# Audio-WestlakeU/FullSubNet

Hardware: NVIDIA H100
Metric: frames_per_sec (higher is better)
Workload: dtype f16x3(hi+lo split, fp32-class)xf32acc

## Files before the change

### fullsubnet_b200/_lib.py

```python
from __future__ import annotations

import ctypes as C
import os
from typing import Optional

import numpy as np
import torch

_HERE = os.path.dirname(os.path.abspath(__file__))
LIB_PATH = os.path.join(_HERE, "csrc", "libfsn_b200.so")

FSN_OK, FSN_ERR_SHAPE, FSN_ERR_UNSUPPORTED, FSN_ERR_CUDA, FSN_ERR_WORKSPACE = 0, 1, 2, 3, 4
ACT = {None: 0, False: 0, "": 0, "ReLU": 1, "Tanh": 2, "ReLU6": 3}
CELL = {"LSTM": 0, "GRU": 1}
PREC = {"fp32": 0, "f16_tc": 1, "tf32_tc": 2, "f16x3_tc": 3}


class ModelDesc(C.Structure):
    _fields_ = [(n, C.c_int32) for n in (
        "num_freqs", "look_ahead", "fb_num_neighbors", "sb_num_neighbors", "fb_hidden", "sb_hidden",
        "fb_activation", "sb_activation", "norm_type", "num_groups_in_drop_band", "precision", "cell_type")]


class SeqWeights(C.Structure):
# ... 29 lines not shown

class FastGrads(C.Structure):
    _fields_ = [("enc1", LstmGrads), ("enc2", LstmGrads), ("enc_fc_w", C.c_void_p), ("enc_fc_b", C.c_void_p),
                ("bn", LstmGrads * 2), ("bn_fc_w", C.c_void_p), ("bn_fc_b", C.c_void_p),
                ("dec1", LstmGrads), ("dec2", LstmGrads), ("dec_fc_w", C.c_void_p), ("dec_fc_b", C.c_void_p)]


MAX_PARAM_TENSORS = 64
SB_PROBE_FIELDS, SB_PROBE_SLOTS = 16, 4


class ParamList(C.Structure):
    _fields_ = [("n", C.c_int), ("param", C.c_void_p * MAX_PARAM_TENSORS), ("grad", C.c_void_p * MAX_PARAM_TENSORS),
                ("exp_avg", C.c_void_p * MAX_PARAM_TENSORS), ("exp_avg_sq", C.c_void_p * MAX_PARAM_TENSORS),
                ("numel", C.c_int64 * MAX_PARAM_TENSORS)]


class FullbandDesc(C.Structure):
    _fields_ = [("num_freqs", C.c_int32), ("hidden", C.c_int32), ("num_layers", C.c_int32), ("look_ahead", C.c_int32),
                ("activation", C.c_int32), ("norm_type", C.c_int32), ("precision", C.c_int32), ("cell_type", C.c_int32)]


class FullbandGrads(C.Structure):
    _fields_ = [("layer", LstmGrads * 8), ("fc_w", C.c_void_p), ("fc_b", C.c_void_p)]


IMP_MAX_SECTIONS = 8


class ImprovedDesc(C.Structure):
    _fields_ = [("n_fft", C.c_int32), ("hop_length", C.c_int32), ("win_length", C.c_int32), ("num_freqs", C.c_int32),
                ("fdrc", C.c_float), ("num_sections", C.c_int32), ("freq_cutoffs", C.c_int32 * IMP_MAX_SECTIONS),
                ("sb_num_center", C.c_int32 * IMP_MAX_SECTIONS), ("sb_num_neighbor", C.c_int32 * IMP_MAX_SECTIONS),
                ("fb_num_center", C.c_int32 * IMP_MAX_SECTIONS), ("fb_num_neighbor", C.c_int32 * IMP_MAX_SECTIONS),
                ("fb_hidden", C.c_int32), ("sb_hidden", C.c_int32), ("fb_activation", C.c_int32),
                ("sb_activation", C.c_int32), ("precision", C.c_int32), ("cell_type", C.c_int32)]


class ImprovedWeights(C.Structure):
    _fields_ = [("fb", SeqWeights), ("sb", SeqWeights * IMP_MAX_SECTIONS), ("sb_packed", C.c_void_p * IMP_MAX_SECTIONS)]


class ImprovedGrads(C.Structure):
    _fields_ = [("fb", SeqGrads), ("sb", SeqGrads * IMP_MAX_SECTIONS)]


_P, _I, _L, _F, _S = C.c_void_p, C.c_int, C.c_int64, C.c_float, C.c_size_t
_SIGNATURES = {
    "fsn_version": (C.c_int, []),
    "fsn_last_error": (C.c_char_p, []),
    "fsn_built_arch": (C.c_int, []),
    "fsn_stft": (C.c_int, [_P, _I, _I, _I, _I, _I, _P, _P, _P, _P, _P, _I, _P]),
    "fsn_istft": (C.c_int, [_P, _P, _I, _P, _I, _I, _I, _I, _I, _I, _P, _P]),
    "fsn_decompress_cirm": (C.c_int, [_P, _P, _L, _F, _F, _P]),
    "fsn_compress_cirm": (C.c_int, [_P, _P, _L, _F, _F, _P]),
    "fsn_build_cirm": (C.c_int, [_P, _P, _P, _P, _P, _L, _P]),
    "fsn_drop_band": (C.c_int, [_P, _P, _I, _I, _I, _I, _I, _P]),
    "fsn_model_workspace_bytes": (_S, [C.POINTER(ModelDesc), _I, _I]),
    "fsn_sb_packed_bytes": (_S, [C.POINTER(ModelDesc)]),
    "fsn_pack_sb_weights": (C.c_int, [C.POINTER(ModelDesc), C.POINTER(SeqWeights), _P, _P]),
    "fsn_model_forward": (C.c_int, [C.POINTER(ModelDesc), C.POINTER(SeqWeights), C.POINTER(SeqWeights), _P, _P,
                                    _I, _I, _P, _P, _S, _P]),
    "fsn_enhance_workspace_bytes": (_S, [C.POINTER(ModelDesc), _I, _I, _I, _I]),
    "fsn_enhance": (C.c_int, [C.POINTER(ModelDesc), C.POINTER(SeqWeights), C.POINTER(SeqWeights), _P, _P, _P, _I, _I,
                              _I, _I, _I, _P, _P, _P, _F, _P, _S, _P]),
    "fsn_fast_workspace_bytes": (_S, [C.POINTER(FastDesc), _I, _I]),
    "fsn_fast_packed_bytes": (_S, [C.POINTER(FastDesc)]),
    "fsn_fast_pack_bn_weights": (C.c_int, [C.POINTER(FastDesc), C.POINTER(FastWeights), _P, _P]),
    "fsn_fast_model_forward": (C.c_int, [C.POINTER(FastDesc), C.POINTER(FastWeights), _P, _I, _I, _P, _P, _S, _P]),
    "fsn_improved_workspace_bytes": (_S, [C.POINTER(ImprovedDesc), _I, _I]),
    "fsn_improved_forward": (C.c_int, [C.POINTER(ImprovedDesc), C.POINTER(ImprovedWeights), _P, _I, _I, _P, _P, _P, _S,
                                       _P]),
    "fsn_improved_enhance_workspace_bytes": (_S, [C.POINTER(ImprovedDesc), _I, _I]),
    "fsn_improved_enhance": (C.c_int, [C.POINTER(ImprovedDesc), C.POINTER(ImprovedWeights), _P, _P, _I, _I, _P, _P, _P, _F,
                                       _P, _S, _P]),
    "fsn_improved_packed_bytes": (_S, [C.POINTER(ImprovedDesc), _I]),
    "fsn_improved_pack_sb_weights": (C.c_int, [C.POINTER(ImprovedDesc), C.POINTER(ImprovedWeights), _I, _P, _P]),
    "fsn_improved_train_workspace_bytes": (_S, [C.POINTER(ImprovedDesc), _I, _I]),
    "fsn_improved_train_forward": (C.c_int, [C.POINTER(ImprovedDesc), C.POINTER(ImprovedWeights), _P, _I, _I, _P, _P, _S,
                                             _P]),
    "fsn_improved_train_backward": (C.c_int, [C.POINTER(ImprovedDesc), C.POINTER(ImprovedWeights), _P, _I, _I,
                                              C.POINTER(ImprovedGrads), _P, _S, _P]),
    "fsn_train_workspace_bytes": (_S, [C.POINTER(ModelDesc), _I, _I]),
    "fsn_train_forward": (C.c_int, [C.POINTER(ModelDesc), C.POINTER(SeqWeights), C.POINTER(SeqWeights), _P, _I, _I, _P,
                                    _P, _S, _P]),
    "fsn_train_backward": (C.c_int, [C.POINTER(ModelDesc), C.POINTER(SeqWeights), C.POINTER(SeqWeights), _P, _I, _I,
                                     C.POINTER(SeqGrads), C.POINTER(SeqGrads), _P, _S, _P]),
    "fsn_fast_train_workspace_bytes": (_S, [C.POINTER(FastDesc), _I, _I]),
    "fsn_fast_train_forward": (C.c_int, [C.POINTER(FastDesc), C.POINTER(FastWeights), _P, _I, _I, _P, _P, _S, _P]),
    "fsn_fast_train_backward": (C.c_int, [C.POINTER(FastDesc), C.POINTER(FastWeights), _P, _I, _I, C.POINTER(FastGrads), _P,
                                          _S, _P]),
    "fsn_mse_loss_scratch_bytes": (_S, []),
    "fsn_mse_loss": (C.c_int, [_P, _P, _I, _I, _I, _P, _P, _P, _S, _P]),
    "fsn_cirm_mse_per_clip_workspace_bytes": (_S, [_I, _I, _I, _I]),
    "fsn_cirm_mse_per_clip": (C.c_int, [_P, _P, _P, _I, _I, _I, _I, _I, _P, _P, _P, _S, _P]),
    "fsn_clip_adam_scratch_bytes": (_S, []),
    "fsn_clip_adam": (C.c_int, [C.POINTER(ParamList), _F, _F, _F, _F, _F, _F, _I, _P, _P, _S, _P]),
    "fsn_clip_adam_steps": (C.c_int, [C.POINTER(ParamList), _F, _F, _F, _F, _F, _F, _P, _P, _P, _S, _P]),
    "fsn_fullband_workspace_bytes": (_S, [C.POINTER(FullbandDesc), _I, _I]),
    "fsn_fullband_forward": (C.c_int, [C.POINTER(FullbandDesc), _P, _P, _P, _P, _I, _I, _P, _P, _S, _P]),
    "fsn_fullband_enhance_workspace_bytes": (_S, [C.POINTER(FullbandDesc), _I, _I, _I, _I]),
    "fsn_fullband_enhance": (C.c_int, [C.POINTER(FullbandDesc), _P, _P, _P, _P, _P, _I, _I, _I, _I, _I, _P, _P, _P, _F, _P,
                                       _S, _P]),
    "fsn_fullband_stream_state_bytes": (_S, [C.POINTER(FullbandDesc), _I, _I, _I]),
    "fsn_fullband_stream_workspace_bytes": (_S, [C.POINTER(FullbandDesc), _I, _I, _I, _I]),
    "fsn_fullband_stream_delay": (C.c_int, [C.POINTER(FullbandDesc), _I, _I]),
    "fsn_fullband_stream_step": (C.c_int, [C.POINTER(FullbandDesc), _P, _P, _P, _P, _P, _P, _I, _I, _I, _I, _I, _P, _P, _S,
                                           _P, _S, _P]),
    "fsn_fast_stream_state_bytes": (_S, [C.POINTER(FastDesc), _I, _I, _I]),
    "fsn_fast_stream_workspace_bytes": (_S, [C.POINTER(FastDesc), _I, _I, _I, _I]),
    "fsn_fast_stream_delay": (C.c_int, [C.POINTER(FastDesc), _I, _I]),
    "fsn_fast_stream_step": (C.c_int, [C.POINTER(FastDesc), C.POINTER(FastWeights), _P, _P, _P, _I, _I, _I, _I, _I, _P, _P,
                                       _S, _P, _S, _P]),
    "fsn_fast_stream_tc_state_bytes": (_S, [C.POINTER(FastDesc), _I, _I, _I]),
    "fsn_fast_stream_tc_workspace_bytes": (_S, [C.POINTER(FastDesc), _I, _I, _I, _I]),
    "fsn_fast_stream_tc_delay": (C.c_int, [C.POINTER(FastDesc), _I, _I]),
    "fsn_fast_stream_tc_step": (C.c_int, [C.POINTER(FastDesc), C.POINTER(FastWeights), _P, _P, _P, _I, _I, _I, _I, _I, _P,
                                          _P, _S, _P, _S, _P]),
    "fsn_stream_state_bytes": (_S, [C.POINTER(ModelDesc), _I, _I, _I]),
    "fsn_stream_workspace_bytes": (_S, [C.POINTER(ModelDesc), _I, _I, _I, _I]),
    "fsn_stream_delay": (C.c_int, [C.POINTER(ModelDesc), _I, _I]),
    "fsn_stream_step": (C.c_int, [C.POINTER(ModelDesc), C.POINTER(SeqWeights), C.POINTER(SeqWeights), _P, _P, _P, _I, _I,
                                  _I, _I, _I, _P, _P, _S, _P, _S, _P]),
    "fsn_stream_tc_state_bytes": (_S, [C.POINTER(ModelDesc), _I, _I, _I]),
    "fsn_stream_tc_workspace_bytes": (_S, [C.POINTER(ModelDesc), _I, _I, _I, _I]),
    "fsn_stream_tc_delay": (C.c_int, [C.POINTER(ModelDesc), _I, _I]),
    "fsn_stream_tc_step": (C.c_int, [C.POINTER(ModelDesc), C.POINTER(SeqWeights), C.POINTER(SeqWeights), _P, _P, _P, _P,
                                     _I, _I, _I, _I, _I, _P, _P, _S, _P, _S, _P]),
    "fsn_fullband_train_workspace_bytes": (_S, [C.POINTER(FullbandDesc), _I, _I]),
    "fsn_fullband_train_forward": (C.c_int, [C.POINTER(FullbandDesc), _P, _P, _P, _P, _I, _I, _P, _P, _S, _P]),
    "fsn_fullband_train_backward": (C.c_int, [C.POINTER(FullbandDesc), _P, _P, _P, _P, _I, _I, C.POINTER(FullbandGrads), _P,
                                              _S, _P]),
    "fsn_peak_normalize_int16": (C.c_int, [_P, _I, _I, _F, _P, _P]),
    "fsn_si_sdr": (C.c_int, [_P, _P, _I, _I, _P, _P]),
    "fsn_si_sdr_lengths": (C.c_int, [_P, _P, _P, _I, _I, _P, _P]),
    "fsn_stoi_workspace_bytes": (_S, [_I, _I, _I]),
    "fsn_stoi": (C.c_int, [_P, _P, _P, _I, _I, _I, _P, _P, _S, _P]),
    "fsn_rir_convolve": (C.c_int, [_P, _P, _P, _I, _I, _I, _P, _P]),
    "fsn_snr_mix": (C.c_int, [_P, _P, _P, _P, _F, _F, _I, _I, _P, _P, _P]),
    "fsn_debug_row_to_unit": (C.c_int, [_I, _I, _I, _I, C.POINTER(C.c_int), C.POINTER(C.c_int)]),
    "fsn_debug_unit_to_row": (C.c_int, [_I, _I, _I, _I, _I]),
    "fsn_debug_reflect_count": (C.c_int, [_I, _I, _I]),
    "fsn_debug_lstm_tc_workspace_bytes": (_S, [_I, _I, _I, _I, _I]),
    "fsn_debug_lstm_layer_tc": (C.c_int, [_P, _P, _P, _P, _P, _I, _I, _I, _I, _I, _P, _P, _S, _P]),
    "fsn_debug_lstm_tc_carry": (C.c_int, [_P, _P, _P, _P, _P, _I, _I, _I, _I, _I, _P, _P, _P, _I, _P, _P, _S, _P]),
    "fsn_debug_linear_tc": (C.c_int, [_P, _I, _I, _P, _P, _I, _I, _I, _P, _P, _S, _P]),
    "fsn_debug_lstm_rec_tc_scratch_bytes": (_S, [_I, _I]),
    "fsn_debug_lstm_rec_tc": (C.c_int, [_P, _P, _P, _P, _L, _L, _P, _L, _L, _I, _I, _I, _I, _P, _P, _P, _L, _P, _I, _P, _P,
                                        _S, _P]),
    "fsn_debug_sb_lstm_tc_packed_bytes": (_S, [_I, _I]),
    "fsn_debug_sb_lstm_tc_max_clusters": (C.c_int, [_I, _I, _I, _I, C.POINTER(C.c_int)]),
    "fsn_debug_sb_lstm_tc": (C.c_int, [C.POINTER(SeqWeights), _I, _I, _I, _I, _I, _I, _P, _P, _I, _I, _I, _I, _P, _P, _I,
                                       _I, _I, _I, _I, _P, _P, _P]),
    "fsn_debug_sb_lstm_tc_carry": (C.c_int, [C.POINTER(SeqWeights), _I, _I, _I, _I, _I, _P, _P, _I, _I, _I, _P, _I, _P,
                                             _I, _P, _P, _P, _P, _P]),
    "fsn_debug_sb_lstm_tc_phased": (C.c_int, [C.POINTER(SeqWeights), _I, _I, _I, _I, _P, _P, _I, _I, _I, _I, _P, _P, _P,
                                              _P, _P, _P, _P, _P, _P, _P]),
    "fsn_debug_sb_lstm_tc_probe": (C.c_int, [C.POINTER(SeqWeights), _I, _I, _I, _I, _I, _I, _P, _P, _I, _I, _I, _I, _P, _P,
                                             _I, _I, _I, _I, _I, _P, _P, _P, _I, _I, _P]),
    "fsn_debug_tgemm": (C.c_int, [_P, _L, _P, _L, _P, _L, _I, _I, _I, _I, _P, _L, _P]),
    "fsn_debug_tgemm_blocked": (C.c_int, [_P, _P, _P, _I, _I, _I, _I, _I, _P, _L, _P]),
    "fsn_debug_lstm_fwd_step": (C.c_int, [_P, _P, _P, _P, _I, _P, _P, _P, _P, _P, _P, _I, _I, _I, _P, _L, _P]),
    "fsn_debug_fc_gemm": (C.c_int, [_P, _P, _P, _P, _I, _I, _I, _I, _I, _P]),
    "fsn_debug_sgemm": (C.c_int, [_I, _P, _L, _P, _L, _P, _L, _I, _I, _I, _I, _P, _L, _P]),
    "fsn_debug_colsum": (C.c_int, [_P, _L, _I, _L, _P, _P, _P, _L, _P]),
    "fsn_debug_small_out_wgrad": (C.c_int, [_P, _P, _L, _I, _P, _P, _L, _P]),
    "fsn_debug_transpose": (C.c_int, [_P, _L, _I, _P, _P]),
    "fsn_debug_transpose_blocked": (C.c_int, [_P, _L, _I, _L, _P, _P, _I, C.POINTER(C.c_int), _P, _P]),
    "fsn_debug_gemm_tc": (C.c_int, [_P, _L, _I, _P, _I, _I, _P, _I, _P, _I, _I, _P, _L, _L, _P, _S, _P]),
    "fsn_debug_lstm_train_workspace_bytes": (_S, [_I, _I, _I, _I, _I, _I]),
    "fsn_debug_lstm_train": (C.c_int, [C.POINTER(LstmLayer), _I, _I, _I, _I, _I, _I, _P, _P, _P, _P, _I, _P, _P,
                                       C.POINTER(LstmGrads), _P, _P, _S, _P]),
    "fsn_debug_seq_stack_workspace_bytes": (_S, [_I, C.POINTER(C.c_int), _I, _I, _I, _I, _I, _I, _I, _I]),
    "fsn_debug_seq_stack": (C.c_int, [C.POINTER(LstmLayer), _I, C.POINTER(C.c_int), _I, _I, _I, _I, _I, _I, _I, _I, _P, _P,
                                      _P, _P, _I, _I, _P, _P, _S, C.POINTER(C.c_int), _P]),
    "fsn_debug_stft": (C.c_int, [_P, _I, _I, _I, _I, _I, _P, _P, _P, _P, _P, _P, _P, _I, _P]),
    "fsn_debug_istft": (C.c_int, [_P, _P, _I, _P, _I, _I, _I, _I, _I, _I, _I, _P, _P, _P, _P, _P, _F, _P, _P]),
    "fsn_debug_istft_mask_adjoint": (C.c_int, [_P, _P, _P, _I, _I, _I, _I, _I, _I, _P, _P]),
    "fsn_debug_wav_epilogue": (C.c_int, [_P, _P, _I, _I, _P, _P, _F, _P, _P, _I, _I, _I, _P]),
    "fsn_debug_norm_unfold_bwd": (C.c_int, [_P, _P, _P, _P, _I, _I, _I, _I, _I, _I, _F, _I, _P, _P, _P]),
    "fsn_debug_fast_norm_unfold_bwd": (C.c_int, [_P, _P, _P, _P, _P, _P, _I, _I, _I, _I, _I, _I, _I, _F, _P, _P, _P, _P]),
    "fsn_debug_imp_unfold_bwd": (C.c_int, [_P, _P, _P, _P, _I, _I, _I, _I, _I, _I, _I, _I, _I, _I, _I, _P, _P, _P]),
    "fsn_debug_imp_section_input": (C.c_int, [_P, _P, _I, _I, _I, _I, _I, _I, _I, _I, _I, _I, _P, _P, _P]),
    "fsn_debug_imp_section_lstm_tc_workspace_bytes": (_S, [_I, _I, _I, _I, _I]),
    "fsn_debug_imp_section_lstm_tc": (C.c_int, [C.POINTER(SeqWeights), _I, _I, _I, _P, _I, _I, _I, _I, _P, _P, _P, _S, _P]),
    "fsn_debug_norm_stats": (C.c_int, [_P, _I, _I, _I, _I, _L, _L, _P, _P, _I, _I, _P, _F, _F, _F, _P, _P, _P, _P, _P]),
    "fsn_debug_train_stats": (C.c_int, [_P, _I, _I, _I, _I, _I, _P, _P]),
    "fsn_debug_forgetting_scale": (C.c_int, [_P, _I, _P, _I, _I, _I, _I, _L, _L, _F, _P, _P, _I, _I, _P, _P, _P, _P, _P]),
    "fsn_debug_forgetting_bwd": (C.c_int, [_P, _P, _P, _P, _I, _I, _I, _I, _I, _I, _P, _P, _P]),
    "fsn_debug_stoi_stages": (C.c_int, [_P, _P, _P, _I, _I, _I, _P, _P, _P, _P, _P, _P, _P, _S, _P]),
    "fsn_debug_cum_clip_scale": (C.c_int, [_P, _I, _I, _I, _L, _L, _F, _P, _P, _P]),
    "fsn_debug_cum_unit_scale": (C.c_int, [_P, _P, _I, _I, _I, _I, _I, _I, _F, _I, _P, _P]),
    "fsn_debug_forget_unit_broadcast": (C.c_int, [_P, _I, _I, _I, _I, _P, _P]),
    "fsn_debug_fast_bn": (C.c_int, [_P, _P, _L, _L, _I, _I, _I, _I, _I, _I, _I, _F, _P, _P, _P, _P, _P]),
    "fsn_debug_fast_dec_input": (C.c_int, [_P, _P, _L, _L, _L, _I, _I, _I, _I, _I, _L, _L, _P, _P]),
    "fsn_debug_transpose_mag": (C.c_int, [_P, _I, _I, _I, _I, _L, _L, _P, _P, _P, _P]),
    "fsn_debug_crm_output": (C.c_int, [_P, _L, _L, _I, _I, _I, _I, _P, _P]),
    "fsn_debug_scale_rows": (C.c_int, [_P, _P, _L, _I, _I, _I, _P, _P]),
    "fsn_debug_imp_compress": (C.c_int, [_P, _I, _I, _I, _F, _I, _P, _P]),
    "fsn_debug_train_gather": (C.c_int, [_P, _P, _P, _P, _I, _I, _I, _I, _I, _I, _P, _P]),
    "fsn_debug_sb_head": (C.c_int, [_P, _I, _I, _I, _P, _P, _I, _I, _I, _I, _I, _I, _L, _L, _I, _P, _P]),
    "fsn_debug_sb_head_bwd": (C.c_int, [_P, _P, _I, _I, _I, _I, _I, _I, _I, _I, _I, _L, _L, _P, _P]),
    "fsn_debug_train_dy": (C.c_int, [_P, _P, _I, _I, _I, _I, _I, _I, _P, _P]),
    "fsn_last_error_code": (C.c_int, []),
    "fsn_last_launch_count": (C.c_int64, []),
    "fsn_total_launch_count": (C.c_int64, []),
    "fsn_set_profiling": (C.c_int, [_I]),
    "fsn_last_stage_ms": (C.c_float, [_I]),
}
EXPORTED_SYMBOLS = tuple(_SIGNATURES)

_lib: Optional[C.CDLL] = None


def load() -> C.CDLL:
    global _lib
    if _lib is None:
        if not os.path.exists(LIB_PATH):
            raise RuntimeError(
                f"fullsubnet_b200: {LIB_PATH} is missing. Build it with `python -c 'import __graft_entry__ as g; "
                "g.build()'` (nvcc, sm_90a). There is no CPU/PyTorch fallback for this path.")
        lib = C.CDLL(LIB_PATH)
        for name, (res, args) in _SIGNATURES.items():
            fn = getattr(lib, name)
            fn.restype, fn.argtypes = res, args
        _lib = lib
    return _lib


def check(rc: int) -> None:
    if rc == FSN_OK:
        return
    msg = load().fsn_last_error().decode()
    if rc == FSN_ERR_SHAPE:
        raise AssertionError(msg)
    if rc == FSN_ERR_UNSUPPORTED:
        raise NotImplementedError(msg)
    raise RuntimeError(f"libfsn_b200 error {rc}: {msg}")


def check_workspace(nbytes: int) -> int:
    if nbytes == 0:
        check(load().fsn_last_error_code() or FSN_ERR_SHAPE)
    return nbytes


def require_cuda(t: torch.Tensor, what: str) -> torch.Tensor:
    if not t.is_cuda:
        raise RuntimeError(
            f"fullsubnet_b200: {what} must be a CUDA tensor (got {t.device}); this package has no CPU path.")
    if t.dtype != torch.float32:
        t = t.float()
    return t.contiguous()


def lengths_table(lengths, B: int, L: int) -> np.ndarray:
    if isinstance(lengths, torch.Tensor):
        if lengths.is_cuda or lengths.is_floating_point() or lengths.is_complex() or lengths.dim() != 1:
            raise ValueError("lengths must be a 1-D CPU integer tensor or a sequence of ints")
        lengths = lengths.tolist()
    lens = np.ascontiguousarray([int(v) for v in lengths], dtype=np.int32)
    if lens.shape != (B,):
        raise ValueError(f"lengths has {lens.size} entries for a batch of {B} clips")
    if lens.size and int(lens.max()) > L:
        b = int(lens.argmax())
        raise ValueError(f"lengths[{b}] = {int(lens[b])} exceeds the {L} samples of a row")
    return lens


def stream_ptr(device) -> int:
    return torch.cuda.current_stream(device).cuda_stream


def ptr(t: Optional[torch.Tensor]) -> Optional[int]:
    return None if t is None else t.data_ptr()
```

### fullsubnet_b200/csrc/fsn_internal.cuh

```cuda
#pragma once
#include <cudaTypedefs.h>
#include <cuda_fp16.h>

#include "fsn_common.cuh"

namespace fsn {

struct Carver {
  char* base; size_t off;
  explicit Carver(void* p) : base((char*)p), off(0) {}
  template <class T> T* take(size_t n) {
    T* r = base ? (T*)(base + off) : nullptr;
    off = align_up(off + n * sizeof(T), 256);
    return r;
  }
};

inline fsn_lstm_layer seq_layer(const fsn_seq_weights& w, int l) { return {w.w_ih[l], w.w_hh[l], w.b_ih[l], w.b_hh[l]}; }

inline unsigned ew_grid(size_t n) {
  const size_t g = (n + 255) / 256;
  return (unsigned)(g < 1 ? 1 : (g > 132 * 16 ? 132 * 16 : g));
}

// ... 226 lines not shown
                 unsigned int* peak_bits = nullptr, const int* lens = nullptr);

struct WavWs {
  float *real, *imag, *crm;
  unsigned int* peak;
  int* lens;
};
void wav_carve(Carver& c, int B, int F, int T, WavWs& w);
int wav_check(const int32_t* lengths, int B, int L_max, int n_fft, bool pow2_lengths, const float* enhanced,
              const char* who);
int wav_prologue(const int32_t* lengths, int B, WavWs& w, cudaStream_t st);
int wav_epilogue(const WavWs& w, const float* enhanced, int B, int L, int16_t* pcm, float gain, float* crm_out, int F, int T,
                 int hop, cudaStream_t st);

int istft_mask_adjoint_launch(const float* dwav, const float* real, const float* imag, int B, int L, int T, int n_fft,
                              int hop, int win_length, float* dcrm, cudaStream_t st);

struct SecGeom { int lo, N, cs, ns, cf, nf, W; };
struct ImpDims { int B, L, T, F, Fu, S; SecGeom sec[FSN_IMP_MAX_SECTIONS]; int maxRW, maxR; };
int imp_dims(const fsn_improved_desc* d, int B, int L, ImpDims& m);
int imp_compress_launch(const float* mag, int B, int F, int T, float fdrc, bool tm, float* out, cudaStream_t st);
int imp_section_input_launch(const float* magc, const float* fbT, int B, int T, int Fu, const SecGeom& g, float* X, float2* fs,
                             bool tm, cudaStream_t st);
int sec_geom(int lo, int hi, int cs, int ns, int cf, int nf, int Fu, SecGeom& g);
int imp_unfold_bwd_launch(const float* dX, const float* invs, const float* dot, float cnt, const SecGeom& g, int B, int T,
                          int Fu, bool first, int act, const float* y, float* dfb, cudaStream_t st);
inline HeadGeom imp_head_geom(const SecGeom& g, int F, int T) { return HeadGeom{g.N, g.cs, g.lo, F, (size_t)T}; }

struct FbState {
  const float* h_init[2]; const float* c_init[2];
  float* h_fin[2]; float* c_fin[2];
  const int* restart;
  int fin_step;
};
bool fb_persistent_supported(int F, int H0, int H1);
int fb_persistent_launch(const fsn_lstm_layer* L, const float* x, const float* inv1, float* h0buf, float* h1all,
                         unsigned int* barrier, int R, int F, int H0, int H1, int Tp, cudaStream_t st,
                         const FbState* io = nullptr);

bool lstm_rec_tc_supported(int H, bool x3);
int lstm_rec_tc_rows_per_launch(int H);
size_t lstm_rec_tc_scratch_bytes(int H, bool x3);
struct RecCarry {
  const float *h_init, *c_init;
  float* c_fin;
  size_t row;
  const int* restart;
  int fin_step;
};
struct RecTcInfo {
  int rows_per_launch, stages, launches, smem_bytes;
};
int lstm_rec_tc_launch(const float* w_hh, const float* b_ih, const float* b_hh, const float* P, size_t p_row, size_t p_t,
                       float* hall, size_t h_row, size_t h_t, int R, int T, int H, bool x3, void* scratch,
                       cudaStream_t st, const RecCarry* io = nullptr, RecTcInfo* info = nullptr);
int split_tf32_launch(const float* in, size_t rows, int K, size_t ldi, const float* row_scale, int rows_per_scale,
                      float* out, int Kp, int cat, cudaStream_t st, int scale_B = 0);
int bias_act_launch(float* x, size_t rows, int N, size_t ld, const float* bias, int act, cudaStream_t st);
struct LstmTcWs { float *a, *w, *P; void* rec; };
void lstm_tc_carve(Carver& c, size_t rows_T, int Kmax, int Hmax, bool x3, LstmTcWs& ws);
int lstm_layer_tc(const fsn_lstm_layer& L, const float* x, size_t ldx, int K, const float* row_scale, int rows_per_scale,
                  int scale_B, int R, int T, int H, bool x3, const LstmTcWs& ws, float* hall, cudaStream_t st,
                  const RecCarry* io = nullptr);
int linear_tc(const float* x, size_t ldx, int K, const float* W, const float* bias, int N, int act, float* out, size_t ldo,
              size_t rows, bool x3, const LstmTcWs& ws, cudaStream_t st);
int gemm_tc_split_launch(const float* a, size_t lda, const float* W, int N, int K, float* w, float* C, size_t ldc, size_t M,
                         bool x3, cudaStream_t st);

static const int SEQ_MAX_LAYERS = 8;
struct SeqStack {
  int R, Tp, K0, n, O, act;
  int H[SEQ_MAX_LAYERS];
  fsn_lstm_layer L[SEQ_MAX_LAYERS];
  bool gru, step_scale, tc, x3;
  bool force_stepwise;
  const float *x, *scale, *fc_w, *fc_b;
  float* out;
};
enum SeqPath {
  SEQ_PATH_TC = FSN_SEQ_PATH_TC,
  SEQ_PATH_PERSISTENT = FSN_SEQ_PATH_PERSISTENT,
  SEQ_PATH_STEP2 = FSN_SEQ_PATH_STEP2,
  SEQ_PATH_ONE_LAYER = FSN_SEQ_PATH_ONE_LAYER
};
SeqPath seq_stack_path(const SeqStack& s);
struct SeqStackWs {
  float *hall[2], *h0[2], *c0, *c1, *pp;
  unsigned int* barrier;
  LstmTcWs tc;
};
void seq_stack_carve(Carver& c, const SeqStack& s, SeqStackWs& w);
int seq_stack_forward(const SeqStack& s, const SeqStackWs& w, cudaStream_t st);

struct StreamGeom { int n, hop, la, c, D, Hs, Rc, Q, E; };
int stream_geom(int n_fft, int hop, int win_length, int la, StreamGeom& g);
struct StreamMeta { int pos, active; float acc; int pad; };
int stream_prologue(const int32_t* start, const int32_t* tail, int B, char* state, size_t slot_bytes, int* pos0, int* act0,
                    int* tail_dev, cudaStream_t st);
int stream_norm_launch(const float2* fs, int B, int S, int K, int F, const StreamGeom& g, int norm_type, const int* pos0,
                       const int* act0, const int* tail, char* state, size_t slot_bytes, float* scaleT, cudaStream_t st,
                       const float2* fs2 = nullptr, size_t acc_off = 0);
int stream_cum_unit_launch(const float* magT, const float* fbT, int B, int S, int K, int F, int Ns, int Nf,
                           const StreamGeom& g, const int* pos0, const int* act0, char* state, size_t slot_bytes,
                           size_t run_off, float* scaleT, cudaStream_t st);
int stream_reset_launch(const int* pos0, int B, const StreamGeom& g, int j, int H, float* h, size_t h_row, float* c,
                        cudaStream_t st);
int stream_restart_launch(const int* pos0, int B, const StreamGeom& g, int* restart, cudaStream_t st);
int stream_dsp_check(int n_fft, int hop, int win_length);
int stft_stream_launch(const float* win, int Wn, int Hs, const int* pos0, const int* tail, int B, int n_fft, int hop,
                       int win_length, int c, int S, int Q, float* magT, float* spec, cudaStream_t st);
int istft_stream_launch(const float* spec, const float* crm, const int* pos0, const int* act0, const int* tail, int B,
                        int K, int D, int n_fft, int hop, int win_length, int c, int la, int Rc, int Q, int S, float* wav,
                        cudaStream_t st);
struct StackCarry { char* state; size_t slot, h, c; const int* pos0; StreamGeom g; const int* restart; int K; };
struct StreamStackWs { SeqStackWs seq; float* h; float *h_fin[2], *c_fin[2]; };
void stream_stack_carve(Carver& c, const SeqStack& s, StreamStackWs& w);
int stream_seq_stack(const SeqStack& s, const StreamStackWs& w, const StackCarry& io, cudaStream_t st);
int copy_rows(void* dst, size_t dp, const void* src, size_t sp, size_t width, int B, cudaStream_t st);

struct StreamSlot {
  size_t hist, spec, crm, end;
  StreamSlot(const StreamGeom& g, int F);
  size_t sec(size_t floats) { const size_t at = end; end = align_up(end + floats * 4, 16); return at; }
  size_t slot() const { return align_up(end, 256); }
};
struct StreamWs {
  int *pos0, *act0, *tail;
  float *wav, *magT, *spec, *crm;
};
void stream_carve(Carver& c, const StreamGeom& g, int B, int K, int F, StreamWs& w);
int stream_query_check(int rc, const char* who, int B, int K_max);
inline int stream_delay(int rc, const StreamGeom& g) { return rc ? -rc : g.D; }
int stream_check(const char* who, const StreamGeom& g, int B, int K, const int32_t* tail, const float* wav,
                 const float* enhanced, int& St);
int stream_check_sizes(const void* state, size_t state_bytes, size_t slot, int B, const void* workspace,
                       size_t workspace_bytes, size_t ws_need);
int stream_open(const StreamGeom& g, const StreamSlot& sl, const StreamWs& w, int F, int B, int K, int St, int win_length,
                const int32_t* start, const int32_t* tail, const float* wav, char* state, int* restart, cudaStream_t st);
int stream_close(const StreamGeom& g, const StreamSlot& sl, const StreamWs& w, int F, int B, int K, int St, int win_length,
                 const float* y, float* enhanced, char* state, cudaStream_t st);

struct SbTcArgs {
  const void* packed;
  const float* magT; const float* fbT; const float* inv2;
  const float* unit_scale;
  float* crm;
  int B, F, Tp, la, Ns, Nf, H, act;
  int steps, shrink;
  bool x3;
  RowMap map;
  int stages, cluster;
  long long* stamps;
  int stamp_ctas, stamp_its;
};
size_t sb_tc_packed_bytes(const fsn_model_desc* d);
size_t sb_tc_packed_bytes_raw(int H, bool x3, bool proj = false);
int sb_tc_pack(const fsn_model_desc* d, const fsn_seq_weights* sb, void* packed, cudaStream_t st);
int sb_tc_pack_raw(const fsn_seq_weights* sb, int H, int Ksb, int fc_out, void* packed, cudaStream_t st, bool x3,
                   bool proj = false);
int sb_tc_forward(const SbTcArgs& a, cudaStream_t st);
struct SbCarry {
  float *h, *c;
  size_t slot, layer;
  int rps;
  const int* restart;
  int store_step;
  size_t crm_bs;
  int crm_t0;
  const float* x;
  const int* store_at;
};
int sb_tc_carry_forward(const SbTcArgs& a, const SbCarry& io, cudaStream_t st);
bool sb_tc_supported(const fsn_model_desc* d);
void sb_tc_ring_defaults(int& stages, int& cluster);
struct SbProjArgs {
  const void* packed;
  const float* P;
  float* h1;
  int R, T, H;
  bool x3;
  int stages, cluster;
};
int sb_proj_forward(const SbProjArgs& a, cudaStream_t st);
struct ImpSecTcWs { LstmTcWs gemm; float *P, *h1; };
void imp_section_tc_carve(Carver& c, size_t rows_T, int Wmax, int H, bool x3, ImpSecTcWs& w);
int imp_section_lstm_tc(const fsn_seq_weights& sw, const void* packed, const float* X, int R, int T, int W, int H, bool x3,
                        const ImpSecTcWs& w, cudaStream_t st, int stages = 0, int cluster = 0);

}
```

### fullsubnet_b200/csrc/fsn_model.cu

```cuda
#include <string.h>

#include "fsn_internal.cuh"

namespace fsn {

static thread_local char g_err[512] = "";
static thread_local int64_t g_launches = 0;

void set_error(const char* fmt, ...) {
  va_list ap;
  va_start(ap, fmt);
  vsnprintf(g_err, sizeof(g_err), fmt, ap);
  va_end(ap);
}
static thread_local int g_err_code = 0;
int& last_error_code() { return g_err_code; }
int64_t& launch_counter() { return g_launches; }
static int64_t g_total_launches = 0;
int64_t& total_launch_counter() { return g_total_launches; }

static thread_local bool g_prof = false;
static thread_local cudaEvent_t g_ev[5] = {nullptr, nullptr, nullptr, nullptr, nullptr};
static thread_local bool g_ev_valid[5] = {false, false, false, false, false};
static void prof_mark(int i, cudaStream_t st) {
  if (!g_prof) return;
  if (!g_ev[i] && cudaEventCreate(&g_ev[i]) != cudaSuccess) return;
  g_ev_valid[i] = (cudaEventRecord(g_ev[i], st) == cudaSuccess);
}
static void prof_reset() { for (int i = 0; i < 5; ++i) g_ev_valid[i] = false; }

struct ModelWs {
  float *magT, *fbT, *inv1, *inv2;
  float2 *fs, *sums_mag, *sums_fb;
  float *cum1, *cum2;
  float2* fs2;
  SeqStackWs fb;
  float *sb_h0[2], *sb_h1[2], *sb_c0, *sb_c1;
  size_t bytes;
};

static SeqStack fb_stack(const fsn_model_desc* d, int B, int Tp) {
  SeqStack s;
  memset(&s, 0, sizeof(s));
  const int F = d->num_freqs;
  s.R = B; s.Tp = Tp; s.K0 = F; s.n = 2; s.H[0] = s.H[1] = d->fb_hidden; s.O = F; s.act = d->fb_activation;
  s.gru = d->cell_type == FSN_CELL_GRU;
  s.step_scale = norm_per_step(d->norm_type);
  s.x3 = d->precision == FSN_PREC_F16X3_TC;
  s.tc = (s.x3 || d->precision == FSN_PREC_F16_TC) && !s.gru && lstm_rec_tc_supported(d->fb_hidden, s.x3);
  return s;
}

int make_dims(const fsn_model_desc* d, int B, int T, Dims& m) {
  FSN_REQUIRE(d && d->num_freqs > 1 && d->fb_hidden > 0 && d->sb_hidden > 0 && d->look_ahead >= 0, FSN_ERR_SHAPE,
              "model: bad descriptor");
  FSN_REQUIRE(B > 0 && T > 0, FSN_ERR_SHAPE, "model: empty input (B=%d, T=%d)", B, T);
  FSN_REQUIRE(d->norm_type == FSN_NORM_OFFLINE_LAPLACE || d->norm_type == FSN_NORM_CUMULATIVE_LAPLACE ||
                  d->norm_type == FSN_NORM_FORGETTING,
              FSN_ERR_UNSUPPORTED,
              "You must set up a type of Norm. (offline_laplace_norm / cumulative_laplace_norm / forgetting_norm are built)");
  FSN_REQUIRE(d->cell_type == FSN_CELL_LSTM || (d->cell_type == FSN_CELL_GRU && d->precision == FSN_PREC_FP32),
              FSN_ERR_UNSUPPORTED, "model: sequence_model must be LSTM, or GRU on the fp32 kernels (precision fp32)");
  FSN_REQUIRE(d->sb_num_neighbors >= 0 && d->fb_num_neighbors >= 0 && d->sb_num_neighbors < d->num_freqs &&
                  d->fb_num_neighbors < d->num_freqs,
              FSN_ERR_SHAPE, "model: reflect padding needs num_neighbors < num_freqs");
  m.B = B; m.T = T; m.Tp = T + d->look_ahead; m.F = d->num_freqs;
  m.G = (B > 1 && d->num_groups_in_drop_band > 1) ? d->num_groups_in_drop_band : 1;
  if (B > 1)
    FSN_REQUIRE(B > d->num_groups_in_drop_band, FSN_ERR_SHAPE,
                "Batch size = %d, num_groups = %d. The batch size should larger than the num_groups.", B,
                d->num_groups_in_drop_band);
  m.Fsub = (m.G > 1) ? m.F / m.G : m.F;
  FSN_REQUIRE(m.Fsub > 0, FSN_ERR_SHAPE, "model: num_freqs < num_groups");
  m.R = B * m.Fsub;
  m.Ksb = (2 * d->sb_num_neighbors + 1) + (2 * d->fb_num_neighbors + 1);
  return FSN_OK;
}

static void carve_model(const fsn_model_desc* d, const Dims& m, void* base, ModelWs& w) {
  Carver c(base);
  const size_t BTF = (size_t)m.B * m.Tp * m.F;
  w.magT = c.take<float>(BTF);
  w.fbT = c.take<float>(BTF);
  w.fs = c.take<float2>((size_t)m.B * m.Tp);
  w.sums_mag = c.take<float2>(m.B);
  w.sums_fb = c.take<float2>(m.B);
  w.inv1 = c.take<float>(m.B);
  w.inv2 = c.take<float>(m.B);
  seq_stack_carve(c, fb_stack(d, m.B, m.Tp), w.fb);
  if (d->precision == FSN_PREC_FP32) {
    const size_t RH = (size_t)m.R * d->sb_hidden;
    for (int i = 0; i < 2; ++i) { w.sb_h0[i] = c.take<float>(RH); w.sb_h1[i] = c.take<float>(RH); }
    w.sb_c0 = c.take<float>(RH);
    w.sb_c1 = c.take<float>(RH);
  }
  w.cum1 = w.cum2 = nullptr;
  w.fs2 = nullptr;
  if (norm_per_step(d->norm_type)) {
    w.cum1 = c.take<float>((size_t)m.Tp * m.B);
    w.cum2 = c.take<float>((size_t)m.Tp * m.R);
  }
  if (d->norm_type == FSN_NORM_FORGETTING) w.fs2 = c.take<float2>((size_t)m.B * m.Tp);
  w.bytes = c.off;
}

static int model_core(const fsn_model_desc* d, const fsn_seq_weights* fb, const fsn_seq_weights* sb,
                      const void* sb_packed, const Dims& m, const ModelWs& w, float* crm, cudaStream_t st,
                      const int* lens = nullptr, int hop = 0) {
  int rc;
  const int F = m.F, Tp = m.Tp, B = m.B, Hs = d->sb_hidden, la = d->look_ahead;
  const int tp_cnt = lens ? 1 : Tp;
  if ((rc = clip_stats_launch(w.magT, B, Tp, F, d->sb_num_neighbors, w.fs, w.sums_mag, st, lens, hop, la))) return rc;
  if ((rc = norm_scales_launch(w.sums_mag, w.sums_mag, B, (float)F * tp_cnt, 1.f, w.inv1, nullptr, st, 1e-5f, lens, hop,
                               la)))
    return rc;
  const bool cum = d->norm_type == FSN_NORM_CUMULATIVE_LAPLACE, fgt = d->norm_type == FSN_NORM_FORGETTING;
  const float cum_eps = 1.1920928955078125e-07f;
  if (cum && (rc = cum_clip_scale_launch(w.fs, B, Tp, F, cum_eps, w.cum1, st))) return rc;
  if (fgt && (rc = forget_scale_launch(w.fs, nullptr, B, Tp, (float)F, w.cum1, nullptr, st))) return rc;

  SeqStack s = fb_stack(d, B, Tp);
  s.L[0] = seq_layer(*fb, 0); s.L[1] = seq_layer(*fb, 1);
  s.x = w.magT; s.scale = (cum || fgt) ? w.cum1 : w.inv1; s.fc_w = fb->fc_w; s.fc_b = fb->fc_b; s.out = w.fbT;
  if ((rc = seq_stack_forward(s, w.fb, st))) return rc;

  if ((rc = clip_stats_launch(w.fbT, B, Tp, F, d->fb_num_neighbors, fgt ? w.fs2 : w.fs, w.sums_fb, st, lens, hop, la)))
    return rc;
  if ((rc = norm_scales_launch(w.sums_mag, w.sums_fb, B, 1.f, (float)F * m.Ksb * tp_cnt, nullptr, w.inv2, st, 1e-5f, lens,
                               hop, la)))
    return rc;

  prof_mark(2, st);
  RowMap map{B, F, m.Fsub, m.G};
  if (cum && (rc = cum_unit_scale_launch(w.magT, w.fbT, map, m.R, Tp, d->sb_num_neighbors, d->fb_num_neighbors, cum_eps,
                                         w.cum2, st)))
    return rc;
  if (fgt) {
    if ((rc = forget_scale_launch(w.fs, w.fs2, B, Tp, (float)F * m.Ksb, w.cum1, nullptr, st))) return rc;
    if ((rc = forget_unit_broadcast_launch(w.cum1, map, m.R, Tp, w.cum2, st))) return rc;
  }
  if (d->precision == FSN_PREC_F16_TC || d->precision == FSN_PREC_F16X3_TC) {
    FSN_REQUIRE(sb_packed, FSN_ERR_SHAPE, "model: the tensor-core precisions need packed sub-band weights");
    SbTcArgs a;
    memset(&a, 0, sizeof(a));
    a.packed = sb_packed; a.magT = w.magT; a.fbT = w.fbT; a.inv2 = w.inv2; a.crm = crm;
    a.B = B; a.F = F; a.Tp = Tp; a.la = d->look_ahead; a.Ns = d->sb_num_neighbors; a.Nf = d->fb_num_neighbors;
    a.H = Hs; a.act = d->sb_activation; a.map = map; a.x3 = d->precision == FSN_PREC_F16X3_TC;
    a.unit_scale = (cum || fgt) ? w.cum2 : nullptr;
    rc = sb_tc_forward(a, st);
    prof_mark(3, st);
    return rc;
  }

  const Step2State s2{{w.sb_h0[0], w.sb_h0[1]}, w.sb_c0, {w.sb_h1[0], w.sb_h1[1]}, w.sb_c1, Hs, 0};
  for (int t = 0; t < Tp; ++t) {
    StepParams p;
    memset(&p, 0, sizeof(p));
    p.R = m.R; p.H = Hs; p.gru = d->cell_type == FSN_CELL_GRU;
    p.K0 = m.Ksb;
    p.w_ih = sb->w_ih[0]; p.w_hh = sb->w_hh[0]; p.b_ih = sb->b_ih[0]; p.b_hh = sb->b_hh[0];
    p.magT = w.magT; p.fbT = w.fbT; p.inv2 = w.inv2;
    p.unit_scale = (cum || fgt) ? w.cum2 + (size_t)t * m.R : nullptr;
    p.F = F; p.Tp = Tp; p.t = t; p.Ns = d->sb_num_neighbors; p.Nf = d->fb_num_neighbors; p.map = map;
    if ((rc = lstm_step2_launch(p, SEG0_GATHER, t, seq_layer(*sb, 1), s2, st))) return rc;
    if (t >= d->look_ahead)
      if ((rc = sb_head_launch(s2.h1_at(t), m.R, Hs, 1, sb->fc_w, sb->fc_b, 2, d->sb_activation, crm,
                               fsn_head_geom(m.Fsub, m.T), t - d->look_ahead, st)))
        return rc;
  }
  prof_mark(3, st);
  return FSN_OK;
}

}

using namespace fsn;

extern "C" int fsn_version(void) { return 102; }
extern "C" const char* fsn_last_error(void) { return g_err; }
extern "C" int fsn_last_error_code(void) { return g_err_code; }
extern "C" int64_t fsn_last_launch_count(void) { return g_launches; }
extern "C" int64_t fsn_total_launch_count(void) { return g_total_launches; }
extern "C" int fsn_set_profiling(int enable) { g_prof = enable != 0; return FSN_OK; }
extern "C" float fsn_last_stage_ms(int stage) {
  if (stage < 0 || stage > 3 || !g_ev_valid[stage] || !g_ev_valid[stage + 1]) return -1.0f;
  float ms = -1.0f;
  if (cudaEventElapsedTime(&ms, g_ev[stage], g_ev[stage + 1]) != cudaSuccess) return -1.0f;
  return ms;
}
extern "C" int fsn_debug_row_to_unit(int B, int F, int G, int r, int* b, int* f) {
  const int g = (B > 1 && G > 1) ? G : 1;
  RowMap m{B, F, g > 1 ? F / g : F, g};
  if (r < 0 || r >= B * m.Fsub) return FSN_ERR_SHAPE;
  row_to_unit(m, r, *b, *f);
  return FSN_OK;
}
extern "C" int fsn_debug_unit_to_row(int B, int F, int G, int b, int f) {
  const int g = (B > 1 && G > 1) ? G : 1;
  RowMap m{B, F, g > 1 ? F / g : F, g};
  return unit_to_row(m, b, f);
}
extern "C" int fsn_debug_reflect_count(int r, int F, int N) { return reflect_count(r, F, N); }

extern "C" int fsn_built_arch(void) {
#ifdef FSN_BUILT_ARCH
  return FSN_BUILT_ARCH;
#else
  return 0;
#endif
}

extern "C" size_t fsn_model_workspace_bytes(const fsn_model_desc* d, int B, int T) {
  Dims m;
  if (make_dims(d, B, T, m)) return 0;
  ModelWs w;
  carve_model(d, m, nullptr, w);
  return w.bytes;
}

extern "C" size_t fsn_sb_packed_bytes(const fsn_model_desc* d) { return sb_tc_packed_bytes(d); }

extern "C" int fsn_pack_sb_weights(const fsn_model_desc* d, const fsn_seq_weights* sb, void* packed,
                                   fsn_stream_t stream) {
  return sb_tc_pack(d, sb, packed, (cudaStream_t)stream);
}

extern "C" int fsn_model_forward(const fsn_model_desc* d, const fsn_seq_weights* fb, const fsn_seq_weights* sb,
                                 const void* sb_packed, const float* noisy_mag, int B, int T, float* crm,
                                 void* workspace, size_t workspace_bytes, fsn_stream_t stream) {
  g_launches = 0;
  Dims m;
  int rc = make_dims(d, B, T, m);
  if (rc) return rc;
  if ((rc = layout_clips_check(B, false, "model"))) return rc;
  FSN_REQUIRE(d->precision == FSN_PREC_FP32 || sb_tc_supported(d), FSN_ERR_UNSUPPORTED,
              "FSN_PREC_F16_TC / FSN_PREC_F16X3_TC need sb_hidden in {128,256,384} and sub-band input width <= 32");
  ModelWs w;
  carve_model(d, m, workspace, w);
  FSN_REQUIRE(workspace && workspace_bytes >= w.bytes, FSN_ERR_WORKSPACE, "workspace too small: %zu < %zu",
              workspace_bytes, w.bytes);
  cudaStream_t st = (cudaStream_t)stream;
  prof_reset();
  prof_mark(0, st);
  if ((rc = transpose_mag_launch(noisy_mag, B, m.F, T, m.Tp, (size_t)m.Tp * m.F, m.F, w.magT, nullptr, nullptr, st))) return rc;
  prof_mark(1, st);
  return model_core(d, fb, sb, sb_packed, m, w, crm, st);
}

static int enhance_dims(const fsn_model_desc* d, int B, int L, int n_fft, int hop, fsn_model_desc& dd, Dims& m) {
  FSN_REQUIRE(hop > 0 && n_fft > 0, FSN_ERR_SHAPE, "enhance: bad n_fft/hop");
  dd = *d;
  dd.num_groups_in_drop_band = 1;
  int rc = make_dims(&dd, B, 1 + L / hop, m);
  if (rc) return rc;
  FSN_REQUIRE(n_fft / 2 + 1 == d->num_freqs, FSN_ERR_SHAPE, "enhance: n_fft/2+1 = %d != num_freqs = %d",
              n_fft / 2 + 1, d->num_freqs);
  return FSN_OK;
}

static size_t carve_enhance(const fsn_model_desc* d, const Dims& m, void* base, WavWs& e, ModelWs& w) {
  Carver c(base);
  wav_carve(c, m.B, m.F, m.T, e);
  carve_model(d, m, base ? (char*)base + c.off : nullptr, w);
  return c.off + w.bytes;
}

extern "C" size_t fsn_enhance_workspace_bytes(const fsn_model_desc* d, int B, int L_max, int n_fft, int hop) {
  fsn_model_desc dd;
  Dims m;
  if (enhance_dims(d, B, L_max, n_fft, hop, dd, m)) return 0;
  WavWs e;
  ModelWs w;
  return carve_enhance(&dd, m, nullptr, e, w);
}

extern "C" int fsn_enhance(const fsn_model_desc* d, const fsn_seq_weights* fb, const fsn_seq_weights* sb,
                           const void* sb_packed, const float* wav, const int32_t* lengths, int B, int L_max, int n_fft,
                           int hop, int win_length, float* enhanced, float* crm_out, int16_t* pcm, float gain,
                           void* workspace, size_t workspace_bytes, fsn_stream_t stream) {
  g_launches = 0;
  fsn_model_desc dd;
  Dims m;
  int rc = enhance_dims(d, B, L_max, n_fft, hop, dd, m);
  if (rc) return rc;
  FSN_REQUIRE(dd.precision == FSN_PREC_FP32 || sb_tc_supported(&dd), FSN_ERR_UNSUPPORTED,
              "FSN_PREC_F16_TC / FSN_PREC_F16X3_TC need sb_hidden in {128,256,384} and sub-band input width <= 32");
  if ((rc = wav_check(lengths, B, L_max, n_fft, true, enhanced, "enhance"))) return rc;
  WavWs e;
  ModelWs w;
  const size_t bytes = carve_enhance(&dd, m, workspace, e, w);
  FSN_REQUIRE(workspace && workspace_bytes >= bytes, FSN_ERR_WORKSPACE, "workspace too small: %zu < %zu",
              workspace_bytes, bytes);
  cudaStream_t st = (cudaStream_t)stream;
  float* crm = crm_out ? crm_out : e.crm;
  prof_reset();
  prof_mark(0, st);
  if ((rc = wav_prologue(lengths, B, e, st))) return rc;
  if ((rc = stft_launch(wav, B, L_max, n_fft, hop, win_length, nullptr, nullptr, e.real, e.imag, w.magT, m.Tp, st,
                        e.lens)))
    return rc;
  prof_mark(1, st);
// ... 222 lines not shown
```

### fullsubnet_b200/csrc/fsn_subband_tc.cu

```cuda
#include <cuda_fp16.h>
#include <stdlib.h>
#include <string.h>

#include "fsn_internal.cuh"
#include "fsn_tc_ptx.cuh"
#include "fsn_wgmma.cuh"

namespace fsn {
namespace tc {

using namespace ptx;

constexpr int NB = 32;
constexpr int KB = 64;
constexpr int KS = 32;
constexpr int US = 64;
constexpr int W_SUB = US * KS * 2;
constexpr int W_TILE = 4 * W_SUB;
constexpr int S_KBLK = NB * KB * 2;
constexpr int X_BLK = NB * KS * 2;
constexpr int MAX_STAGES = 4;
constexpr int MAX_MT = 3;
constexpr int OUT_T = 8;
constexpr int NTHREADS = 128 + 128 * MAX_MT;

struct PackedLayout {
  int H, MT, nkb0, nkb1, parts;
  size_t tiles0, tiles1;
  size_t off_bias, off_fcw, off_fcb, bytes;
};

__host__ __device__ inline PackedLayout packed_layout(int H, bool x3, bool proj = false) {
  PackedLayout L;
  L.H = H; L.MT = H / 128;
  L.nkb0 = (proj ? 0 : 1) + H / KS; L.nkb1 = 2 * H / KS;
  L.parts = x3 ? 2 : 1;
  L.tiles0 = (size_t)L.MT * L.nkb0 * L.parts;
  L.tiles1 = (size_t)L.MT * L.nkb1 * L.parts;
  L.off_bias = 2 * (L.tiles0 + L.tiles1) * W_TILE;
  L.off_fcw = L.off_bias + (size_t)2 * 4 * H * sizeof(float);
  L.off_fcb = L.off_fcw + (size_t)2 * H * sizeof(float);
  L.bytes = L.off_fcb + 256;
  return L;
}

__global__ void pack_kernel(const float* __restrict__ wih0, const float* __restrict__ whh0,
                            const float* __restrict__ wih1, const float* __restrict__ whh1,
                            const float* __restrict__ bih0, const float* __restrict__ bhh0,
                            const float* __restrict__ bih1, const float* __restrict__ bhh1,
                            const float* __restrict__ fcw, const float* __restrict__ fcb, int H, int Ksb, int x3,
                            int fc_out, int proj, uint8_t* __restrict__ out) {
  const PackedLayout L = packed_layout(H, x3 != 0, proj != 0);
  const size_t per_half = L.tiles0 + L.tiles1;
  const size_t total = 2 * per_half * 4 * US * 4;
  for (size_t i = blockIdx.x * (size_t)blockDim.x + threadIdx.x; i < total; i += (size_t)gridDim.x * blockDim.x) {
    const int c = (int)(i & 3);
    const int r = (int)((i >> 2) & (US - 1));
    const int g = (int)((i >> 8) & 3);
    const size_t st_abs = i >> 10;
    const int half = (int)(st_abs / per_half);
    size_t st = st_abs - half * per_half;
    const int layer = st >= L.tiles0;
    if (layer) st -= L.tiles0;
    const int part = (int)(st % L.parts);
    st /= L.parts;
    const int nkb = layer ? L.nkb1 : L.nkb0;
    const int kb = (int)(st % nkb);
    const int m = (int)(st / nkb);
    const int wrow = g * H + (half * L.MT + m) * US + r;
    __half v[8];
#pragma unroll
    for (int e = 0; e < 8; ++e) {
      const int kk = c * 8 + e;
      float w = 0.f;
      if (layer == 0 && proj) {
        w = whh0[(size_t)wrow * H + kb * KS + kk];
      } else if (layer == 0) {
        if (kb == 0) { if (kk < Ksb) w = wih0[(size_t)wrow * Ksb + kk]; }
        else w = whh0[(size_t)wrow * H + (kb - 1) * KS + kk];
      } else {
        const int k = kb * KS + kk;
        w = (k < H) ? wih1[(size_t)wrow * H + k] : whh1[(size_t)wrow * H + (k - H)];
      }
      const __half hi = __float2half_rn(w);
      v[e] = part ? __float2half_rn(w - __half2float(hi)) : hi;
    }
    uint8_t* dst = out + st_abs * W_TILE + g * W_SUB + swz64_off(r, c * 8);
    *reinterpret_cast<uint4*>(dst) = *reinterpret_cast<const uint4*>(v);
  }
  float* bias = reinterpret_cast<float*>(out + L.off_bias);
  float* pfcw = reinterpret_cast<float*>(out + L.off_fcw);
  float* pfcb = reinterpret_cast<float*>(out + L.off_fcb);
  for (int i = blockIdx.x * blockDim.x + threadIdx.x; i < 4 * H; i += gridDim.x * blockDim.x) {
    bias[i] = proj ? 0.f : bih0[i] + bhh0[i];
    bias[4 * H + i] = bih1[i] + bhh1[i];
  }
  for (int i = blockIdx.x * blockDim.x + threadIdx.x; i < 2 * H; i += gridDim.x * blockDim.x)
    pfcw[i] = (!proj && i < fc_out * H) ? fcw[i] : 0.f;
  if (blockIdx.x == 0 && threadIdx.x < 2)
    pfcb[threadIdx.x] = (!proj && (int)threadIdx.x < fc_out) ? fcb[threadIdx.x] : 0.f;
}

struct Smem {
  uint32_t w, x, h0, h1, lo, fcw, fcp, outst, rows, bars, total;
};
__host__ __device__ inline Smem smem_plan(int H, int stages, bool x3) {
  Smem s;
  const int nkh = H / KB;
  uint32_t o = 0;
  s.w = o; o += stages * W_TILE;
  s.x = o; o += 2 * X_BLK;
  s.h0 = o; o += 2 * nkh * S_KBLK;
  s.h1 = o; o += nkh * S_KBLK;
  s.lo = o; o += x3 ? (o - s.x) : 0;
  s.fcw = o; o += 4 * MAX_MT * 2 * NB * 4;
  s.fcp = o; o += 2 * 2 * NB * 4;
  s.outst = o; o += NB * 2 * OUT_T * 4;
  s.rows = o; o += NB * 16;
  s.bars = o; o += 256;
  s.total = o;
  return s;
}

struct Bars {
  uint64_t w_full[MAX_STAGES], w_empty[MAX_STAGES];
  uint64_t x_full[2], x_empty[2];
  uint64_t h0_ready[2], h0_empty[2];
  uint64_t h1_ready, h1_empty, fc_done;
  uint64_t l1_done;
  uint64_t fcp_full[2], fcp_empty[2];
  uint64_t turn[MAX_MT];
};
static_assert(sizeof(Bars) <= 256, "barrier block too large");

struct RowInfo {
  int src_b, src_f;
  float scale;
  union {
    int out_idx;
    int restart;
  };
};

struct KArgs {
  const uint8_t* packed;
  const float* magT; const float* fbT; const float* inv2;
  const float* unit_scale;
  float* crm;
  int R, F, Tp, la, T, Ns, Nf, H, Ksb, act, Fsub, stages, cluster;
  int src_T, shrink;
  RowMap map;
  long long* stamps;
  int stamp_ctas, stamp_its;
  const float* proj; float* h1;
  float* io_h; float* io_c;
  size_t io_slot, io_layer, crm_bs;
  const int* restart;
  int io_rps, store_step, crm_t0;
  const float* xin;
  const int* store_at;
};

enum ProbeField {
  PF_T_BEGIN = 0,
  PF_T_MMA0 = 1,
  PF_T_MMA1 = 2,
  PF_T_END = 3,
  PF_OPERAND = 4,
  PF_TURN = 5,
  PF_W_FULL = 6,
  PF_WAIT_GROUP = 7,
  PF_GROUP_LAT = 8,
  PF_STAGES = 9,
  PF_CELL = 10,
  PF_L1_DONE = 11,
  PF_H1_EMPTY = 12,
  PF_H0_EMPTY = 13,
  PF_FC_DONE = 14,
  PF_GT_BEGIN = 15,
  PROBE_FIELDS = 16
};
constexpr int PROBE_SLOTS = MAX_MT + 1;
static_assert(PROBE_FIELDS == FSN_SB_PROBE_FIELDS && PROBE_SLOTS == FSN_SB_PROBE_SLOTS,
              "probe record layout differs from fsn_b200.h (and fullsubnet_b200/_lib.py)");

__device__ __forceinline__ long long globaltimer() {
  uint64_t t;
  asm volatile("mov.u64 %0, %%globaltimer;" : "=l"(t));
  return (long long)t;
}

__device__ __forceinline__ float act_apply(float v, int act) {
  switch (act) {
    case FSN_ACT_RELU: return fmaxf(v, 0.f);
    case FSN_ACT_TANH: return tanhf(v);
    case FSN_ACT_RELU6: return fminf(fmaxf(v, 0.f), 6.f);
    default: return v;
  }
}
template <bool X3> __device__ __forceinline__ float sg(float x) { return X3 ? 1.0f / (1.0f + expf(-x)) : fast_sigmoid(x); }
template <bool X3> __device__ __forceinline__ float th(float x) { return X3 ? 1.0f - 2.0f / (1.0f + expf(2.0f * x)) : fast_tanh(x); }

__device__ __forceinline__ void release_stage(uint32_t bar, uint32_t pred, uint32_t local, uint32_t remote,
                                              uint32_t rank) {
  mbar_arrive_elect_if(bar, pred & local);
  mbar_arrive_remote_elect_if(bar, rank, pred & remote);
}

__device__ __forceinline__ float proj_at(const KArgs& a, int t, int row0, int s, int q, int lane, int g, int i) {
  const int j = i >> 2, hh = (i >> 1) & 1, e = i & 1;
  const int u = s * US + 16 * q + (lane >> 2) + 8 * hh;
  const int r = min(row0 + 8 * j + 2 * (lane & 3) + e, a.R - 1);
  return __ldg(a.proj + ((size_t)t * a.R + r) * 4 * a.H + g * a.H + u);
}

__device__ __forceinline__ size_t carry_idx(const KArgs& a, int r, int u) {
  const int sl = r / a.io_rps;
  return (size_t)sl * a.io_slot + (size_t)(r - sl * a.io_rps) * a.H + u;
}

template <bool X3, bool PROBE, bool PROJ, bool CARRY, bool PHASED = false>
__device__ __forceinline__ void sb_lstm_tc_body(const KArgs& a) {
  static_assert(!PHASED || CARRY, "the block-phased policy is a carry policy");
  constexpr int PARTS = X3 ? 2 : 1;
  long long pt = 0;
  auto mark = [&]() -> uint32_t {
    if constexpr (PROBE) {
      const long long n = clock64();
      const uint32_t d = (uint32_t)(n - pt);
      pt = n;
      return d;
    } else {
      return 0u;
    }
  };
  auto record = [&](int it, int layer, int slot) -> long long* {
    return a.stamps + ((((size_t)blockIdx.x * a.stamp_its + it) * 2 + layer) * PROBE_SLOTS + slot) * PROBE_FIELDS;
  };
  const bool probe_cta = PROBE && (int)blockIdx.x < a.stamp_ctas;
  extern __shared__ uint8_t smem_raw[];
  uint8_t* smem = smem_raw + ((1024u - (smem_u32(smem_raw) & 1023u)) & 1023u);
  const int H = a.H;
  const int MT = H / 128;
  const int nkh = H / KB;
  const int STAGES = a.stages;
  const int CL = a.cluster;
  const uint32_t cl_rank = cluster_ctarank();
  const int half = (int)(cl_rank & 1u);
  const uint32_t peer = cl_rank ^ 1u;
  const uint16_t cl_mask = (uint16_t)((0x55u & ((1u << (2 * CL)) - 1u)) << half);
  const Smem sp = smem_plan(H, STAGES, X3);
  const uint32_t LO = sp.lo - sp.x;
  const PackedLayout PL = packed_layout(H, X3, PROJ);
  Bars& bars = *reinterpret_cast<Bars*>(smem + sp.bars);
  RowInfo* rows = reinterpret_cast<RowInfo*>(smem + sp.rows);
  float* fc_part = reinterpret_cast<float*>(smem + sp.fcw);
  float* fcp = reinterpret_cast<float*>(smem + sp.fcp);
  float* outst = reinterpret_cast<float*>(smem + sp.outst);
  const int warp = threadIdx.x >> 5, lane = threadIdx.x & 31;
  const int row0 = (blockIdx.x >> 1) * NB;
  const int Tp = a.Tp;

  if (threadIdx.x == 0) {
    for (int s = 0; s < STAGES; ++s) { mbar_init(&bars.w_full[s], 1); mbar_init(&bars.w_empty[s], CL); }
    for (int i = 0; i < 2; ++i) {
      mbar_init(&bars.x_full[i], 1); mbar_init(&bars.x_empty[i], 4 * MT);
      mbar_init(&bars.h0_ready[i], 5 * MT);
      mbar_init(&bars.h0_empty[i], MT);
      mbar_init(&bars.fcp_full[i], 1); mbar_init(&bars.fcp_empty[i], 1);
    }
    mbar_init(&bars.h1_ready, 5 * MT);
    mbar_init(&bars.h1_empty, MT);
    mbar_init(&bars.fc_done, 1);
    mbar_init(&bars.l1_done, 4 * MT);
    for (int m = 0; m < MAX_MT; ++m) mbar_init(&bars.turn[m], 4);
    asm volatile("fence.mbarrier_init.release.cluster;" ::: "memory");
  }
  if (!PROJ && threadIdx.x < NB) {
    RowInfo ri;
    const int r = row0 + threadIdx.x;
    ri.src_b = -1; ri.src_f = 0; ri.scale = 0.f; ri.out_idx = 0;
    if (r < a.R) {
      row_to_unit(a.map, r, ri.src_b, ri.src_f);
      if constexpr (CARRY) {
        ri.restart = a.restart[r / a.io_rps];
        if constexpr (PHASED) ri.scale = __int_as_float(a.store_at[r / a.io_rps]);
      } else {
        ri.scale = a.inv2[ri.src_b];
        const int bq = r / a.Fsub, fq = r - bq * a.Fsub;
        ri.out_idx = bq * 2 * a.Fsub + fq;
      }
    }
    rows[threadIdx.x] = ri;
  }
  {
    uint4* z = reinterpret_cast<uint4*>(smem + sp.x);
    const int n16 = (sp.fcw - sp.x) / 16;
    for (int i = threadIdx.x; i < n16; i += blockDim.x) z[i] = make_uint4(0, 0, 0, 0);
  }
  if constexpr (CARRY) {
    __syncthreads();
    const int nkh0 = H / KB;
    for (int i = threadIdx.x; i < 2 * NB * H; i += blockDim.x) {
      const int l = i / (NB * H), n = (i / H) % NB, U = i % H;
      const int r = row0 + n;
      if (r >= a.R || a.restart[r / a.io_rps] == 0) continue;
      const float v = a.io_h[carry_idx(a, r, U) + l * a.io_layer];
      uint8_t* p = smem + (l ? sp.h1 : sp.h0 + nkh0 * S_KBLK) + (U >> 6) * S_KBLK + (n >> 3) * 1024 + (n & 7) * 128 +
                   ((((U & 63) >> 3) ^ (n & 7)) << 4) + (U & 7) * 2;
      const __half hi = __float2half_rn(v);
      *reinterpret_cast<__half*>(p) = hi;
      if (X3) *reinterpret_cast<__half*>(p + (sp.lo - sp.x)) = __float2half_rn(v - __half2float(hi));
    }
  }
  fence_proxy_async_smem();
  __syncthreads();
  cluster_sync_all();

  if (warp < 4) {
    asm volatile("setmaxnreg.dec.sync.aligned.u32 56;");
  if (warp == 0) {
    const uint8_t* stream = a.packed + (size_t)half * (PL.tiles0 + PL.tiles1) * W_TILE;
    uint32_t stage = 0, phase = 0;
    for (int it = 0; it <= Tp; ++it) {
      const size_t t_begin = (it < Tp) ? 0 : PL.tiles0;
      const size_t t_end = (it >= 1) ? PL.tiles0 + PL.tiles1 : PL.tiles0;
      const uint8_t* src = stream + t_begin * W_TILE;
      long long p_t0 = 0, p_g0 = 0;
      uint32_t p_empty = 0;
      if constexpr (PROBE) { p_g0 = globaltimer(); p_t0 = clock64(); pt = p_t0; }
      for (size_t tile = t_begin; tile < t_end; ++tile, src += W_TILE) {
        mark();
        mbar_wait_cta<false>(&bars.w_empty[stage], phase ^ 1);
        p_empty += mark();
        if (elect_one()) {
          mbar_expect_tx(&bars.w_full[stage], W_TILE);
          if (CL == 1) {
            bulk_g2s(smem + sp.w + stage * W_TILE, src, W_TILE, &bars.w_full[stage]);
          } else {
            const uint32_t slice = W_TILE / CL, off = (cl_rank >> 1) * slice;
            bulk_g2s_mc(smem + sp.w + stage * W_TILE + off, src + off, slice, &bars.w_full[stage], cl_mask);
          }
        }
        __syncwarp();
        if (++stage == (uint32_t)STAGES) { stage = 0; phase ^= 1; }
      }
      if (probe_cta && it < a.stamp_its && lane == 0) {
        long long* r = record(it, 0, MAX_MT);
        r[PF_T_BEGIN] = p_t0; r[PF_T_END] = clock64(); r[PF_OPERAND] = p_empty;
        r[PF_STAGES] = (long long)(t_end - t_begin); r[PF_GT_BEGIN] = p_g0;
      }
    }
  } else if (!PROJ && warp == 2) {
    const int nmag = 2 * a.Ns + 1;
// ... 98 lines not shown
      if constexpr (CARRY) {
#pragma unroll
        for (int i = 0; i < 16; ++i) {
          const int hh = i >> 3, j = (i >> 1) & 3, e = i & 1;
          const int r = row0 + 8 * j + 2 * (lane & 3) + e;
          if (r < a.R) {
            const float* p = a.io_c + carry_idx(a, r, s * US + 16 * q + (lane >> 2) + 8 * hh);
            c0[i] = p[0];
            c1[i] = p[a.io_layer];
          }
        }
      }
      const uint32_t a_lo0 = wg::desc_lo(smem_u32(smem + sp.w));
      const uint32_t w_full0 = smem_u32(&bars.w_full[0]), w_empty0 = smem_u32(&bars.w_empty[0]);
      const uint32_t turn_next = smem_u32(&bars.turn[m + 1 < MT ? m + 1 : 0]);
      const uint32_t rel_local = CL == 1 && q == 0, rel_remote = CL > 1 && q < CL;
      const uint32_t rel_rank = 2 * q + half;
      int h0_seen = 0, h1_seen = 0, turns = 0;
      bool first_block = true;
      size_t tile_base = 0;
      for (int it = 0; it <= Tp; ++it) {
        for (int layer = 0; layer < 2; ++layer) {
          const int t = it - layer;
          if (t < 0 || t >= Tp) continue;
          long long p_t0 = 0, p_g0 = 0, p_mma0 = 0, p_mma1 = 0, p_commit = 0, p_commit_prev = 0;
          uint32_t p_opnd = 0, p_turn = 0, p_wfull = 0, p_wgw = 0, p_lat = 0, p_cell = 0, p_l1 = 0, p_h1e = 0, p_h0e = 0,
                   p_fc = 0;
          if constexpr (PROBE) { p_g0 = globaltimer(); p_t0 = clock64(); pt = p_t0; }
          if (layer == 0) {
            if constexpr (!PROJ) mbar_wait_cta<false>(&bars.x_full[t & 1], (t >> 1) & 1);
            for (; h0_seen < t; ++h0_seen) mbar_wait_cta<false>(&bars.h0_ready[h0_seen & 1], (h0_seen >> 1) & 1);
          } else {
            for (; h0_seen < t + 1; ++h0_seen) mbar_wait_cta<false>(&bars.h0_ready[h0_seen & 1], (h0_seen >> 1) & 1);
            for (; h1_seen < t; ++h1_seen) mbar_wait_cta<false>(&bars.h1_ready, h1_seen & 1);
          }
          p_opnd += mark();
          const uint32_t x_addr = smem_u32(smem + sp.x + (t & 1) * X_BLK);
          const uint32_t h0_cur = smem_u32(smem + sp.h0 + (t & 1) * nkh * S_KBLK);
          const uint32_t h0_prev = smem_u32(smem + sp.h0 + ((t + 1) & 1) * nkh * S_KBLK);
          const uint32_t h1_prev = smem_u32(smem + sp.h1);
          const int nkb = layer ? PL.nkb1 : PL.nkb0;
          const size_t first = tile_base + (layer ? ((it < Tp) ? PL.tiles0 : 0) : 0) + (size_t)m * nkb * PARTS;
          float acc[4][16];
#pragma unroll
          for (int g = 0; g < 4; ++g) {
#pragma unroll
            for (int i = 0; i < 16; ++i) acc[g][i] = 0.f;
            if constexpr (PROJ && X3) {
              if (layer == 0) {
#pragma unroll
                for (int i = 0; i < 16; ++i) acc[g][i] = proj_at(a, t, row0, s, q, lane, g, i);
              }
            }
            wg::fence_operand(acc[g]);
          }
          if constexpr (PROJ && !X3) {
            if (layer == 0) {
#pragma unroll
              for (int i = 0; i < 4; ++i) {
                const int idx = lane + 32 * i;
                const int r = min(row0 + (idx & 31), a.R - 1);
                const float* p = a.proj + ((size_t)t * a.R + r) * 4 * H + (idx >> 5) * H + s * US + 16 * q;
                asm volatile("prefetch.global.L2 [%0];" ::"l"(p));
              }
            }
          }
          int prev_stage = -1;
          if (m > 0 || !first_block) { mbar_wait_cta<false>(&bars.turn[m], turns & 1); ++turns; }
          first_block = false;
          p_turn += mark();
          p_mma0 = pt;
          int stage = __shfl_sync(0xffffffffu, (int)(first % (size_t)STAGES), 0);
          uint32_t wphase = __shfl_sync(0xffffffffu, (uint32_t)((first / (size_t)STAGES) & 1), 0);
          auto issue_stage = [&](int part, uint32_t bd, uint32_t b_hi, uint32_t ends_block) {
            mark();
            mbar_wait_cta_warp(w_full0 + 8 * stage, wphase);
            p_wfull += mark();
            mbar_arrive_elect_if(turn_next, ends_block);
            wg::fence();
            const uint32_t ad = a_lo0 + stage * (W_TILE >> 4);
#pragma unroll
            for (int kk = 0; kk < 2; ++kk)
#pragma unroll
              for (int g = 0; g < 4; ++g) {
                const uint32_t a_off = g * (W_SUB >> 4) + kk * 2;
                wg::mma_f16_n32_w(acc[g], ad, a_off, wg::DESC_SW64_HI, bd, kk * 2, b_hi);
                if (X3 && part == 0) wg::mma_f16_n32_w(acc[g], ad, a_off, wg::DESC_SW64_HI, bd, (LO >> 4) + kk * 2, b_hi);
              }
            wg::commit();
            if constexpr (PROBE) p_commit = clock64();
            mark();
            wg::wait<1>();
            p_wgw += mark();
            if constexpr (PROBE) {
              if (prev_stage >= 0) p_lat += (uint32_t)(pt - p_commit_prev);
              p_commit_prev = p_commit;
            }
            release_stage(w_empty0 + 8 * prev_stage, prev_stage >= 0, rel_local, rel_remote, rel_rank);
            prev_stage = stage;
            if (++stage == STAGES) { stage = 0; wphase ^= 1; }
          };
          if (!PROJ && layer == 0) {
#pragma unroll
            for (int part = 0; part < PARTS; ++part) issue_stage(part, wg::desc_lo(x_addr), wg::DESC_SW64_HI, 0u);
          }
          const int nseg = layer ? 2 : 1;
          int seg = 0;
          do {
            uint32_t bd = wg::desc_lo(layer == 0 ? h0_prev : seg == 0 ? h0_cur : h1_prev);
            int kb = 0;
            do {
              const uint32_t ends_block = seg == nseg - 1 && kb == nkh - 1;
#pragma unroll
              for (int part = 0; part < PARTS; ++part) issue_stage(part, bd, wg::DESC_SW128_HI, 0u);
#pragma unroll
              for (int part = 0; part < PARTS; ++part)
                issue_stage(part, bd + (64 >> 4), wg::DESC_SW128_HI, part == PARTS - 1 ? ends_block : 0u);
              bd += S_KBLK >> 4;
            } while (++kb < nkh);
          } while (++seg < nseg);
          mark();
          wg::wait<0>();
#pragma unroll
          for (int g = 0; g < 4; ++g) wg::fence_operand(acc[g]);
          if constexpr (PROJ && !X3) {
            if (layer == 0) {
#pragma unroll
              for (int g = 0; g < 4; ++g)
#pragma unroll
                for (int i = 0; i < 16; ++i) acc[g][i] += proj_at(a, t, row0, s, q, lane, g, i);
            }
          }
          p_wgw += mark();
          if constexpr (PROBE) { p_lat += (uint32_t)(pt - p_commit_prev); p_mma1 = pt; }
          release_stage(w_empty0 + 8 * prev_stage, 1u, rel_local, rel_remote, rel_rank);
          if (lane == 0 && (!PROJ || layer)) mbar_arrive(layer ? &bars.l1_done : &bars.x_empty[t & 1]);
          if (layer == 1 && lane == 0) {
            if (q == 2) mbar_arrive_remote(&bars.h0_empty[t & 1], peer);
            if (q == 3) mbar_arrive_remote(&bars.h1_empty, peer);
          }
          p_cell += mark();
          if (!PROJ && layer == 1 && t >= 1) mbar_wait_cta<false>(&bars.fc_done, (t - 1) & 1);
          p_fc += mark();
          float fsum[2][8];
#pragma unroll
          for (int i = 0; i < 16; ++i) fsum[i >> 3][i & 7] = 0.f;
          __half hv[2][8];
          __half lv[2][8];
          uint8_t* hb = smem + (layer ? sp.h1 : sp.h0 + (t & 1) * nkh * S_KBLK) + s * S_KBLK;
#pragma unroll
          for (int hh = 0; hh < 2; ++hh) {
            const int u = s * US + 16 * q + (lane >> 2) + 8 * hh;
            const float* bl = bias_g + (layer ? 4 * H : 0);
            const float bi = bl[u], bff = bl[H + u], bg = bl[2 * H + u], bo = bl[3 * H + u];
            const float w0 = fcw[u], w1 = fcw[H + u];
#pragma unroll
            for (int j = 0; j < 4; ++j)
#pragma unroll
              for (int e = 0; e < 2; ++e) {
                const int ri = 4 * j + 2 * hh + e;
                const int ci = hh * 8 + j * 2 + e;
                float cp = layer ? c1[ci] : c0[ci];
                if constexpr (CARRY) {
                  if (rows[8 * j + 2 * (lane & 3) + e].restart == t) cp = 0.f;
                }
                const float cn = sg<X3>(acc[1][ri] + bff) * cp + sg<X3>(acc[0][ri] + bi) * th<X3>(acc[2][ri] + bg);
                if (layer) c1[ci] = cn; else c0[ci] = cn;
                const float h = sg<X3>(acc[3][ri] + bo) * th<X3>(cn);
                __half hi = __float2half_rn(h);
                __half lo = __float2half_rn(h - __half2float(hi));
                if constexpr (CARRY) {
                  const int n = 8 * j + 2 * (lane & 3) + e, r = row0 + n;
                  int store_t;
                  if constexpr (PHASED) store_t = __float_as_int(rows[n].scale); else store_t = a.store_step;
                  if (t == store_t && r < a.R) {
                    const size_t o = carry_idx(a, r, u) + layer * a.io_layer;
                    a.io_h[o] = h;
                    a.io_c[o] = cn;
                  }
                  if (rows[n].restart == t + 1) hi = lo = __float2half_rn(0.f);
                }
                hv[hh][j * 2 + e] = hi;
                lv[hh][j * 2 + e] = lo;
                if (!PROJ && layer) { fsum[0][j * 2 + e] += h * w0; fsum[1][j * 2 + e] += h * w1; }
                if constexpr (PROJ) {
                  const int r = row0 + 8 * j + 2 * (lane & 3) + e;
                  if (layer && r < a.R) a.h1[((size_t)t * a.R + r) * H + u] = h;
                }
              }
          }
          if (layer == 1) {
            if constexpr (!PROJ) {
#pragma unroll
              for (int o = 0; o < 2; ++o)
#pragma unroll
                for (int r = 0; r < 8; ++r) {
                  float v = fsum[o][r];
                  v += __shfl_xor_sync(0xffffffffu, v, 4);
                  v += __shfl_xor_sync(0xffffffffu, v, 8);
                  v += __shfl_xor_sync(0xffffffffu, v, 16);
                  fsum[o][r] = v;
                }
              if (lane < 4) {
#pragma unroll
                for (int o = 0; o < 2; ++o)
#pragma unroll
                  for (int r = 0; r < 8; ++r) my_part[o * NB + 8 * (r >> 1) + 2 * lane + (r & 1)] = fsum[o][r];
              }
            }
            p_cell += mark();
            mbar_wait_cta<false>(&bars.l1_done, t & 1);
            p_l1 += mark();
            mbar_wait_cta<false>(&bars.h1_empty, t & 1);
            p_h1e += mark();
          } else if (t >= 2) {
            p_cell += mark();
            mbar_wait_cta<false>(&bars.h0_empty[t & 1], ((t - 2) >> 1) & 1);
            p_h0e += mark();
          }
#pragma unroll
          for (int hh = 0; hh < 2; ++hh) {
            const int u = 16 * q + (lane >> 2) + 8 * hh;
            uint8_t* ub = hb + (u & 7) * 2;
            const int chunk = u >> 3;
#pragma unroll
            for (int j = 0; j < 4; ++j)
#pragma unroll
              for (int e = 0; e < 2; ++e) {
                const int n = 8 * j + 2 * (lane & 3) + e;
                uint8_t* p = ub + (n >> 3) * 1024 + (n & 7) * 128 + ((chunk ^ (n & 7)) << 4);
                *reinterpret_cast<__half*>(p) = hv[hh][j * 2 + e];
                if (X3) *reinterpret_cast<__half*>(p + LO) = lv[hh][j * 2 + e];
              }
          }
          fence_proxy_async_smem();
          __syncwarp();
          uint64_t* ready = layer ? &bars.h1_ready : &bars.h0_ready[t & 1];
          if (lane == 0) mbar_arrive(ready);
          named_sync(1 + m, 128);
          if (q == 0 && lane == 0) {
            mbar_arrive_expect_tx_remote(ready, peer, PARTS * S_KBLK);
            bulk_s2s_remote(hb, S_KBLK, ready, peer);
            if (X3) bulk_s2s_remote(hb + LO, S_KBLK, ready, peer);
          }
          if constexpr (PROBE) {
            p_cell += mark();
            if (probe_cta && it < a.stamp_its && q == 0 && lane == 0) {
              long long* r = record(it, layer, m);
              r[PF_T_BEGIN] = p_t0; r[PF_T_MMA0] = p_mma0; r[PF_T_MMA1] = p_mma1; r[PF_T_END] = pt;
              r[PF_OPERAND] = p_opnd; r[PF_TURN] = p_turn; r[PF_W_FULL] = p_wfull; r[PF_WAIT_GROUP] = p_wgw;
              r[PF_GROUP_LAT] = p_lat; r[PF_STAGES] = nkb * PARTS; r[PF_CELL] = p_cell; r[PF_L1_DONE] = p_l1;
              r[PF_H1_EMPTY] = p_h1e; r[PF_H0_EMPTY] = p_h0e; r[PF_FC_DONE] = p_fc; r[PF_GT_BEGIN] = p_g0;
            }
          }
        }
        tile_base += ((it < Tp) ? PL.tiles0 : 0) + ((it >= 1) ? PL.tiles1 : 0);
      }
    }
  }

  __syncthreads();
  cluster_sync_all();
}

template <bool X3, bool PROBE>
__global__ void __launch_bounds__(NTHREADS, 1) sb_lstm_tc_kernel(const __grid_constant__ KArgs a) {
  sb_lstm_tc_body<X3, PROBE, false, false>(a);
}

template <bool X3>
__global__ void __launch_bounds__(NTHREADS, 1) sb_proj_lstm_tc_kernel(const __grid_constant__ KArgs a) {
  sb_lstm_tc_body<X3, false, true, false>(a);
}

template <bool X3>
__global__ void __launch_bounds__(NTHREADS, 1) sb_carry_lstm_tc_kernel(const __grid_constant__ KArgs a) {
  sb_lstm_tc_body<X3, false, false, true>(a);
}

template <bool X3>
__global__ void __launch_bounds__(NTHREADS, 1) sb_phased_lstm_tc_kernel(const __grid_constant__ KArgs a) {
  sb_lstm_tc_body<X3, false, false, true, true>(a);
}

}

static int sb_ksb(const fsn_model_desc* d) { return (2 * d->sb_num_neighbors + 1) + (2 * d->fb_num_neighbors + 1); }

static bool sb_tc_shape_ok(int H, int Ksb) { return H % 128 == 0 && H / 128 <= tc::MAX_MT && H >= 128 && Ksb <= tc::KS; }

bool sb_tc_supported(const fsn_model_desc* d) {
  if (d->cell_type != FSN_CELL_LSTM) return false;
  return sb_tc_shape_ok(d->sb_hidden, sb_ksb(d));
}

size_t sb_tc_packed_bytes_raw(int H, bool x3, bool proj) { return tc::packed_layout(H, x3, proj).bytes; }

size_t sb_tc_packed_bytes(const fsn_model_desc* d) {
  if (!sb_tc_supported(d)) return 0;
  return sb_tc_packed_bytes_raw(d->sb_hidden, d->precision == FSN_PREC_F16X3_TC);
}

int sb_tc_pack_raw(const fsn_seq_weights* sb, int H, int Ksb, int fc_out, void* packed, cudaStream_t st, bool x3,
                   bool proj) {
  FSN_REQUIRE(sb_tc_shape_ok(H, proj ? 0 : Ksb), FSN_ERR_UNSUPPORTED,
              "the fp16 tensor-core LSTM stack needs a hidden size in {128,256,384} and an input width <= 32");
  int dev = 0, sms = 132;
  cudaGetDevice(&dev);
  cudaDeviceGetAttribute(&sms, cudaDevAttrMultiProcessorCount, dev);
  tc::pack_kernel<<<sms * 4, 256, 0, st>>>(sb->w_ih[0], sb->w_hh[0], sb->w_ih[1], sb->w_hh[1], sb->b_ih[0], sb->b_hh[0],
                                           sb->b_ih[1], sb->b_hh[1], sb->fc_w, sb->fc_b, H, Ksb, x3 ? 1 : 0, fc_out,
                                           proj ? 1 : 0, (uint8_t*)packed);
  FSN_CHECK_LAUNCH("sb pack_kernel");
  return FSN_OK;
}

int sb_tc_pack(const fsn_model_desc* d, const fsn_seq_weights* sb, void* packed, cudaStream_t st) {
  FSN_REQUIRE(sb_tc_supported(d), FSN_ERR_UNSUPPORTED,
              "FSN_PREC_F16_TC / FSN_PREC_F16X3_TC need sb_hidden in {128,256,384} and sub-band input width <= 32");
  return sb_tc_pack_raw(sb, d->sb_hidden, sb_ksb(d), 2, packed, st, d->precision == FSN_PREC_F16X3_TC);
}

template <bool X3, bool PROBE = false>
static int sb_tc_config(int H, int stages, int cluster, int pairs, cudaStream_t st, cudaLaunchConfig_t& cfg,
                        cudaLaunchAttribute* attr, const void* kern = (const void*)tc::sb_lstm_tc_kernel<X3, PROBE>) {
  const tc::Smem sp = tc::smem_plan(H, stages, X3);
  const size_t smem = sp.total + 1024;
  int rc = check_cuda(cudaFuncSetAttribute(kern, cudaFuncAttributeMaxDynamicSharedMemorySize, (int)smem),
                      "sb_lstm_tc smem attr");
  if (rc) return rc;
  memset(&cfg, 0, sizeof(cfg));
  cfg.gridDim = dim3(2 * pairs);
  cfg.blockDim = dim3(128 + 128 * (H / 128));
  cfg.dynamicSmemBytes = smem;
  cfg.stream = st;
  attr[0].id = cudaLaunchAttributeClusterDimension;
  attr[0].val.clusterDim.x = 2 * cluster;
  attr[0].val.clusterDim.y = 1;
  attr[0].val.clusterDim.z = 1;
  cfg.attrs = attr;
  cfg.numAttrs = 1;
  return FSN_OK;
}

template <bool X3, bool PROBE>
static int sb_tc_launch(const tc::KArgs& a, int H, cudaStream_t st) {
  const int pairs = cdiv(cdiv(a.R, tc::NB), a.cluster) * a.cluster;
  cudaLaunchConfig_t cfg;
  cudaLaunchAttribute attr[1];
  int rc = sb_tc_config<X3, PROBE>(H, a.stages, a.cluster, pairs, st, cfg, attr);
  if (rc) return rc;
  rc = check_cuda(cudaLaunchKernelEx(&cfg, tc::sb_lstm_tc_kernel<X3, PROBE>, a), "sb_lstm_tc_kernel launch");
  if (rc) return rc;
  FSN_CHECK_LAUNCH("sb_lstm_tc_kernel");
  return FSN_OK;
}

static int sb_tc_kargs(const SbTcArgs& s, tc::KArgs& a) {
  memset(&a, 0, sizeof(a));
  a.packed = (const uint8_t*)s.packed;
  a.magT = s.magT; a.fbT = s.fbT; a.inv2 = s.inv2; a.unit_scale = s.unit_scale; a.crm = s.crm;
  a.R = s.map.B * s.map.Fsub; a.F = s.F; a.Tp = s.steps > 0 ? s.steps : s.Tp; a.la = s.la; a.T = a.Tp - s.la;
  a.src_T = s.Tp; a.shrink = s.shrink > 1 ? s.shrink : 1;
  a.Ns = s.Ns; a.Nf = s.Nf; a.H = s.H; a.Ksb = (2 * s.Ns + 1) + (2 * s.Nf + 1); a.act = s.act;
  a.Fsub = s.map.Fsub; a.map = s.map;
  a.stamps = s.stamps; a.stamp_ctas = s.stamp_ctas; a.stamp_its = s.stamp_its;
  FSN_REQUIRE(sb_tc_shape_ok(a.H, a.Ksb), FSN_ERR_UNSUPPORTED, "sb_lstm_tc: unsupported hidden size %d / input width %d",
              a.H, a.Ksb);
  a.proj = nullptr; a.h1 = nullptr;
  int stages = 0, cluster = 0;
  sb_tc_ring_defaults(stages, cluster);
  a.stages = s.stages ? s.stages : stages;
  a.cluster = s.cluster ? s.cluster : cluster;
  return FSN_OK;
}

int sb_tc_forward(const SbTcArgs& s, cudaStream_t st) {
  tc::KArgs a;
  int rc = sb_tc_kargs(s, a);
  if (rc) return rc;
  if (s.stamps) return s.x3 ? sb_tc_launch<true, true>(a, s.H, st) : sb_tc_launch<false, true>(a, s.H, st);
  return s.x3 ? sb_tc_launch<true, false>(a, s.H, st) : sb_tc_launch<false, false>(a, s.H, st);
}

int sb_tc_carry_forward(const SbTcArgs& s, const SbCarry& io, cudaStream_t st) {
  const bool phased = io.store_at != nullptr;
  FSN_REQUIRE((phased ? io.x != nullptr : s.unit_scale != nullptr) && io.h && io.c && io.restart && io.rps > 0 && s.la == 0 &&
                  s.shrink <= 1 && s.map.G <= 1,
              FSN_ERR_SHAPE,
              "sb_carry_lstm_tc: per-row scales (block-phased: the input), state, restart steps, la = 0 and no drop_band / "
              "shrink");
  tc::KArgs a;
  int rc = sb_tc_kargs(s, a);
  if (rc) return rc;
  a.io_h = io.h; a.io_c = io.c; a.io_slot = io.slot; a.io_layer = io.layer; a.io_rps = io.rps;
  a.restart = io.restart; a.store_step = io.store_step; a.crm_bs = io.crm_bs; a.crm_t0 = io.crm_t0;
  a.xin = io.x; a.store_at = io.store_at;
  const int pairs = cdiv(cdiv(a.R, tc::NB), a.cluster) * a.cluster;
  cudaLaunchConfig_t cfg;
  cudaLaunchAttribute attr[1];
  void (*kern)(tc::KArgs);
  if (phased) kern = s.x3 ? tc::sb_phased_lstm_tc_kernel<true> : tc::sb_phased_lstm_tc_kernel<false>;
  else        kern = s.x3 ? tc::sb_carry_lstm_tc_kernel<true> : tc::sb_carry_lstm_tc_kernel<false>;
  rc = s.x3 ? sb_tc_config<true>(s.H, a.stages, a.cluster, pairs, st, cfg, attr, (const void*)kern)
            : sb_tc_config<false>(s.H, a.stages, a.cluster, pairs, st, cfg, attr, (const void*)kern);
  if (rc) return rc;
  const char* name = phased ? "sb_phased_lstm_tc_kernel" : "sb_carry_lstm_tc_kernel";
  if ((rc = check_cuda(cudaLaunchKernelEx(&cfg, kern, a), name))) return rc;
  FSN_CHECK_LAUNCH(name);
  return FSN_OK;
}

int sb_proj_forward(const SbProjArgs& s, cudaStream_t st) {
  FSN_REQUIRE(s.R > 0 && s.T > 0 && sb_tc_shape_ok(s.H, 0), FSN_ERR_UNSUPPORTED,
              "sb_proj_lstm_tc: unsupported hidden size %d (R=%d, T=%d)", s.H, s.R, s.T);
  FSN_REQUIRE(s.packed && s.P && s.h1, FSN_ERR_SHAPE, "sb_proj_lstm_tc: missing buffer");
  tc::KArgs a;
  memset(&a, 0, sizeof(a));
  a.packed = (const uint8_t*)s.packed; a.proj = s.P; a.h1 = s.h1;
  a.R = s.R; a.Tp = s.T; a.T = s.T; a.H = s.H;
  int stages = 0, cluster = 0;
  sb_tc_ring_defaults(stages, cluster);
  a.stages = s.stages ? s.stages : stages;
  a.cluster = s.cluster ? s.cluster : cluster;
  const int pairs = cdiv(cdiv(a.R, tc::NB), a.cluster) * a.cluster;
  cudaLaunchConfig_t cfg;
  cudaLaunchAttribute attr[1];
  const void* kern = s.x3 ? (const void*)tc::sb_proj_lstm_tc_kernel<true> : (const void*)tc::sb_proj_lstm_tc_kernel<false>;
  int rc = s.x3 ? sb_tc_config<true>(s.H, a.stages, a.cluster, pairs, st, cfg, attr, kern)
                : sb_tc_config<false>(s.H, a.stages, a.cluster, pairs, st, cfg, attr, kern);
  if (rc) return rc;
  rc = s.x3 ? check_cuda(cudaLaunchKernelEx(&cfg, tc::sb_proj_lstm_tc_kernel<true>, a), "sb_proj_lstm_tc_kernel launch")
            : check_cuda(cudaLaunchKernelEx(&cfg, tc::sb_proj_lstm_tc_kernel<false>, a), "sb_proj_lstm_tc_kernel launch");
  if (rc) return rc;
  FSN_CHECK_LAUNCH("sb_proj_lstm_tc_kernel");
  return FSN_OK;
}

void sb_tc_ring_defaults(int& stages, int& cluster) {
  static int stages_env = -1;
  if (stages_env < 0) {
    const char* e = getenv("FSN_TC_STAGES");
    stages_env = e ? atoi(e) : 4;
    if (stages_env < 2) stages_env = 2;
    if (stages_env > tc::MAX_STAGES) stages_env = tc::MAX_STAGES;
  }
  static int cluster_env = -1;
  if (cluster_env < 0) {
    const char* e = getenv("FSN_TC_CLUSTER");
    cluster_env = e ? atoi(e) : 1;
    if (cluster_env != 1 && cluster_env != 2 && cluster_env != 4) cluster_env = 1;
  }
  stages = stages_env;
  cluster = cluster_env;
}

}

extern "C" size_t fsn_debug_sb_lstm_tc_packed_bytes(int H, int x3) {
  return fsn::sb_tc_shape_ok(H, 0) ? fsn::sb_tc_packed_bytes_raw(H, x3 != 0) : 0;
}

extern "C" int fsn_debug_sb_lstm_tc_max_clusters(int H, int x3, int stages, int cluster, int* clusters) {
  using namespace fsn;
  FSN_REQUIRE(cluster == 1 || cluster == 2 || cluster == 4, FSN_ERR_UNSUPPORTED,
              "sb_lstm_tc: cluster size %d (1, 2 or 4)", cluster);
  FSN_REQUIRE(stages >= 2 && stages <= tc::MAX_STAGES, FSN_ERR_UNSUPPORTED, "sb_lstm_tc: ring depth %d (2, 3 or 4)",
              stages);
  FSN_REQUIRE(sb_tc_shape_ok(H, 0), FSN_ERR_UNSUPPORTED, "sb_lstm_tc: unsupported hidden size %d", H);
  FSN_REQUIRE(clusters, FSN_ERR_SHAPE, "sb_lstm_tc: missing output");
  cudaLaunchConfig_t cfg;
  cudaLaunchAttribute attr[1];
  int rc = x3 ? sb_tc_config<true>(H, stages, cluster, cluster, nullptr, cfg, attr)
              : sb_tc_config<false>(H, stages, cluster, cluster, nullptr, cfg, attr);
  if (rc) return rc;
  return x3 ? check_cuda(cudaOccupancyMaxActiveClusters(clusters, tc::sb_lstm_tc_kernel<true, false>, &cfg), "sb_lstm_tc occupancy")
            : check_cuda(cudaOccupancyMaxActiveClusters(clusters, tc::sb_lstm_tc_kernel<false, false>, &cfg), "sb_lstm_tc occupancy");
}

static int sb_lstm_tc_hook(const fsn_seq_weights* sb, int H, int Ns, int Nf, int fc_out, int act, int x3,
                           const float* magT, const float* fbT, int B, int F, int src_T, int G, const float* inv2,
                           const float* unit_scale, int la, int steps, int shrink, int stages, int cluster, void* packed,
                           float* crm, long long* stamps, int stamp_ctas, int stamp_steps, fsn_stream_t stream) {
  using namespace fsn;
  FSN_REQUIRE(cluster == 0 || cluster == 1 || cluster == 2 || cluster == 4, FSN_ERR_UNSUPPORTED,
              "sb_lstm_tc: cluster size %d (0, 1, 2 or 4)", cluster);
  FSN_REQUIRE(stages == 0 || (stages >= 2 && stages <= tc::MAX_STAGES), FSN_ERR_UNSUPPORTED,
              "sb_lstm_tc: ring depth %d (0, 2, 3 or 4)", stages);
  FSN_REQUIRE(sb && magT && fbT && inv2 && packed && crm, FSN_ERR_SHAPE, "sb_lstm_tc: missing buffer");
  FSN_REQUIRE(B > 0 && F > 1 && src_T > 0 && Ns >= 0 && Nf >= 0 && Ns < F && Nf < F, FSN_ERR_SHAPE,
              "sb_lstm_tc: bad shape B=%d F=%d src_T=%d Ns=%d Nf=%d", B, F, src_T, Ns, Nf);
  FSN_REQUIRE(fc_out == 1 || fc_out == 2, FSN_ERR_SHAPE, "sb_lstm_tc: fc_out %d (1 or 2)", fc_out);
  FSN_REQUIRE(act >= FSN_ACT_NONE && act <= FSN_ACT_RELU6, FSN_ERR_SHAPE, "sb_lstm_tc: activation %d", act);
  FSN_REQUIRE(shrink >= 1 && G >= 1, FSN_ERR_SHAPE, "sb_lstm_tc: shrink %d / groups %d", shrink, G);
  const int g = (B > 1 && G > 1) ? G : 1;
  FSN_REQUIRE(B == 1 || B > G, FSN_ERR_SHAPE, "sb_lstm_tc: batch size %d <= num_groups %d", B, G);
  const int Fsub = g > 1 ? F / g : F;
  FSN_REQUIRE(Fsub > 0, FSN_ERR_SHAPE, "sb_lstm_tc: num_freqs < num_groups");
  const int max_steps = shrink > 1 ? 1 + cdiv(src_T - 1, shrink) : src_T;
  FSN_REQUIRE(steps > 0 && steps <= max_steps && la >= 0 && la < steps, FSN_ERR_SHAPE,
              "sb_lstm_tc: steps %d / look-ahead %d for %d source frames (shrink %d)", steps, la, src_T, shrink);
  FSN_REQUIRE(!(unit_scale && shrink > 1), FSN_ERR_UNSUPPORTED, "sb_lstm_tc: per-step scales with time down-sampling");
  FSN_REQUIRE(sb_tc_shape_ok(H, (2 * Ns + 1) + (2 * Nf + 1)), FSN_ERR_UNSUPPORTED,
              "sb_lstm_tc: unsupported hidden size %d / input width %d", H, (2 * Ns + 1) + (2 * Nf + 1));
  if (stamps) {
    const int ctas = 2 * cdiv(B * Fsub, tc::NB);
    FSN_REQUIRE(stamp_ctas >= 1 && stamp_ctas <= ctas, FSN_ERR_SHAPE, "sb_lstm_tc probe: %d sampled CTAs (1 .. %d)",
                stamp_ctas, ctas);
    FSN_REQUIRE(stamp_steps >= 1 && stamp_steps <= steps + 1, FSN_ERR_SHAPE,
                "sb_lstm_tc probe: %d sampled iterations (1 .. steps + 1 = %d)", stamp_steps, steps + 1);
  }
  cudaStream_t st = (cudaStream_t)stream;
  int rc = sb_tc_pack_raw(sb, H, (2 * Ns + 1) + (2 * Nf + 1), fc_out, packed, st, x3 != 0);
  if (rc) return rc;
  SbTcArgs a;
  memset(&a, 0, sizeof(a));
  a.packed = packed; a.magT = magT; a.fbT = fbT; a.inv2 = inv2; a.unit_scale = unit_scale; a.crm = crm;
  a.B = B; a.F = F; a.Tp = src_T; a.la = la; a.Ns = Ns; a.Nf = Nf; a.H = H; a.act = act;
  a.steps = steps; a.shrink = shrink; a.x3 = x3 != 0;
  a.map = RowMap{B, F, Fsub, g};
  a.stages = stages; a.cluster = cluster;
  a.stamps = stamps; a.stamp_ctas = stamp_ctas; a.stamp_its = stamp_steps;
  return sb_tc_forward(a, st);
}

extern "C" int fsn_debug_sb_lstm_tc(const fsn_seq_weights* sb, int H, int Ns, int Nf, int fc_out, int act, int x3,
                                    const float* magT, const float* fbT, int B, int F, int src_T, int G,
                                    const float* inv2, const float* unit_scale, int la, int steps, int shrink, int stages,
                                    int cluster, void* packed, float* crm, fsn_stream_t stream) {
  return sb_lstm_tc_hook(sb, H, Ns, Nf, fc_out, act, x3, magT, fbT, B, F, src_T, G, inv2, unit_scale, la, steps, shrink,
                         stages, cluster, packed, crm, nullptr, 0, 0, stream);
}

extern "C" int fsn_debug_sb_lstm_tc_probe(const fsn_seq_weights* sb, int H, int Ns, int Nf, int fc_out, int act, int x3,
                                          const float* magT, const float* fbT, int B, int F, int src_T, int G,
                                          const float* inv2, const float* unit_scale, int la, int steps, int shrink,
                                          int stages, int cluster, void* packed, float* crm, long long* stamps,
                                          int stamp_ctas, int stamp_steps, fsn_stream_t stream) {
  using namespace fsn;
  FSN_REQUIRE(stamps, FSN_ERR_SHAPE, "sb_lstm_tc probe: missing stamp buffer");
  return sb_lstm_tc_hook(sb, H, Ns, Nf, fc_out, act, x3, magT, fbT, B, F, src_T, G, inv2, unit_scale, la, steps, shrink,
                         stages, cluster, packed, crm, stamps, stamp_ctas, stamp_steps, stream);
}

extern "C" int fsn_debug_sb_lstm_tc_carry(const fsn_seq_weights* sb, int H, int Ns, int Nf, int act, int x3,
                                          const float* magT, const float* fbT, int B, int F, int src_T,
                                          const float* unit_scale, int steps, const int32_t* restart, int store_step,
                                          float* h, float* c, void* packed, float* crm, fsn_stream_t stream) {
  using namespace fsn;
  FSN_REQUIRE(sb && magT && fbT && unit_scale && restart && h && c && packed && crm, FSN_ERR_SHAPE,
              "sb_carry_lstm_tc: missing buffer");
  FSN_REQUIRE(B > 0 && F > 1 && src_T > 0 && Ns >= 0 && Nf >= 0 && Ns < F && Nf < F && steps > 0 && steps <= src_T &&
                  store_step >= -1 && store_step < steps,
              FSN_ERR_SHAPE, "sb_carry_lstm_tc: bad shape B=%d F=%d src_T=%d steps=%d store_step=%d", B, F, src_T, steps,
              store_step);
  FSN_REQUIRE(act >= FSN_ACT_NONE && act <= FSN_ACT_RELU6, FSN_ERR_SHAPE, "sb_carry_lstm_tc: activation %d", act);
  FSN_REQUIRE(sb_tc_shape_ok(H, (2 * Ns + 1) + (2 * Nf + 1)), FSN_ERR_UNSUPPORTED,
              "sb_carry_lstm_tc: unsupported hidden size %d / input width %d", H, (2 * Ns + 1) + (2 * Nf + 1));
  cudaStream_t st = (cudaStream_t)stream;
  int rc = sb_tc_pack_raw(sb, H, (2 * Ns + 1) + (2 * Nf + 1), 2, packed, st, x3 != 0);
  if (rc) return rc;
  SbTcArgs a;
  memset(&a, 0, sizeof(a));
  a.packed = packed; a.magT = magT; a.fbT = fbT; a.unit_scale = unit_scale; a.crm = crm;
  a.B = B; a.F = F; a.Tp = src_T; a.Ns = Ns; a.Nf = Nf; a.H = H; a.act = act; a.steps = steps; a.x3 = x3 != 0;
  a.map = RowMap{B, F, F, 1};
  const size_t R = (size_t)B * F;
  const SbCarry io{h, c, (size_t)H, R * H, 1, restart, store_step, (size_t)steps * 2 * F, 0};
  return sb_tc_carry_forward(a, io, st);
}
```

### fullsubnet_b200/csrc/fsn_tc_ptx.cuh

```cuda
#pragma once
#include <cuda_fp16.h>
#include <stdint.h>
#include <stdio.h>

namespace fsn {
namespace ptx {

__device__ __forceinline__ uint32_t smem_u32(const void* p) { return (uint32_t)__cvta_generic_to_shared(p); }

__device__ __forceinline__ uint32_t cluster_ctarank() {
  uint32_t r;
  asm volatile("mov.u32 %0, %%cluster_ctarank;" : "=r"(r));
  return r;
}
__device__ __forceinline__ uint32_t mapa(uint32_t addr, uint32_t rank) {
  uint32_t r;
  asm volatile("mapa.shared::cluster.u32 %0, %1, %2;" : "=r"(r) : "r"(addr), "r"(rank));
  return r;
}
__device__ __forceinline__ void cluster_sync_all() {
  asm volatile("barrier.cluster.arrive.release.aligned;\n\tbarrier.cluster.wait.acquire.aligned;" ::: "memory");
}
__device__ __forceinline__ bool elect_one() {
  uint32_t pred;
// ... 4 lines not shown
      : "=r"(pred));
  return pred != 0;
}

__device__ __forceinline__ void mbar_init(uint64_t* bar, uint32_t count) {
  asm volatile("mbarrier.init.shared::cta.b64 [%0], %1;" ::"r"(smem_u32(bar)), "r"(count));
}
__device__ __forceinline__ void mbar_expect_tx(uint64_t* bar, uint32_t bytes) {
  asm volatile("mbarrier.arrive.expect_tx.shared::cta.b64 _, [%0], %1;" ::"r"(smem_u32(bar)), "r"(bytes) : "memory");
}
__device__ __forceinline__ void mbar_arrive_cluster(uint64_t* bar, uint32_t rank) {
  asm volatile("mbarrier.arrive.release.cluster.shared::cluster.b64 _, [%0];" ::"r"(mapa(smem_u32(bar), rank))
               : "memory");
}
__device__ __forceinline__ void mbar_arrive_cluster_relaxed(uint64_t* bar, uint32_t rank) {
  asm volatile("mbarrier.arrive.relaxed.cluster.shared::cluster.b64 _, [%0];" ::"r"(mapa(smem_u32(bar), rank))
               : "memory");
}
__device__ __forceinline__ void fence_release_cluster() { asm volatile("fence.acq_rel.cluster;" ::: "memory"); }
__device__ __forceinline__ bool mbar_try_wait(uint64_t* bar, uint32_t parity) {
  uint32_t ok;
  asm volatile(
      "{\n\t.reg .pred p;\n\t"
      "mbarrier.try_wait.parity.acquire.cluster.shared::cta.b64 p, [%1], %2;\n\t"
      "selp.b32 %0, 1, 0, p;\n\t}"
      : "=r"(ok)
      : "r"(smem_u32(bar)), "r"(parity)
      : "memory");
  return ok != 0;
}
__device__ __forceinline__ bool mbar_test_wait(uint64_t* bar, uint32_t parity) {
  uint32_t ok;
  asm volatile(
      "{\n\t.reg .pred p;\n\t"
      "mbarrier.test_wait.parity.acquire.cluster.shared::cta.b64 p, [%1], %2;\n\t"
      "selp.b32 %0, 1, 0, p;\n\t}"
      : "=r"(ok)
      : "r"(smem_u32(bar)), "r"(parity)
      : "memory");
  return ok != 0;
}
template <bool RELAXED>
__device__ __forceinline__ void mbar_wait(uint64_t* bar, uint32_t parity) {
  uint32_t spins = 0;
  while (!mbar_try_wait(bar, parity)) {
    if (RELAXED) __nanosleep(64);
    if (++spins > (RELAXED ? (1u << 24) : (1u << 27))) asm volatile("trap;");
  }
}

__device__ __forceinline__ void mbar_wait_mma(uint64_t* bar, uint32_t parity) {
  uint32_t spins = 0;
  while (!mbar_try_wait(bar, parity))
    if (++spins > (1u << 27)) asm volatile("trap;");
}

__device__ __forceinline__ bool mbar_try_wait_cta(uint64_t* bar, uint32_t parity) {
  uint32_t ok;
  asm volatile(
      "{\n\t.reg .pred p;\n\t"
      "mbarrier.try_wait.parity.acquire.cta.shared::cta.b64 p, [%1], %2;\n\t"
      "selp.b32 %0, 1, 0, p;\n\t}"
      : "=r"(ok)
      : "r"(smem_u32(bar)), "r"(parity)
      : "memory");
  return ok != 0;
}
template <bool SLEEP>
__device__ __forceinline__ void mbar_wait_cta(uint64_t* bar, uint32_t parity) {
  uint32_t spins = 0;
  while (!mbar_try_wait_cta(bar, parity)) {
    if (SLEEP) __nanosleep(64);
    if (++spins > (SLEEP ? (1u << 24) : (1u << 27))) asm volatile("trap;");
  }
}
__device__ __forceinline__ void mbar_wait_cta_warp(uint32_t bar, uint32_t parity) {
  asm volatile(
      "{\n\t.reg .pred p;\n\t.reg .b32 n;\n\t"
      "mov.b32 n, 0;\n"
      "WAIT:\n\t"
      "mbarrier.try_wait.parity.acquire.cta.shared::cta.b64 p, [%0], %1;\n\t"
      "vote.sync.all.pred p, p, 0xffffffff;\n\t"
      "@p bra.uni DONE;\n\t"
      "add.u32 n, n, 1;\n\t"
      "setp.gt.u32 p, n, 134217728;\n\t"
      "@p trap;\n\t"
      "bra.uni WAIT;\n"
      "DONE:\n\t}"
      ::"r"(bar), "r"(parity)
      : "memory");
}
__device__ __forceinline__ void mbar_arrive_elect_if(uint32_t bar, uint32_t pred) {
  asm volatile(
      "{\n\t.reg .pred e, p;\n\t"
      "elect.sync _|e, 0xffffffff;\n\t"
      "setp.ne.and.b32 p, %1, 0, e;\n\t"
      "@p mbarrier.arrive.shared::cta.b64 _, [%0];\n\t}"
      ::"r"(bar), "r"(pred)
      : "memory");
}
__device__ __forceinline__ void mbar_arrive_remote_elect_if(uint32_t bar, uint32_t rank, uint32_t pred) {
  asm volatile(
      "{\n\t.reg .pred e, p;\n\t.reg .b32 r;\n\t"
      "elect.sync _|e, 0xffffffff;\n\t"
      "setp.ne.and.b32 p, %2, 0, e;\n\t"
      "@p mapa.shared::cluster.u32 r, %0, %1;\n\t"
      "@p mbarrier.arrive.shared::cluster.b64 _, [r];\n\t}"
      ::"r"(bar), "r"(rank), "r"(pred)
      : "memory");
}
__device__ __forceinline__ void fence_proxy_async_smem() { asm volatile("fence.proxy.async.shared::cta;" ::: "memory"); }
__device__ __forceinline__ void mbar_arrive_remote(uint64_t* bar, uint32_t rank) {
  asm volatile("mbarrier.arrive.shared::cluster.b64 _, [%0];" ::"r"(mapa(smem_u32(bar), rank)) : "memory");
}
__device__ __forceinline__ void mbar_arrive_expect_tx_remote(uint64_t* bar, uint32_t rank, uint32_t bytes) {
  asm volatile("mbarrier.arrive.expect_tx.shared::cluster.b64 _, [%0], %1;" ::"r"(mapa(smem_u32(bar), rank)), "r"(bytes)
               : "memory");
}
__device__ __forceinline__ void bulk_s2s_remote(const void* src, uint32_t bytes, uint64_t* bar, uint32_t rank) {
  const uint32_t s = smem_u32(src);
  asm volatile("cp.async.bulk.shared::cluster.shared::cta.mbarrier::complete_tx::bytes [%0], [%1], %2, [%3];" ::"r"(
                   mapa(s, rank)),
               "r"(s), "r"(bytes), "r"(mapa(smem_u32(bar), rank))
               : "memory");
}
__device__ __forceinline__ void st_remote_f32(float* p, uint32_t rank, float v) {
  asm volatile("st.shared::cluster.f32 [%0], %1;" ::"r"(mapa(smem_u32(p), rank)), "f"(v) : "memory");
}
__device__ __forceinline__ void named_sync(uint32_t id, uint32_t count) {
  asm volatile("bar.sync %0, %1;" ::"r"(id), "r"(count) : "memory");
}

__device__ __forceinline__ void bulk_g2s(void* dst, const void* src, uint32_t bytes, uint64_t* bar) {
  asm volatile("cp.async.bulk.shared::cluster.global.mbarrier::complete_tx::bytes [%0], [%1], %2, [%3];" ::"r"(
                   smem_u32(dst)),
               "l"(src), "r"(bytes), "r"(smem_u32(bar))
               : "memory");
}
__device__ __forceinline__ void bulk_g2s_mc(void* dst, const void* src, uint32_t bytes, uint64_t* bar, uint16_t mask) {
  asm volatile(
      "cp.async.bulk.shared::cluster.global.mbarrier::complete_tx::bytes.multicast::cluster [%0], [%1], %2, [%3], %4;" ::"r"(
          smem_u32(dst)),
      "l"(src), "r"(bytes), "r"(smem_u32(bar)), "h"(mask)
      : "memory");
}
__device__ __forceinline__ void tma_load_2d(void* dst, const void* tmap, int c0, int c1, uint64_t* bar) {
  asm volatile(
      "cp.async.bulk.tensor.2d.shared::cluster.global.mbarrier::complete_tx::bytes [%0], [%1, {%2, %3}], [%4];" ::"r"(
          smem_u32(dst)),
      "l"(tmap), "r"(c0), "r"(c1), "r"(smem_u32(bar))
      : "memory");
}
__device__ __forceinline__ void fence_proxy_async() { asm volatile("fence.proxy.async;" ::: "memory"); }

__device__ __forceinline__ void mbar_arrive(uint64_t* bar) {
  asm volatile("mbarrier.arrive.shared::cta.b64 _, [%0];" ::"r"(smem_u32(bar)) : "memory");
}
__host__ __device__ __forceinline__ int swz128_off(int row, int k) {
  return (row >> 3) * 1024 + (row & 7) * 128 + ((((k >> 3) ^ (row & 7)) & 7) << 4) + (k & 7) * 2;
}
__host__ __device__ __forceinline__ int swz64_off(int row, int k) {
  return (row >> 3) * 512 + (row & 7) * 64 + ((((k >> 3) ^ ((row >> 1) & 3)) & 3) << 4) + (k & 7) * 2;
}

__device__ __forceinline__ float fast_sigmoid(float x) { return __fdividef(1.0f, 1.0f + __expf(-x)); }
__device__ __forceinline__ float fast_tanh(float x) { return 1.0f - __fdividef(2.0f, 1.0f + __expf(2.0f * x)); }

}
}
```

### fullsubnet_b200/csrc/fsn_wgmma.cuh

```cuda
#pragma once
#include <stdint.h>

namespace fsn {
namespace wg {

__device__ __forceinline__ void fence() { asm volatile("wgmma.fence.sync.aligned;" ::: "memory"); }
__device__ __forceinline__ void commit() { asm volatile("wgmma.commit_group.sync.aligned;" ::: "memory"); }
template <int N>
__device__ __forceinline__ void wait() { asm volatile("wgmma.wait_group.sync.aligned %0;" ::"n"(N) : "memory"); }
template <int R>
__device__ __forceinline__ void fence_operand(float (&d)[R]) {
#pragma unroll
  for (int i = 0; i < R; ++i) asm volatile("" : "+f"(d[i])::"memory");
}

__device__ __forceinline__ uint64_t desc_sw128(uint32_t saddr) {
  return (uint64_t)((saddr >> 4) & 0x3FFF) | (1ull << 16) | (64ull << 32) | (1ull << 62);
}
__device__ __forceinline__ uint64_t desc_sw64(uint32_t saddr) {
  return (uint64_t)((saddr >> 4) & 0x3FFF) | (1ull << 16) | (32ull << 32) | (2ull << 62);
}

__device__ __forceinline__ void mma_f16_n16(float (&d)[8], uint64_t a, uint64_t b, uint32_t scale_d) {
  asm volatile(
      "{\n\t.reg .pred p;\n\tsetp.ne.b32 p, %10, 0;\n\t"
      "wgmma.mma_async.sync.aligned.m64n16k16.f32.f16.f16 {%0,%1,%2,%3,%4,%5,%6,%7}, %8, %9, p, 1, 1, 0, 0;\n\t}"
      : "+f"(d[0]), "+f"(d[1]), "+f"(d[2]), "+f"(d[3]), "+f"(d[4]), "+f"(d[5]), "+f"(d[6]), "+f"(d[7])
      : "l"(a), "l"(b), "r"(scale_d)
      : "memory");
}

__device__ __forceinline__ void mma_f16_n32(float (&d)[16], uint64_t a, uint64_t b, uint32_t scale_d) {
  asm volatile(
      "{\n\t.reg .pred p;\n\tsetp.ne.b32 p, %18, 0;\n\t"
      "wgmma.mma_async.sync.aligned.m64n32k16.f32.f16.f16 {%0,%1,%2,%3,%4,%5,%6,%7,%8,%9,%10,%11,%12,%13,%14,%15}, %16, %17, p, 1, 1, 0, 0;\n\t}"
      : "+f"(d[0]), "+f"(d[1]), "+f"(d[2]), "+f"(d[3]), "+f"(d[4]), "+f"(d[5]), "+f"(d[6]), "+f"(d[7]), "+f"(d[8]), "+f"(d[9]), "+f"(d[10]), "+f"(d[11]), "+f"(d[12]), "+f"(d[13]), "+f"(d[14]), "+f"(d[15])
      : "l"(a), "l"(b), "r"(scale_d)
      : "memory");
}

constexpr uint32_t DESC_SW128_HI = 64u | (1u << 30), DESC_SW64_HI = 32u | (2u << 30);
__device__ __forceinline__ uint32_t desc_lo(uint32_t saddr) { return ((saddr >> 4) & 0x3FFF) | (1u << 16); }

__device__ __forceinline__ void mma_f16_n32_w(float (&d)[16], uint32_t a_lo, uint32_t a_off, uint32_t a_hi,
                                              uint32_t b_lo, uint32_t b_off, uint32_t b_hi) {
  asm volatile(
      "{\n\t.reg .b32 al, bl;\n\t.reg .b64 a, b;\n\t"
      "add.u32 al, %16, %17;\n\tadd.u32 bl, %19, %20;\n\t"
      "mov.b64 a, {al, %18};\n\tmov.b64 b, {bl, %21};\n\t"
      "wgmma.mma_async.sync.aligned.m64n32k16.f32.f16.f16 {%0,%1,%2,%3,%4,%5,%6,%7,%8,%9,%10,%11,%12,%13,%14,%15}, a, b, 1, 1, 1, 0, 0;\n\t}"
      : "+f"(d[0]), "+f"(d[1]), "+f"(d[2]), "+f"(d[3]), "+f"(d[4]), "+f"(d[5]), "+f"(d[6]), "+f"(d[7]), "+f"(d[8]), "+f"(d[9]), "+f"(d[10]), "+f"(d[11]), "+f"(d[12]), "+f"(d[13]), "+f"(d[14]), "+f"(d[15])
      : "r"(a_lo), "r"(a_off), "r"(a_hi), "r"(b_lo), "r"(b_off), "r"(b_hi)
      : "memory");
}

__device__ __forceinline__ void mma_f16_n64(float (&d)[32], uint64_t a, uint64_t b, uint32_t scale_d) {
  asm volatile(
      "{\n\t.reg .pred p;\n\tsetp.ne.b32 p, %34, 0;\n\t"
      "wgmma.mma_async.sync.aligned.m64n64k16.f32.f16.f16 {%0,%1,%2,%3,%4,%5,%6,%7,%8,%9,%10,%11,%12,%13,%14,%15,%16,%17,%18,%19,%20,%21,%22,%23,%24,%25,%26,%27,%28,%29,%30,%31}, %32, %33, p, 1, 1, 0, 0;\n\t}"
      : "+f"(d[0]), "+f"(d[1]), "+f"(d[2]), "+f"(d[3]), "+f"(d[4]), "+f"(d[5]), "+f"(d[6]), "+f"(d[7]), "+f"(d[8]), "+f"(d[9]), "+f"(d[10]), "+f"(d[11]), "+f"(d[12]), "+f"(d[13]), "+f"(d[14]), "+f"(d[15]), "+f"(d[16]), "+f"(d[17]), "+f"(d[18]), "+f"(d[19]), "+f"(d[20]), "+f"(d[21]), "+f"(d[22]), "+f"(d[23]), "+f"(d[24]), "+f"(d[25]), "+f"(d[26]), "+f"(d[27]), "+f"(d[28]), "+f"(d[29]), "+f"(d[30]), "+f"(d[31])
      : "l"(a), "l"(b), "r"(scale_d)
      : "memory");
}

__device__ __forceinline__ void mma_f16_n128(float (&d)[64], uint64_t a, uint64_t b, uint32_t scale_d) {
  asm volatile(
      "{\n\t.reg .pred p;\n\tsetp.ne.b32 p, %66, 0;\n\t"
      "wgmma.mma_async.sync.aligned.m64n128k16.f32.f16.f16 {%0,%1,%2,%3,%4,%5,%6,%7,%8,%9,%10,%11,%12,%13,%14,%15,%16,%17,%18,%19,%20,%21,%22,%23,%24,%25,%26,%27,%28,%29,%30,%31,%32,%33,%34,%35,%36,%37,%38,%39,%40,%41,%42,%43,%44,%45,%46,%47,%48,%49,%50,%51,%52,%53,%54,%55,%56,%57,%58,%59,%60,%61,%62,%63}, %64, %65, p, 1, 1, 0, 0;\n\t}"
      : "+f"(d[0]), "+f"(d[1]), "+f"(d[2]), "+f"(d[3]), "+f"(d[4]), "+f"(d[5]), "+f"(d[6]), "+f"(d[7]), "+f"(d[8]), "+f"(d[9]), "+f"(d[10]), "+f"(d[11]), "+f"(d[12]), "+f"(d[13]), "+f"(d[14]), "+f"(d[15]), "+f"(d[16]), "+f"(d[17]), "+f"(d[18]), "+f"(d[19]), "+f"(d[20]), "+f"(d[21]), "+f"(d[22]), "+f"(d[23]), "+f"(d[24]), "+f"(d[25]), "+f"(d[26]), "+f"(d[27]), "+f"(d[28]), "+f"(d[29]), "+f"(d[30]), "+f"(d[31]), "+f"(d[32]), "+f"(d[33]), "+f"(d[34]), "+f"(d[35]), "+f"(d[36]), "+f"(d[37]), "+f"(d[38]), "+f"(d[39]), "+f"(d[40]), "+f"(d[41]), "+f"(d[42]), "+f"(d[43]), "+f"(d[44]), "+f"(d[45]), "+f"(d[46]), "+f"(d[47]), "+f"(d[48]), "+f"(d[49]), "+f"(d[50]), "+f"(d[51]), "+f"(d[52]), "+f"(d[53]), "+f"(d[54]), "+f"(d[55]), "+f"(d[56]), "+f"(d[57]), "+f"(d[58]), "+f"(d[59]), "+f"(d[60]), "+f"(d[61]), "+f"(d[62]), "+f"(d[63])
      : "l"(a), "l"(b), "r"(scale_d)
      : "memory");
}

__device__ __forceinline__ void mma_tf32_n128(float (&d)[64], uint64_t a, uint64_t b, uint32_t scale_d) {
  asm volatile(
      "{\n\t.reg .pred p;\n\tsetp.ne.b32 p, %66, 0;\n\t"
      "wgmma.mma_async.sync.aligned.m64n128k8.f32.tf32.tf32 {%0,%1,%2,%3,%4,%5,%6,%7,%8,%9,%10,%11,%12,%13,%14,%15,%16,%17,%18,%19,%20,%21,%22,%23,%24,%25,%26,%27,%28,%29,%30,%31,%32,%33,%34,%35,%36,%37,%38,%39,%40,%41,%42,%43,%44,%45,%46,%47,%48,%49,%50,%51,%52,%53,%54,%55,%56,%57,%58,%59,%60,%61,%62,%63}, %64, %65, p, 1, 1;\n\t}"
      : "+f"(d[0]), "+f"(d[1]), "+f"(d[2]), "+f"(d[3]), "+f"(d[4]), "+f"(d[5]), "+f"(d[6]), "+f"(d[7]), "+f"(d[8]), "+f"(d[9]), "+f"(d[10]), "+f"(d[11]), "+f"(d[12]), "+f"(d[13]), "+f"(d[14]), "+f"(d[15]), "+f"(d[16]), "+f"(d[17]), "+f"(d[18]), "+f"(d[19]), "+f"(d[20]), "+f"(d[21]), "+f"(d[22]), "+f"(d[23]), "+f"(d[24]), "+f"(d[25]), "+f"(d[26]), "+f"(d[27]), "+f"(d[28]), "+f"(d[29]), "+f"(d[30]), "+f"(d[31]), "+f"(d[32]), "+f"(d[33]), "+f"(d[34]), "+f"(d[35]), "+f"(d[36]), "+f"(d[37]), "+f"(d[38]), "+f"(d[39]), "+f"(d[40]), "+f"(d[41]), "+f"(d[42]), "+f"(d[43]), "+f"(d[44]), "+f"(d[45]), "+f"(d[46]), "+f"(d[47]), "+f"(d[48]), "+f"(d[49]), "+f"(d[50]), "+f"(d[51]), "+f"(d[52]), "+f"(d[53]), "+f"(d[54]), "+f"(d[55]), "+f"(d[56]), "+f"(d[57]), "+f"(d[58]), "+f"(d[59]), "+f"(d[60]), "+f"(d[61]), "+f"(d[62]), "+f"(d[63])
      : "l"(a), "l"(b), "r"(scale_d)
      : "memory");
}

__device__ __forceinline__ void mma_tf32_n256(float (&d)[128], uint64_t a, uint64_t b, uint32_t scale_d) {
  asm volatile(
      "{\n\t.reg .pred p;\n\tsetp.ne.b32 p, %130, 0;\n\t"
      "wgmma.mma_async.sync.aligned.m64n256k8.f32.tf32.tf32 {%0,%1,%2,%3,%4,%5,%6,%7,%8,%9,%10,%11,%12,%13,%14,%15,%16,%17,%18,%19,%20,%21,%22,%23,%24,%25,%26,%27,%28,%29,%30,%31,%32,%33,%34,%35,%36,%37,%38,%39,%40,%41,%42,%43,%44,%45,%46,%47,%48,%49,%50,%51,%52,%53,%54,%55,%56,%57,%58,%59,%60,%61,%62,%63,%64,%65,%66,%67,%68,%69,%70,%71,%72,%73,%74,%75,%76,%77,%78,%79,%80,%81,%82,%83,%84,%85,%86,%87,%88,%89,%90,%91,%92,%93,%94,%95,%96,%97,%98,%99,%100,%101,%102,%103,%104,%105,%106,%107,%108,%109,%110,%111,%112,%113,%114,%115,%116,%117,%118,%119,%120,%121,%122,%123,%124,%125,%126,%127}, %128, %129, p, 1, 1;\n\t}"
      : "+f"(d[0]), "+f"(d[1]), "+f"(d[2]), "+f"(d[3]), "+f"(d[4]), "+f"(d[5]), "+f"(d[6]), "+f"(d[7]), "+f"(d[8]), "+f"(d[9]), "+f"(d[10]), "+f"(d[11]), "+f"(d[12]), "+f"(d[13]), "+f"(d[14]), "+f"(d[15]), "+f"(d[16]), "+f"(d[17]), "+f"(d[18]), "+f"(d[19]), "+f"(d[20]), "+f"(d[21]), "+f"(d[22]), "+f"(d[23]), "+f"(d[24]), "+f"(d[25]), "+f"(d[26]), "+f"(d[27]), "+f"(d[28]), "+f"(d[29]), "+f"(d[30]), "+f"(d[31]), "+f"(d[32]), "+f"(d[33]), "+f"(d[34]), "+f"(d[35]), "+f"(d[36]), "+f"(d[37]), "+f"(d[38]), "+f"(d[39]), "+f"(d[40]), "+f"(d[41]), "+f"(d[42]), "+f"(d[43]), "+f"(d[44]), "+f"(d[45]), "+f"(d[46]), "+f"(d[47]), "+f"(d[48]), "+f"(d[49]), "+f"(d[50]), "+f"(d[51]), "+f"(d[52]), "+f"(d[53]), "+f"(d[54]), "+f"(d[55]), "+f"(d[56]), "+f"(d[57]), "+f"(d[58]), "+f"(d[59]), "+f"(d[60]), "+f"(d[61]), "+f"(d[62]), "+f"(d[63]), "+f"(d[64]), "+f"(d[65]), "+f"(d[66]), "+f"(d[67]), "+f"(d[68]), "+f"(d[69]), "+f"(d[70]), "+f"(d[71]), "+f"(d[72]), "+f"(d[73]), "+f"(d[74]), "+f"(d[75]), "+f"(d[76]), "+f"(d[77]), "+f"(d[78]), "+f"(d[79]), "+f"(d[80]), "+f"(d[81]), "+f"(d[82]), "+f"(d[83]), "+f"(d[84]), "+f"(d[85]), "+f"(d[86]), "+f"(d[87]), "+f"(d[88]), "+f"(d[89]), "+f"(d[90]), "+f"(d[91]), "+f"(d[92]), "+f"(d[93]), "+f"(d[94]), "+f"(d[95]), "+f"(d[96]), "+f"(d[97]), "+f"(d[98]), "+f"(d[99]), "+f"(d[100]), "+f"(d[101]), "+f"(d[102]), "+f"(d[103]), "+f"(d[104]), "+f"(d[105]), "+f"(d[106]), "+f"(d[107]), "+f"(d[108]), "+f"(d[109]), "+f"(d[110]), "+f"(d[111]), "+f"(d[112]), "+f"(d[113]), "+f"(d[114]), "+f"(d[115]), "+f"(d[116]), "+f"(d[117]), "+f"(d[118]), "+f"(d[119]), "+f"(d[120]), "+f"(d[121]), "+f"(d[122]), "+f"(d[123]), "+f"(d[124]), "+f"(d[125]), "+f"(d[126]), "+f"(d[127])
      : "l"(a), "l"(b), "r"(scale_d)
      : "memory");
}

}
}
```

### include/fsn_b200.h

```cpp
#ifndef FSN_B200_H
#define FSN_B200_H

#include <stddef.h>
#include <stdint.h>

#ifdef __cplusplus
extern "C" {
#endif

typedef void* fsn_stream_t;

enum {
  FSN_OK = 0,
  FSN_ERR_SHAPE = 1,
  FSN_ERR_UNSUPPORTED = 2,
  FSN_ERR_CUDA = 3,
  FSN_ERR_WORKSPACE = 4
};

enum { FSN_ACT_NONE = 0, FSN_ACT_RELU = 1, FSN_ACT_TANH = 2, FSN_ACT_RELU6 = 3 };
enum { FSN_NORM_OFFLINE_LAPLACE = 0, FSN_NORM_CUMULATIVE_LAPLACE = 1, FSN_NORM_FORGETTING = 4 };
enum { FSN_CELL_LSTM = 0, FSN_CELL_GRU = 1 };
enum { FSN_PREC_FP32 = 0, FSN_PREC_F16_TC = 1, FSN_PREC_TF32_TC = 2, FSN_PREC_F16X3_TC = 3 };

// ... 186 lines not shown
int fsn_clip_adam(const fsn_param_list* L, float max_norm, float grad_scale, float lr, float beta1, float beta2,
                  float eps, int step, float* norm_out, void* scratch, size_t scratch_bytes, fsn_stream_t stream);
int fsn_clip_adam_steps(const fsn_param_list* L, float max_norm, float grad_scale, float lr, float beta1, float beta2,
                        float eps, const int* steps, float* norm_out, void* scratch, size_t scratch_bytes,
                        fsn_stream_t stream);

typedef struct fsn_fullband_desc {
  int32_t num_freqs;
  int32_t hidden;
  int32_t num_layers;
  int32_t look_ahead;
  int32_t activation;
  int32_t norm_type;
  int32_t precision;
  int32_t cell_type;
} fsn_fullband_desc;

size_t fsn_fullband_workspace_bytes(const fsn_fullband_desc* d, int B, int T);
int fsn_fullband_forward(const fsn_fullband_desc* d, const fsn_lstm_layer* layers, const float* fc_w, const float* fc_b,
                         const float* noisy_mag, int B, int T, float* out, void* workspace, size_t workspace_bytes,
                         fsn_stream_t stream);
size_t fsn_fullband_enhance_workspace_bytes(const fsn_fullband_desc* d, int B, int L_max, int n_fft, int hop);
int fsn_fullband_enhance(const fsn_fullband_desc* d, const fsn_lstm_layer* layers, const float* fc_w, const float* fc_b,
                         const float* wav, const int32_t* lengths, int B, int L_max, int n_fft, int hop, int win_length,
                         float* enhanced, float* crm_out, int16_t* pcm, float gain, void* workspace,
                         size_t workspace_bytes, fsn_stream_t stream);

size_t fsn_fullband_stream_state_bytes(const fsn_fullband_desc* d, int B, int n_fft, int hop);
size_t fsn_fullband_stream_workspace_bytes(const fsn_fullband_desc* d, int B, int K_max, int n_fft, int hop);
int fsn_fullband_stream_delay(const fsn_fullband_desc* d, int n_fft, int hop);
int fsn_fullband_stream_step(const fsn_fullband_desc* d, const fsn_lstm_layer* layers, const float* fc_w,
                             const float* fc_b, const float* wav, const int32_t* start, const int32_t* tail, int B, int K,
                             int n_fft, int hop, int win_length, float* enhanced, void* state, size_t state_bytes,
                             void* workspace, size_t workspace_bytes, fsn_stream_t stream);

size_t fsn_fast_stream_state_bytes(const fsn_fast_desc* d, int B, int n_fft, int hop);
size_t fsn_fast_stream_workspace_bytes(const fsn_fast_desc* d, int B, int K_max, int n_fft, int hop);
int fsn_fast_stream_delay(const fsn_fast_desc* d, int n_fft, int hop);
int fsn_fast_stream_step(const fsn_fast_desc* d, const fsn_fast_weights* w, const float* wav, const int32_t* start,
                         const int32_t* tail, int B, int K, int n_fft, int hop, int win_length, float* enhanced,
                         void* state, size_t state_bytes, void* workspace, size_t workspace_bytes, fsn_stream_t stream);

size_t fsn_fast_stream_tc_state_bytes(const fsn_fast_desc* d, int B, int n_fft, int hop);
size_t fsn_fast_stream_tc_workspace_bytes(const fsn_fast_desc* d, int B, int K_max, int n_fft, int hop);
int fsn_fast_stream_tc_delay(const fsn_fast_desc* d, int n_fft, int hop);
int fsn_fast_stream_tc_step(const fsn_fast_desc* d, const fsn_fast_weights* w, const float* wav, const int32_t* start,
                            const int32_t* tail, int B, int K, int n_fft, int hop, int win_length, float* enhanced,
                            void* state, size_t state_bytes, void* workspace, size_t workspace_bytes, fsn_stream_t stream);

size_t fsn_stream_state_bytes(const fsn_model_desc* d, int B, int n_fft, int hop);
size_t fsn_stream_workspace_bytes(const fsn_model_desc* d, int B, int K_max, int n_fft, int hop);
int fsn_stream_delay(const fsn_model_desc* d, int n_fft, int hop);
int fsn_stream_step(const fsn_model_desc* d, const fsn_seq_weights* fb, const fsn_seq_weights* sb, const float* wav,
                    const int32_t* start, const int32_t* tail, int B, int K, int n_fft, int hop, int win_length,
                    float* enhanced, void* state, size_t state_bytes, void* workspace, size_t workspace_bytes,
                    fsn_stream_t stream);

size_t fsn_stream_tc_state_bytes(const fsn_model_desc* d, int B, int n_fft, int hop);
size_t fsn_stream_tc_workspace_bytes(const fsn_model_desc* d, int B, int K_max, int n_fft, int hop);
int fsn_stream_tc_delay(const fsn_model_desc* d, int n_fft, int hop);
int fsn_stream_tc_step(const fsn_model_desc* d, const fsn_seq_weights* fb, const fsn_seq_weights* sb,
                       const void* sb_packed, const float* wav, const int32_t* start, const int32_t* tail, int B, int K,
                       int n_fft, int hop, int win_length, float* enhanced, void* state, size_t state_bytes,
                       void* workspace, size_t workspace_bytes, fsn_stream_t stream);

typedef struct fsn_fullband_grads {
  fsn_lstm_grads layer[8];
  float *fc_w, *fc_b;
} fsn_fullband_grads;
size_t fsn_fullband_train_workspace_bytes(const fsn_fullband_desc* d, int B, int T);
int fsn_fullband_train_forward(const fsn_fullband_desc* d, const fsn_lstm_layer* layers, const float* fc_w,
                               const float* fc_b, const float* noisy_mag, int B, int T, float* out, void* workspace,
                               size_t workspace_bytes, fsn_stream_t stream);
int fsn_fullband_train_backward(const fsn_fullband_desc* d, const fsn_lstm_layer* layers, const float* fc_w,
                                const float* fc_b, const float* dout, int B, int T, const fsn_fullband_grads* g,
                                void* workspace, size_t workspace_bytes, fsn_stream_t stream);

typedef struct fsn_improved_grads {
  fsn_seq_grads fb;
  fsn_seq_grads sb[FSN_IMP_MAX_SECTIONS];
} fsn_improved_grads;
size_t fsn_improved_train_workspace_bytes(const fsn_improved_desc* d, int B, int L);
int fsn_improved_train_forward(const fsn_improved_desc* d, const fsn_improved_weights* w, const float* wav, int B, int L,
                               float* enhanced, void* workspace, size_t workspace_bytes, fsn_stream_t stream);
int fsn_improved_train_backward(const fsn_improved_desc* d, const fsn_improved_weights* w, const float* d_enhanced, int B,
                                int L, const fsn_improved_grads* g, void* workspace, size_t workspace_bytes,
                                fsn_stream_t stream);

int fsn_peak_normalize_int16(const float* wav, int B, int L, float gain, int16_t* out, fsn_stream_t stream);

int fsn_si_sdr(const float* reference, const float* estimation, int B, int L, float* out, fsn_stream_t stream);
int fsn_si_sdr_lengths(const float* reference, const float* estimation, const int32_t* lengths, int B, int L_max,
                       float* out, fsn_stream_t stream);

size_t fsn_stoi_workspace_bytes(int B, int L_max, int sr);
int fsn_stoi(const float* clean, const float* estimate, const int32_t* lengths, int B, int L_max, int sr, float* out,
             void* workspace, size_t workspace_bytes, fsn_stream_t stream);

int fsn_rir_convolve(const float* x, const float* rir, const int* rir_len, int B, int L, int Lr_max, float* out,
                     fsn_stream_t stream);
int fsn_snr_mix(const float* clean, const float* noise, const float* snr, const float* noisy_target_dB_FS,
                float target_dB_FS, float eps, int B, int L, float* noisy_out, float* clean_out, fsn_stream_t stream);

int fsn_debug_row_to_unit(int B, int F, int G, int r, int* b, int* f);
int fsn_debug_unit_to_row(int B, int F, int G, int b, int f);
int fsn_debug_reflect_count(int r, int F, int N);

int fsn_debug_tgemm(const float* A, int64_t lda, const float* B, int64_t ldb, float* C, int64_t ldc, int M, int N,
                    int K, int accumulate, float* scratch, int64_t scratch_floats, fsn_stream_t stream);

int fsn_debug_tgemm_blocked(const float* A, const float* B, float* C, int M, int N, int K, int a_k0, int b_k0,
                            float* scratch, int64_t scratch_floats, fsn_stream_t stream);

int fsn_debug_lstm_fwd_step(const float* h_prev, const float* w_hh, const float* x, const float* w_ih, int K0, float* G,
                            const float* b_ih, const float* b_hh, const float* c_prev, float* c_out, float* h_out, int R,
                            int H, int half, void* scratch, int64_t scratch_bytes, fsn_stream_t stream);

int fsn_debug_fc_gemm(const float* A, const float* W, const float* bias, float* out, int M, int K, int O, int act,
                      int w_kmajor, fsn_stream_t stream);
int fsn_debug_sgemm(int ta, const float* A, int64_t lda, const float* B, int64_t ldb, float* C, int64_t ldc, int M, int N,
                    int K, int accumulate, float* scratch, int64_t scratch_floats, fsn_stream_t stream);
int fsn_debug_colsum(const float* X, int64_t rows, int cols, int64_t ldx, float* out, float* out2, float* scratch,
                     int64_t scratch_floats, fsn_stream_t stream);
int fsn_debug_small_out_wgrad(const float* dout, const float* Hm, int64_t rows, int H, float* dW, float* scratch,
                              int64_t scratch_floats, fsn_stream_t stream);
int fsn_debug_transpose(const float* in, int64_t rows, int cols, float* out, fsn_stream_t stream);
int fsn_debug_transpose_blocked(const float* in, int64_t K, int M, int64_t ld, float* out, float* colsum_part,
                                int max_slabs, int* slabs, float* bias_out, fsn_stream_t stream);
int fsn_debug_gemm_tc(const float* x, int64_t ldx, int K, const float* row_scale, int rows_per_scale, int scale_B,
                      const float* W, int N, const float* bias, int act, int x3, float* out, int64_t ldo, int64_t rows,
                      void* workspace, size_t workspace_bytes, fsn_stream_t stream);

size_t fsn_debug_lstm_tc_workspace_bytes(int R, int T, int K, int H, int x3);
int fsn_debug_lstm_layer_tc(const float* w_ih, const float* w_hh, const float* b_ih, const float* b_hh, const float* x,
                            int R, int T, int K, int H, int x3, float* hall, void* workspace, size_t workspace_bytes,
                            fsn_stream_t stream);
int fsn_debug_linear_tc(const float* x, int rows, int K, const float* W, const float* bias, int N, int act, int x3,
                        float* out, void* workspace, size_t workspace_bytes, fsn_stream_t stream);
int fsn_debug_lstm_tc_carry(const float* w_ih, const float* w_hh, const float* b_ih, const float* b_hh, const float* x,
                            int R, int T, int K, int H, int x3, const float* h_init, float* c, const int32_t* restart,
                            int fin_step, float* hall, void* workspace, size_t workspace_bytes, fsn_stream_t stream);
size_t fsn_debug_lstm_rec_tc_scratch_bytes(int H, int x3);
int fsn_debug_lstm_rec_tc(const float* w_hh, const float* b_ih, const float* b_hh, const float* P, int64_t p_row, int64_t p_t,
                          float* hall, int64_t h_row, int64_t h_t, int R, int T, int H, int x3, const float* h_init,
                          const float* c_init, float* c_fin, int64_t c_row, const int32_t* restart, int fin_step, int* info,
                          void* scratch, size_t scratch_bytes, fsn_stream_t stream);

size_t fsn_debug_sb_lstm_tc_packed_bytes(int H, int x3);
int fsn_debug_sb_lstm_tc_max_clusters(int H, int x3, int stages, int cluster, int* clusters);
int fsn_debug_sb_lstm_tc(const fsn_seq_weights* sb, int H, int Ns, int Nf, int fc_out, int act, int x3,
                         const float* magT, const float* fbT, int B, int F, int src_T, int G,
                         const float* inv2, const float* unit_scale, int la, int steps, int shrink,
                         int stages, int cluster, void* packed, float* crm, fsn_stream_t stream);
int fsn_debug_sb_lstm_tc_carry(const fsn_seq_weights* sb, int H, int Ns, int Nf, int act, int x3, const float* magT,
                               const float* fbT, int B, int F, int src_T, const float* unit_scale, int steps,
                               const int32_t* restart, int store_step, float* h, float* c, void* packed, float* crm,
                               fsn_stream_t stream);
int fsn_debug_sb_lstm_tc_phased(const fsn_seq_weights* bn, int H, int Ns, int Nf, int x3, const float* catM,
                                const float* catE, int B, int M, int S, int St, const int32_t* m0, const float* scale,
                                const int32_t* restart, const int32_t* store, float* h, float* c, void* packed, float* x,
                                float* out, fsn_stream_t stream);
#define FSN_SB_PROBE_FIELDS 16
#define FSN_SB_PROBE_SLOTS 4
int fsn_debug_sb_lstm_tc_probe(const fsn_seq_weights* sb, int H, int Ns, int Nf, int fc_out, int act, int x3,
                               const float* magT, const float* fbT, int B, int F, int src_T, int G,
                               const float* inv2, const float* unit_scale, int la, int steps, int shrink,
                               int stages, int cluster, void* packed, float* crm, long long* stamps, int stamp_ctas,
                               int stamp_steps, fsn_stream_t stream);

size_t fsn_debug_lstm_train_workspace_bytes(int n_layers, int R, int T, int K0, int H, int precision);
int fsn_debug_lstm_train(const fsn_lstm_layer* layers, int n_layers, int R, int T, int K0, int H, int precision,
                         const float* x, const float* dh_top, const float* dout, const float* fc_w, int O, float* h_top,
                         float* dx, const fsn_lstm_grads* g, float* trace, void* workspace, size_t workspace_bytes,
                         fsn_stream_t stream);

enum { FSN_SEQ_PATH_TC = 0, FSN_SEQ_PATH_PERSISTENT = 1, FSN_SEQ_PATH_STEP2 = 2, FSN_SEQ_PATH_ONE_LAYER = 3 };
size_t fsn_debug_seq_stack_workspace_bytes(int n, const int* H, int R, int Tp, int K0, int gru, int step_scale, int tc, int x3,
                                           int O);
int fsn_debug_seq_stack(const fsn_lstm_layer* layers, int n, const int* H, int R, int Tp, int K0, int gru, int step_scale,
                        int tc, int x3, int force_stepwise, const float* x, const float* scale, const float* fc_w,
                        const float* fc_b, int O, int act, float* out, void* workspace, size_t workspace_bytes, int* path,
                        fsn_stream_t stream);

int fsn_debug_stft(const float* wav, int B, int L, int n_fft, int hop, int win_length, const int32_t* lengths, int* lens_dev,
                   float* mag, float* phase, float* real, float* imag, float* magT, int T_pad, fsn_stream_t stream);
int fsn_debug_istft(const float* real, const float* imag, int cstride, const float* crm, int mask_mode, int B, int T,
                    int n_fft, int hop, int win_length, int length, const int32_t* lengths, int* lens_dev, float* wav,
                    unsigned int* peak_bits, int16_t* pcm, float gain, float* crm_out, fsn_stream_t stream);
int fsn_debug_istft_mask_adjoint(const float* dwav, const float* real, const float* imag, int B, int L, int T, int n_fft,
                                 int hop, int win_length, float* dcrm, fsn_stream_t stream);
int fsn_debug_wav_epilogue(const float* enhanced, const unsigned int* peak_bits, int B, int L, const int32_t* lengths,
                           int* lens_dev, float gain, int16_t* pcm, float* crm_out, int F, int T, int hop,
                           fsn_stream_t stream);

int fsn_debug_norm_unfold_bwd(const float* dX, const float* X, const float* fbz, const float* scale, int cum, int B, int F,
                              int G, int Tp, int Ns, float cnt2, int act, float* mid, float* dz, fsn_stream_t stream);
int fsn_debug_fast_norm_unfold_bwd(const float* ddec, const float* dX, const float* X, const float* encT,
                                   const float* bn_out, const float* scale, int cum, int B, int Tp, int M, int Nn, int Ne,
                                   int S, float cnt2, float* mid, float* denc, float* dbn, fsn_stream_t stream);
int fsn_debug_imp_unfold_bwd(const float* dX, const float* Xn, const float* invs, const float* y, int B, int T, int Fu,
                             int lo, int hi, int cs, int ns, int cf, int nf, int first, int act, float* dot, float* dfb,
                             fsn_stream_t stream);
int fsn_debug_imp_section_input(const float* magc, const float* fbT, int B, int T, int Fu, int lo, int hi, int cs, int ns,
                                int cf, int nf, int tm, float* X, float* fs, fsn_stream_t stream);
int fsn_debug_cum_clip_scale(const float* x, int B, int Tp, int F, int64_t bs, int64_t ts, float eps, float* fs,
                             float* scale1T, fsn_stream_t stream);
int fsn_debug_cum_unit_scale(const float* magT, const float* fbT, int B, int F, int G, int Tp, int Ns, int Nf, float eps,
                             int time_major, float* scaleT, fsn_stream_t stream);
int fsn_debug_forget_unit_broadcast(const float* scaleT, int B, int F, int G, int Tp, float* unit_scale, fsn_stream_t stream);
int fsn_debug_fast_bn(const float* melT, const float* encT, int64_t bs, int64_t ts, int B, int Tp, int M, int Nn, int Ne,
                      int S, int cum, float eps, float* bn, float* fs, float* sums, float* scale, fsn_stream_t stream);
int fsn_debug_fast_dec_input(const float* encT, const float* bn_out, int64_t nbs, int64_t nms, int64_t nts, int B, int Tp,
                             int M, int S, int Ts, int64_t rbs, int64_t rts, float* dec_in, fsn_stream_t stream);
int fsn_debug_transpose_mag(const float* in, int B, int F, int T, int Tp, int64_t bs, int64_t ts, float* out,
                            const float* scale, float* scaled, fsn_stream_t stream);
int fsn_debug_crm_output(const float* y, int64_t bs, int64_t ts, int B, int Tp, int F, int la, float* out,
                         fsn_stream_t stream);
int fsn_debug_scale_rows(const float* in, const float* scale, int64_t n, int cols, int rows, int div, float* out,
                         fsn_stream_t stream);
int fsn_debug_imp_compress(const float* mag, int B, int F, int T, float fdrc, int tm, float* out, fsn_stream_t stream);
int fsn_debug_train_gather(const float* raw, const float* fbz, const float* inv2, const float* unit_scale, int B, int F, int G,
                           int Tp, int Ns, int Nf, float* X, fsn_stream_t stream);
int fsn_debug_sb_head(const float* h, int R, int H, int steps, const float* W, const float* bias, int O, int act, int N,
                      int c, int lo, int rows, int64_t rs, int64_t bs, int t0, float* out, fsn_stream_t stream);
int fsn_debug_sb_head_bwd(const float* dcrm, const float* y, int act, int R, int O, int steps, int la, int N, int c, int lo,
                          int rows, int64_t rs, int64_t bs, float* dY, fsn_stream_t stream);
int fsn_debug_train_dy(const float* dout, const float* y, int act, int B, int F, int T, int Tp, int la, float* dY,
                       fsn_stream_t stream);

size_t fsn_debug_imp_section_lstm_tc_workspace_bytes(int R, int T, int W, int H, int x3);
int fsn_debug_imp_section_lstm_tc(const fsn_seq_weights* sw, int W, int H, int x3, const float* X, int R, int T, int stages,
                                  int cluster, void* packed, float* h1, void* workspace, size_t workspace_bytes,
                                  fsn_stream_t stream);

int fsn_debug_norm_stats(const float* x, int B, int T_pad, int F, int N, int64_t bs, int64_t ts, const int32_t* lengths,
                         int* lens_dev, int hop, int la, const float* fb_sums, float cnt1, float cnt2, float eps, float* fs,
                         float* sums, float* inv1, float* inv2, fsn_stream_t stream);
int fsn_debug_train_stats(const float* x, int tm, int B, int F, int T, int N, float* sums, fsn_stream_t stream);

int fsn_debug_forgetting_scale(const float* x, int N, const float* x2, int N2, int B, int T_pad, int F, int64_t bs,
                               int64_t ts, float cnt, const int32_t* lengths, int* lens_dev, int hop, int la, float* fs,
                               float* fs2, float* scale, float* mu, fsn_stream_t stream);
int fsn_debug_forgetting_bwd(const float* dX, const float* X, const float* fbz, const float* scale, int B, int F, int G,
                             int Tp, int Ns, int act, float* mid, float* dz, fsn_stream_t stream);

int fsn_debug_stoi_stages(const float* clean, const float* estimate, const int32_t* lengths, int B, int L_max, int sr,
                          double* resampled, int32_t* keep, int32_t* n_kept, double* compacted, double* bands, float* out,
                          void* workspace, size_t workspace_bytes, fsn_stream_t stream);

#ifdef __cplusplus
}
#endif
#endif
```

Measured before the change: 127,300.

## Split sub-band LSTM into per-layer two-pass kernels with global h0 staging

Replaces the fused two-layer sub-band LSTM tensor-core kernel with two separate kernels run in chunks of row pairs. Layer 0 writes its hidden states for every timestep to a global workspace, and layer 1 streams them back with bulk async copies. Tiles now cover 48 rows using m64n48 wgmma with 2-CTA clusters. This is meant to shrink shared memory and register pressure per kernel and raise the row count per CTA, at the cost of extra global traffic and more kernel launches.

```diff
diff --git a/fullsubnet_b200/_lib.py b/fullsubnet_b200/_lib.py
--- a/fullsubnet_b200/_lib.py
+++ b/fullsubnet_b200/_lib.py
@@ -205,6 +205,9 @@
     "fsn_debug_sb_lstm_tc_max_clusters": (C.c_int, [_I, _I, _I, _I, C.POINTER(C.c_int)]),
     "fsn_debug_sb_lstm_tc": (C.c_int, [C.POINTER(SeqWeights), _I, _I, _I, _I, _I, _I, _P, _P, _I, _I, _I, _I, _P, _P, _I,
                                        _I, _I, _I, _I, _P, _P, _P]),
+    "fsn_debug_sb_lstm_tc2_ws_bytes": (_S, [_I, _I, _I, _I, _I]),
+    "fsn_debug_sb_lstm_tc2": (C.c_int, [C.POINTER(SeqWeights), _I, _I, _I, _I, _I, _P, _P, _I, _I, _I, _I, _P, _P, _I, _I,
+                                        _I, _I, _P, _P, _P, _P]),
     "fsn_debug_sb_lstm_tc_carry": (C.c_int, [C.POINTER(SeqWeights), _I, _I, _I, _I, _I, _P, _P, _I, _I, _I, _P, _I, _P,
                                              _I, _P, _P, _P, _P, _P]),
     "fsn_debug_sb_lstm_tc_phased": (C.c_int, [C.POINTER(SeqWeights), _I, _I, _I, _I, _P, _P, _I, _I, _I, _I, _P, _P, _P,
diff --git a/fullsubnet_b200/csrc/fsn_internal.cuh b/fullsubnet_b200/csrc/fsn_internal.cuh
--- a/fullsubnet_b200/csrc/fsn_internal.cuh
+++ b/fullsubnet_b200/csrc/fsn_internal.cuh
@@ -402,7 +402,10 @@
   int stages, cluster;
   long long* stamps;
   int stamp_ctas, stamp_its;
-};
+  void* h0ws;
+  int split_chunk;
+};
+size_t sb_tc_split_ws_bytes(int R, int Tp, int H, bool x3, int chunk_pairs = 0);
 size_t sb_tc_packed_bytes(const fsn_model_desc* d);
 size_t sb_tc_packed_bytes_raw(int H, bool x3, bool proj = false);
 int sb_tc_pack(const fsn_model_desc* d, const fsn_seq_weights* sb, void* packed, cudaStream_t st);
diff --git a/fullsubnet_b200/csrc/fsn_model.cu b/fullsubnet_b200/csrc/fsn_model.cu
--- a/fullsubnet_b200/csrc/fsn_model.cu
+++ b/fullsubnet_b200/csrc/fsn_model.cu
@@ -36,6 +36,7 @@
   float2* fs2;
   SeqStackWs fb;
   float *sb_h0[2], *sb_h1[2], *sb_c0, *sb_c1;
+  void* sb_h0ws;
   size_t bytes;
 };
 
@@ -94,6 +95,9 @@
     w.sb_c0 = c.take<float>(RH);
     w.sb_c1 = c.take<float>(RH);
   }
+  w.sb_h0ws = nullptr;
+  if (d->precision == FSN_PREC_F16_TC || d->precision == FSN_PREC_F16X3_TC)
+    w.sb_h0ws = c.take<uint8_t>(sb_tc_split_ws_bytes(m.R, m.Tp, d->sb_hidden, d->precision == FSN_PREC_F16X3_TC));
   w.cum1 = w.cum2 = nullptr;
   w.fs2 = nullptr;
   if (norm_per_step(d->norm_type)) {
@@ -147,6 +151,7 @@
     a.B = B; a.F = F; a.Tp = Tp; a.la = d->look_ahead; a.Ns = d->sb_num_neighbors; a.Nf = d->fb_num_neighbors;
     a.H = Hs; a.act = d->sb_activation; a.map = map; a.x3 = d->precision == FSN_PREC_F16X3_TC;
     a.unit_scale = (cum || fgt) ? w.cum2 : nullptr;
+    a.h0ws = w.sb_h0ws;
     rc = sb_tc_forward(a, st);
     prof_mark(3, st);
     return rc;
diff --git a/fullsubnet_b200/csrc/fsn_subband_tc.cu b/fullsubnet_b200/csrc/fsn_subband_tc.cu
--- a/fullsubnet_b200/csrc/fsn_subband_tc.cu
+++ b/fullsubnet_b200/csrc/fsn_subband_tc.cu
@@ -1,4 +1,6 @@
 #include <cuda_fp16.h>
+
+#include <algorithm>
 #include <stdlib.h>
 #include <string.h>
 
@@ -200,6 +202,13 @@
 }
 template <bool X3> __device__ __forceinline__ float sg(float x) { return X3 ? 1.0f / (1.0f + expf(-x)) : fast_sigmoid(x); }
 template <bool X3> __device__ __forceinline__ float th(float x) { return X3 ? 1.0f - 2.0f / (1.0f + expf(2.0f * x)) : fast_tanh(x); }
+template <bool X3>
+__device__ __forceinline__ float lstm_cell(float ai, float af, float ag, float ao, const float (&b)[4], float cp,
+                                           float& h) {
+  const float cn = sg<X3>(af + b[1]) * cp + sg<X3>(ai + b[0]) * th<X3>(ag + b[2]);
+  h = sg<X3>(ao + b[3]) * th<X3>(cn);
+  return cn;
+}
 
 __device__ __forceinline__ void release_stage(uint32_t bar, uint32_t pred, uint32_t local, uint32_t remote,
                                               uint32_t rank) {
@@ -604,7 +613,7 @@
           for (int hh = 0; hh < 2; ++hh) {
             const int u = s * US + 16 * q + (lane >> 2) + 8 * hh;
             const float* bl = bias_g + (layer ? 4 * H : 0);
-            const float bi = bl[u], bff = bl[H + u], bg = bl[2 * H + u], bo = bl[3 * H + u];
+            const float b4[4] = {bl[u], bl[H + u], bl[2 * H + u], bl[3 * H + u]};
             const float w0 = fcw[u], w1 = fcw[H + u];
 #pragma unroll
             for (int j = 0; j < 4; ++j)
@@ -616,9 +625,9 @@
                 if constexpr (CARRY) {
                   if (rows[8 * j + 2 * (lane & 3) + e].restart == t) cp = 0.f;
                 }
-                const float cn = sg<X3>(acc[1][ri] + bff) * cp + sg<X3>(acc[0][ri] + bi) * th<X3>(acc[2][ri] + bg);
+                float h;
+                const float cn = lstm_cell<X3>(acc[0][ri], acc[1][ri], acc[2][ri], acc[3][ri], b4, cp, h);
                 if (layer) c1[ci] = cn; else c0[ci] = cn;
-                const float h = sg<X3>(acc[3][ri] + bo) * th<X3>(cn);
                 __half hi = __float2half_rn(h);
                 __half lo = __float2half_rn(h - __half2float(hi));
                 if constexpr (CARRY) {
@@ -735,6 +744,423 @@
   sb_lstm_tc_body<X3, false, false, true, true>(a);
 }
 
+constexpr int NB2 = 48;
+constexpr int S_KBLK2 = NB2 * KB * 2;
+constexpr int X_BLK2 = NB2 * KS * 2;
+constexpr int SPLIT_CHUNK_PAIRS = 132;
+
+__host__ __device__ inline Smem smem_plan2(int H, int stages, bool x3, int layer) {
+  Smem s;
+  const int nkh = H / KB;
+  uint32_t o = 0;
+  s.w = o; o += stages * W_TILE;
+  s.x = o; o += layer ? 0 : 2 * X_BLK2;
+  s.h0 = o; o += (layer ? 1 : 2) * nkh * S_KBLK2;
+  s.h1 = o; o += layer ? nkh * S_KBLK2 : 0;
+  s.lo = o; o += x3 ? (o - s.x) : 0;
+  s.fcw = o; o += layer ? 4 * MAX_MT * 2 * NB2 * 4 : 0;
+  s.fcp = o; o += layer ? 2 * 2 * NB2 * 4 : 0;
+  s.outst = o; o += layer ? NB2 * 2 * OUT_T * 4 : 0;
+  s.rows = o; o += NB2 * 16;
+  s.bars = o; o += 256;
+  s.total = o;
+  return s;
+}
+
+struct Bars2 {
+  uint64_t w_full[MAX_STAGES], w_empty[MAX_STAGES];
+  uint64_t x_full[2], x_empty[2];
+  uint64_t h_ready[2], h_empty[2];
+  uint64_t h0_full, h0_free;
+  uint64_t l1_done, fc_done;
+  uint64_t fcp_full[2], fcp_empty[2];
+  uint64_t turn[MAX_MT];
+};
+static_assert(sizeof(Bars2) <= 256, "barrier block too large");
+
+struct SplitArgs {
+  KArgs k;
+  uint8_t* h0ws;
+  int row_base;
+};
+
+template <bool X3, int LAYER>
+__device__ __forceinline__ void sb_split_body(const SplitArgs& sa) {
+  constexpr int PARTS = X3 ? 2 : 1;
+  constexpr int NJ = NB2 / 8;
+  const KArgs& a = sa.k;
+  extern __shared__ uint8_t smem_raw[];
+  uint8_t* smem = smem_raw + ((1024u - (smem_u32(smem_raw) & 1023u)) & 1023u);
+  const int H = a.H;
+  const int MT = H / 128;
+  const int nkh = H / KB;
+  const int STAGES = a.stages;
+  const uint32_t cl_rank = cluster_ctarank();
+  const int half = (int)(cl_rank & 1u);
+  const uint32_t peer = cl_rank ^ 1u;
+  const Smem sp = smem_plan2(H, STAGES, X3, LAYER);
+  const uint32_t LO = sp.lo - sp.x;
+  const PackedLayout PL = packed_layout(H, X3);
+  Bars2& bars = *reinterpret_cast<Bars2*>(smem + sp.bars);
+  RowInfo* rows = reinterpret_cast<RowInfo*>(smem + sp.rows);
+  float* fc_part = reinterpret_cast<float*>(smem + sp.fcw);
+  float* fcp = reinterpret_cast<float*>(smem + sp.fcp);
+  float* outst = reinterpret_cast<float*>(smem + sp.outst);
+  const int warp = threadIdx.x >> 5, lane = threadIdx.x & 31;
+  const int pair = blockIdx.x >> 1;
+  const int row0 = sa.row_base + pair * NB2;
+  const int Tp = a.Tp;
+  const uint32_t img = PARTS * nkh * S_KBLK2;
+  uint8_t* ws_pair = sa.h0ws + (size_t)pair * Tp * img;
+
+  if (threadIdx.x == 0) {
+    for (int s = 0; s < STAGES; ++s) { mbar_init(&bars.w_full[s], 1); mbar_init(&bars.w_empty[s], 1); }
+    for (int i = 0; i < 2; ++i) {
+      mbar_init(&bars.x_full[i], 1); mbar_init(&bars.x_empty[i], 4 * MT);
+      mbar_init(&bars.h_ready[i], 5 * MT);
+      mbar_init(&bars.h_empty[i], MT);
+      mbar_init(&bars.fcp_full[i], 1); mbar_init(&bars.fcp_empty[i], 1);
+    }
+    mbar_init(&bars.h0_full, 1);
+    mbar_init(&bars.h0_free, 4 * MT);
+    mbar_init(&bars.fc_done, 1);
+    mbar_init(&bars.l1_done, 4 * MT);
+    for (int m = 0; m < MAX_MT; ++m) mbar_init(&bars.turn[m], 4);
+    asm volatile("fence.mbarrier_init.release.cluster;" ::: "memory");
+  }
+  if (threadIdx.x < NB2) {
+    RowInfo ri;
+    const int r = row0 + threadIdx.x;
+    ri.src_b = -1; ri.src_f = 0; ri.scale = 0.f; ri.out_idx = 0;
+    if (r < a.R) {
+      row_to_unit(a.map, r, ri.src_b, ri.src_f);
+      ri.scale = a.inv2[ri.src_b];
+      const int bq = r / a.Fsub, fq = r - bq * a.Fsub;
+      ri.out_idx = bq * 2 * a.Fsub + fq;
+    }
+    rows[threadIdx.x] = ri;
+  }
+  {
+    uint4* z = reinterpret_cast<uint4*>(smem + sp.x);
+    const int n16 = (sp.fcw - sp.x) / 16;
+    for (int i = threadIdx.x; i < n16; i += blockDim.x) z[i] = make_uint4(0, 0, 0, 0);
+  }
+  fence_proxy_async_smem();
+  __syncthreads();
+  cluster_sync_all();
+
+  constexpr int REG0 = (LAYER == 1 && X3) ? 32 : 56, REG1 = (LAYER == 1 && X3) ? 160 : 152;
+  if (warp < 4) {
+    asm volatile("setmaxnreg.dec.sync.aligned.u32 %0;" ::"n"(REG0));
+    if (warp == 0) {
+      const uint8_t* stream = a.packed + ((size_t)half * (PL.tiles0 + PL.tiles1) + (LAYER ? PL.tiles0 : 0)) * W_TILE;
+      const size_t tiles = LAYER ? PL.tiles1 : PL.tiles0;
+      uint32_t stage = 0, phase = 0;
+      for (int t = 0; t < Tp; ++t) {
+        const uint8_t* src = stream;
+        for (size_t tile = 0; tile < tiles; ++tile, src += W_TILE) {
+          mbar_wait_cta<false>(&bars.w_empty[stage], phase ^ 1);
+          if (elect_one()) {
+            mbar_expect_tx(&bars.w_full[stage], W_TILE);
+            bulk_g2s(smem + sp.w + stage * W_TILE, src, W_TILE, &bars.w_full[stage]);
+          }
+          __syncwarp();
+          if (++stage == (uint32_t)STAGES) { stage = 0; phase ^= 1; }
+        }
+      }
+    } else if (LAYER == 0 && warp == 2) {
+      const int nmag = 2 * a.Ns + 1;
+      for (int t = 0; t < Tp; ++t) {
+        mbar_wait_cta<true>(&bars.x_empty[t & 1], ((t >> 1) & 1) ^ 1);
+        uint8_t* xb = smem + sp.x + (t & 1) * X_BLK2;
+#pragma unroll 4
+        for (int n = 0; n < NB2; ++n) {
+          const RowInfo ri = rows[n];
+          float v = 0.f;
+          if (ri.src_b >= 0 && lane < a.Ksb) {
+            const int col = (lane < nmag) ? reflect_idx(ri.src_f + lane - a.Ns, a.F)
+                                          : reflect_idx(ri.src_f + (lane - nmag) - a.Nf, a.F);
+            const float* src = (lane < nmag) ? a.magT : a.fbT;
+            v = src[((size_t)ri.src_b * a.src_T + t) * a.F + col];
+            v *= a.unit_scale ? a.unit_scale[(size_t)t * a.R + row0 + n] : ri.scale;
+          }
+          const __half hi = __float2half_rn(v);
+          *reinterpret_cast<__half*>(xb + swz64_off(n, lane)) = hi;
+          if (X3) *reinterpret_cast<__half*>(xb + LO + swz64_off(n, lane)) = __float2half_rn(v - __half2float(hi));
+        }
+        fence_proxy_async_smem();
+        __syncwarp();
+        if (lane == 0) mbar_arrive(&bars.x_full[t & 1]);
+      }
+    } else if (LAYER == 1 && warp == 2) {
+      for (int t = 0; t < Tp; ++t) {
+        if (t > 0) mbar_wait_cta<false>(&bars.h0_free, (t - 1) & 1);
+        if (elect_one()) {
+          const uint8_t* src = ws_pair + (size_t)t * img;
+          mbar_expect_tx(&bars.h0_full, img);
+          bulk_g2s(smem + sp.h0, src, nkh * S_KBLK2, &bars.h0_full);
+          if (X3) bulk_g2s(smem + sp.h0 + LO, src + nkh * S_KBLK2, nkh * S_KBLK2, &bars.h0_full);
+        }
+        __syncwarp();
+      }
+    } else if (LAYER == 1 && warp == 3) {
+      const float fcb0 = half ? 0.f : reinterpret_cast<const float*>(a.packed + PL.off_fcb)[0];
+      const float fcb1 = half ? 0.f : reinterpret_cast<const float*>(a.packed + PL.off_fcb)[1];
+      int staged = 0, t_stage0 = 0;
+      for (int t = 0; t < Tp; ++t) {
+        mbar_wait_cta<true>(&bars.h_ready[0], t & 1);
+        float s0[2], s1[2];
+#pragma unroll
+        for (int k = 0; k < 2; ++k) {
+          const int n = lane + 32 * k;
+          s0[k] = fcb0; s1[k] = fcb1;
+          if (t >= a.la && n < NB2) {
+            for (int w = 0; w < 4 * MT; ++w) {
+              s0[k] += fc_part[(w * 2 + 0) * NB2 + n];
+              s1[k] += fc_part[(w * 2 + 1) * NB2 + n];
+            }
+          }
+        }
+        __syncwarp();
+        if (lane == 0) mbar_arrive(&bars.fc_done);
+        if (t < a.la) continue;
+        const int u = t - a.la, b = u & 1;
+        float* pb = fcp + b * 2 * NB2;
+        if (half) {
+          mbar_wait<true>(&bars.fcp_empty[b], ((u >> 1) & 1) ^ 1);
+#pragma unroll
+          for (int k = 0; k < 2; ++k) {
+            const int n = lane + 32 * k;
+            if (n < NB2) { st_remote_f32(pb + n, peer, s0[k]); st_remote_f32(pb + NB2 + n, peer, s1[k]); }
+          }
+          __syncwarp();
+          if (lane == 0) mbar_arrive_cluster(&bars.fcp_full[b], peer);
+          continue;
+        }
+        mbar_wait<true>(&bars.fcp_full[b], (u >> 1) & 1);
+#pragma unroll
+        for (int k = 0; k < 2; ++k) {
+          const int n = lane + 32 * k;
+          if (n < NB2) { s0[k] += pb[n]; s1[k] += pb[NB2 + n]; }
+        }
+        __syncwarp();
+        if (lane == 0) mbar_arrive_cluster(&bars.fcp_empty[b], peer);
+        if (staged == 0) t_stage0 = u;
+#pragma unroll
+        for (int k = 0; k < 2; ++k) {
+          const int n = lane + 32 * k;
+          if (n < NB2) {
+            outst[(n * 2 + 0) * OUT_T + staged] = act_apply(s0[k], a.act);
+            outst[(n * 2 + 1) * OUT_T + staged] = act_apply(s1[k], a.act);
+          }
+        }
+        ++staged;
+        if (staged == OUT_T || t == Tp - 1) {
+#pragma unroll
+          for (int k = 0; k < 2; ++k) {
+            const int n = lane + 32 * k;
+            if (n >= NB2) continue;
+            const RowInfo ri = rows[n];
+            if (ri.src_b < 0) continue;
+#pragma unroll
+            for (int o = 0; o < 2; ++o) {
+              float* dst = a.crm + ((size_t)ri.out_idx + (size_t)o * a.Fsub) * a.T + t_stage0;
+              for (int i = 0; i < staged; ++i) dst[i] = outst[(n * 2 + o) * OUT_T + i];
+            }
+          }
+          staged = 0;
+        }
+      }
+    }
+  } else {
+    asm volatile("setmaxnreg.inc.sync.aligned.u32 %0;" ::"n"(REG1));
+    const int m = __shfl_sync(0xffffffffu, (warp - 4) >> 2, 0);
+    const int q = __shfl_sync(0xffffffffu, warp & 3, 0);
+    const int s = half * MT + m;
+    if (m < MT) {
+      const float* bias_g = reinterpret_cast<const float*>(a.packed + PL.off_bias) + (LAYER ? 4 * H : 0);
+      const float* fcw = reinterpret_cast<const float*>(a.packed + PL.off_fcw);
+      float* my_part = fc_part + (size_t)(warp - 4) * 2 * NB2;
+      float c[4 * NJ];
+#pragma unroll
+      for (int i = 0; i < 4 * NJ; ++i) c[i] = 0.f;
+      const uint32_t a_lo0 = wg::desc_lo(smem_u32(smem + sp.w));
+      const uint32_t w_full0 = smem_u32(&bars.w_full[0]), w_empty0 = smem_u32(&bars.w_empty[0]);
+      const uint32_t turn_next = smem_u32(&bars.turn[m + 1 < MT ? m + 1 : 0]);
+      const uint32_t rel_local = q == 0;
+      const int nkb = LAYER ? PL.nkb1 : PL.nkb0;
+      const size_t tiles = LAYER ? PL.tiles1 : PL.tiles0;
+      int h_seen = 0, turns = 0;
+      for (int t = 0; t < Tp; ++t) {
+        if (LAYER == 0) {
+          mbar_wait_cta<false>(&bars.x_full[t & 1], (t >> 1) & 1);
+          for (; h_seen < t; ++h_seen) mbar_wait_cta<false>(&bars.h_ready[h_seen & 1], (h_seen >> 1) & 1);
+        } else {
+          mbar_wait_cta<false>(&bars.h0_full, t & 1);
+        }
+        const uint32_t x_addr = smem_u32(smem + sp.x + (t & 1) * X_BLK2);
+        const uint32_t h0_cur = smem_u32(smem + sp.h0);
+        const uint32_t h0_prev = smem_u32(smem + sp.h0 + ((t + 1) & 1) * nkh * S_KBLK2);
+        const uint32_t h1_prev = smem_u32(smem + sp.h1);
+        const size_t first = (size_t)t * tiles + (size_t)m * nkb * PARTS;
+        float acc[4][4 * NJ];
+#pragma unroll
+        for (int g = 0; g < 4; ++g) {
+#pragma unroll
+          for (int i = 0; i < 4 * NJ; ++i) acc[g][i] = 0.f;
+          wg::fence_operand(acc[g]);
+        }
+        int prev_stage = -1;
+        if (m > 0 || t > 0) { mbar_wait_cta<false>(&bars.turn[m], turns & 1); ++turns; }
+        int stage = __shfl_sync(0xffffffffu, (int)(first % (size_t)STAGES), 0);
+        uint32_t wphase = __shfl_sync(0xffffffffu, (uint32_t)((first / (size_t)STAGES) & 1), 0);
+        auto issue_stage = [&](int part, uint32_t bd, uint32_t b_hi, uint32_t ends_block) {
+          mbar_wait_cta_warp(w_full0 + 8 * stage, wphase);
+          mbar_arrive_elect_if(turn_next, ends_block);
+          wg::fence();
+          const uint32_t ad = a_lo0 + stage * (W_TILE >> 4);
+#pragma unroll
+          for (int kk = 0; kk < 2; ++kk)
+#pragma unroll
+            for (int g = 0; g < 4; ++g) {
+              const uint32_t a_off = g * (W_SUB >> 4) + kk * 2;
+              wg::mma_f16_n48_w(acc[g], ad, a_off, wg::DESC_SW64_HI, bd, kk * 2, b_hi);
+              if (X3 && part == 0) wg::mma_f16_n48_w(acc[g], ad, a_off, wg::DESC_SW64_HI, bd, (LO >> 4) + kk * 2, b_hi);
+            }
+          wg::commit();
+          wg::wait<1>();
+          release_stage(w_empty0 + 8 * prev_stage, prev_stage >= 0, rel_local, 0u, 0u);
+          prev_stage = stage;
+          if (++stage == STAGES) { stage = 0; wphase ^= 1; }
+        };
+        if (LAYER == 0) {
+#pragma unroll
+          for (int part = 0; part < PARTS; ++part) issue_stage(part, wg::desc_lo(x_addr), wg::DESC_SW64_HI, 0u);
+        }
+        const int nseg = LAYER ? 2 : 1;
+        int seg = 0;
+        do {
+          if (LAYER == 1 && seg == 1)
+            for (; h_seen < t; ++h_seen) mbar_wait_cta<false>(&bars.h_ready[0], h_seen & 1);
+          uint32_t bd = wg::desc_lo(LAYER == 0 ? h0_prev : seg == 0 ? h0_cur : h1_prev);
+          int kb = 0;
+          do {
+            const uint32_t ends_block = seg == nseg - 1 && kb == nkh - 1;
+#pragma unroll
+            for (int part = 0; part < PARTS; ++part) issue_stage(part, bd, wg::DESC_SW128_HI, 0u);
+            if (LAYER == 1 && seg == 1 && kb == 0 && lane == 0) mbar_arrive(&bars.h0_free);
+#pragma unroll
+            for (int part = 0; part < PARTS; ++part)
+              issue_stage(part, bd + (64 >> 4), wg::DESC_SW128_HI, part == PARTS - 1 ? ends_block : 0u);
+            bd += S_KBLK2 >> 4;
+          } while (++kb < nkh);
+        } while (++seg < nseg);
+        wg::wait<0>();
+#pragma unroll
+        for (int g = 0; g < 4; ++g) wg::fence_operand(acc[g]);
+        release_stage(w_empty0 + 8 * prev_stage, 1u, rel_local, 0u, 0u);
+        if (lane == 0) mbar_arrive(LAYER ? &bars.l1_done : &bars.x_empty[t & 1]);
+        if (q == 2 && lane == 0) mbar_arrive_remote(&bars.h_empty[LAYER ? 0 : (t + 1) & 1], peer);
+        if (LAYER == 1 && t >= 1) mbar_wait_cta<false>(&bars.fc_done, (t - 1) & 1);
+        __half hv[2][2 * NJ], lv[2][2 * NJ];
+        uint8_t* hb = smem + (LAYER ? sp.h1 : sp.h0 + (t & 1) * nkh * S_KBLK2) + s * S_KBLK2;
+        float bias[2][4], fw[2][2];
+#pragma unroll
+        for (int hh = 0; hh < 2; ++hh) {
+          const int u = s * US + 16 * q + (lane >> 2) + 8 * hh;
+#pragma unroll
+          for (int g = 0; g < 4; ++g) bias[hh][g] = bias_g[g * H + u];
+          fw[hh][0] = LAYER ? fcw[u] : 0.f;
+          fw[hh][1] = LAYER ? fcw[H + u] : 0.f;
+        }
+#pragma unroll
+        for (int j = 0; j < NJ; ++j)
+#pragma unroll
+          for (int e = 0; e < 2; ++e) {
+            float f0 = 0.f, f1 = 0.f;
+#pragma unroll
+            for (int hh = 0; hh < 2; ++hh) {
+              const int ri = 4 * j + 2 * hh + e;
+              const int ci = hh * 2 * NJ + j * 2 + e;
+              float h;
+              c[ci] = lstm_cell<X3>(acc[0][ri], acc[1][ri], acc[2][ri], acc[3][ri], bias[hh], c[ci], h);
+              const __half hi = __float2half_rn(h);
+              hv[hh][j * 2 + e] = hi;
+              lv[hh][j * 2 + e] = __float2half_rn(h - __half2float(hi));
+              if (LAYER == 1) { f0 += h * fw[hh][0]; f1 += h * fw[hh][1]; }
+            }
+            if (LAYER == 1) {
+              f0 += __shfl_xor_sync(0xffffffffu, f0, 4);
+              f0 += __shfl_xor_sync(0xffffffffu, f0, 8);
+              f0 += __shfl_xor_sync(0xffffffffu, f0, 16);
+              f1 += __shfl_xor_sync(0xffffffffu, f1, 4);
+              f1 += __shfl_xor_sync(0xffffffffu, f1, 8);
+              f1 += __shfl_xor_sync(0xffffffffu, f1, 16);
+              if (lane < 4) {
+                my_part[8 * j + 2 * lane + e] = f0;
+                my_part[NB2 + 8 * j + 2 * lane + e] = f1;
+              }
+            }
+          }
+        if (LAYER == 1) {
+          mbar_wait_cta<false>(&bars.l1_done, t & 1);
+          mbar_wait_cta<false>(&bars.h_empty[0], t & 1);
+        } else if (t >= 1) {
+          mbar_wait_cta<false>(&bars.h_empty[t & 1], ((t - 1) >> 1) & 1);
+        }
+#pragma unroll
+        for (int hh = 0; hh < 2; ++hh) {
+          const int u = 16 * q + (lane >> 2) + 8 * hh;
+          uint8_t* ub = hb + (u & 7) * 2;
+          const int chunk = u >> 3;
+#pragma unroll
+          for (int j = 0; j < NJ; ++j)
+#pragma unroll
+            for (int e = 0; e < 2; ++e) {
+              const int n = 8 * j + 2 * (lane & 3) + e;
+              uint8_t* p = ub + (n >> 3) * 1024 + (n & 7) * 128 + ((chunk ^ (n & 7)) << 4);
+              *reinterpret_cast<__half*>(p) = hv[hh][j * 2 + e];
+              if (X3) *reinterpret_cast<__half*>(p + LO) = lv[hh][j * 2 + e];
+            }
+        }
+        fence_proxy_async_smem();
+        __syncwarp();
+        const bool exchange = LAYER == 1 || t < Tp - 1;
+        uint64_t* ready = &bars.h_ready[LAYER ? 0 : t & 1];
+        if (exchange && lane == 0) mbar_arrive(ready);
+        if (LAYER == 0 && q == 0 && lane == 0) bulk_wait_read_all();
+        named_sync(1 + m, 128);
+        if (q == 0 && lane == 0) {
+          if (exchange) {
+            mbar_arrive_expect_tx_remote(ready, peer, PARTS * S_KBLK2);
+            bulk_s2s_remote(hb, S_KBLK2, ready, peer);
+            if (X3) bulk_s2s_remote(hb + LO, S_KBLK2, ready, peer);
+          }
+          if (LAYER == 0) {
+            uint8_t* dst = ws_pair + (size_t)t * img + s * S_KBLK2;
+            bulk_s2g(dst, hb, S_KBLK2);
+            if (X3) bulk_s2g(dst + nkh * S_KBLK2, hb + LO, S_KBLK2);
+            bulk_commit();
+          }
+        }
+      }
+      if (LAYER == 0 && q == 0 && lane == 0) bulk_wait_all();
+    }
+  }
+
+  __syncthreads();
+  cluster_sync_all();
+}
+
+template <bool X3>
+__global__ void __launch_bounds__(NTHREADS, 1) sb_l0_tc_kernel(const __grid_constant__ SplitArgs a) {
+  sb_split_body<X3, 0>(a);
+}
+template <bool X3>
+__global__ void __launch_bounds__(NTHREADS, 1) sb_l1_tc_kernel(const __grid_constant__ SplitArgs a) {
+  sb_split_body<X3, 1>(a);
+}
+
 }
 
 static int sb_ksb(const fsn_model_desc* d) { return (2 * d->sb_num_neighbors + 1) + (2 * d->fb_num_neighbors + 1); }
@@ -827,7 +1253,59 @@
   return FSN_OK;
 }
 
+size_t sb_tc_split_ws_bytes(int R, int Tp, int H, bool x3, int chunk_pairs) {
+  if (!sb_tc_shape_ok(H, 0) || R <= 0 || Tp <= 0) return 0;
+  const int pairs = std::min(cdiv(R, tc::NB2), chunk_pairs > 0 ? chunk_pairs : tc::SPLIT_CHUNK_PAIRS);
+  return (size_t)pairs * Tp * (x3 ? 2 : 1) * (H / tc::KB) * tc::S_KBLK2;
+}
+
+template <bool X3>
+static int sb_split_launch(const tc::SplitArgs& sa, int pairs, int layer, cudaStream_t st) {
+  void (*kern)(tc::SplitArgs) = layer ? tc::sb_l1_tc_kernel<X3> : tc::sb_l0_tc_kernel<X3>;
+  const size_t smem = tc::smem_plan2(sa.k.H, sa.k.stages, X3, layer).total + 1024;
+  const char* name = layer ? "sb_l1_tc_kernel" : "sb_l0_tc_kernel";
+  int rc = check_cuda(cudaFuncSetAttribute((const void*)kern, cudaFuncAttributeMaxDynamicSharedMemorySize, (int)smem), name);
+  if (rc) return rc;
+  cudaLaunchConfig_t cfg;
+  cudaLaunchAttribute attr[1];
+  memset(&cfg, 0, sizeof(cfg));
+  cfg.gridDim = dim3(2 * pairs);
+  cfg.blockDim = dim3(128 + 128 * (sa.k.H / 128));
+  cfg.dynamicSmemBytes = smem;
+  cfg.stream = st;
+  attr[0].id = cudaLaunchAttributeClusterDimension;
+  attr[0].val.clusterDim.x = 2;
+  attr[0].val.clusterDim.y = 1;
+  attr[0].val.clusterDim.z = 1;
+  cfg.attrs = attr;
+  cfg.numAttrs = 1;
+  if ((rc = check_cuda(cudaLaunchKernelEx(&cfg, kern, sa), name))) return rc;
+  FSN_CHECK_LAUNCH(name);
+  return FSN_OK;
+}
+
+static int sb_tc_split_forward(const SbTcArgs& s, cudaStream_t st) {
+  FSN_REQUIRE(s.shrink <= 1, FSN_ERR_UNSUPPORTED, "sb_lstm_tc two-pass: no time down-sampling");
+  tc::SplitArgs sa;
+  memset(&sa, 0, sizeof(sa));
+  int rc = sb_tc_kargs(s, sa.k);
+  if (rc) return rc;
+  sa.k.cluster = 1;
+  sa.h0ws = (uint8_t*)s.h0ws;
+  const int total = cdiv(sa.k.R, tc::NB2);
+  const int chunk = s.split_chunk > 0 ? s.split_chunk : tc::SPLIT_CHUNK_PAIRS;
+  for (int p0 = 0; p0 < total; p0 += chunk) {
+    const int pairs = std::min(chunk, total - p0);
+    sa.row_base = p0 * tc::NB2;
+    for (int layer = 0; layer < 2; ++layer)
+      if ((rc = s.x3 ? sb_split_launch<true>(sa, pairs, layer, st) : sb_split_launch<false>(sa, pairs, layer, st)))
+        return rc;
+  }
+  return FSN_OK;
+}
+
 int sb_tc_forward(const SbTcArgs& s, cudaStream_t st) {
+  if (s.h0ws && !s.stamps) return sb_tc_split_forward(s, st);
   tc::KArgs a;
   int rc = sb_tc_kargs(s, a);
   if (rc) return rc;
@@ -984,6 +1462,44 @@
                          stages, cluster, packed, crm, nullptr, 0, 0, stream);
 }
 
+extern "C" size_t fsn_debug_sb_lstm_tc2_ws_bytes(int R, int steps, int H, int x3, int chunk_pairs) {
+  return fsn::sb_tc_split_ws_bytes(R, steps, H, x3 != 0, chunk_pairs);
+}
+
+extern "C" int fsn_debug_sb_lstm_tc2(const fsn_seq_weights* sb, int H, int Ns, int Nf, int act, int x3, const float* magT,
+                                     const float* fbT, int B, int F, int src_T, int G, const float* inv2,
+                                     const float* unit_scale, int la, int steps, int stages, int chunk_pairs, void* packed,
+                                     void* h0ws, float* crm, fsn_stream_t stream) {
+  using namespace fsn;
+  FSN_REQUIRE(stages == 0 || (stages >= 2 && stages <= tc::MAX_STAGES), FSN_ERR_UNSUPPORTED,
+              "sb_lstm_tc2: ring depth %d (0, 2, 3 or 4)", stages);
+  FSN_REQUIRE(sb && magT && fbT && inv2 && packed && h0ws && crm && chunk_pairs >= 0, FSN_ERR_SHAPE,
+              "sb_lstm_tc2: missing buffer");
+  FSN_REQUIRE(B > 0 && F > 1 && src_T > 0 && Ns >= 0 && Nf >= 0 && Ns < F && Nf < F && G >= 1, FSN_ERR_SHAPE,
+              "sb_lstm_tc2: bad shape B=%d F=%d src_T=%d Ns=%d Nf=%d", B, F, src_T, Ns, Nf);
+  FSN_REQUIRE(act >= FSN_ACT_NONE && act <= FSN_ACT_RELU6, FSN_ERR_SHAPE, "sb_lstm_tc2: activation %d", act);
+  const int g = (B > 1 && G > 1) ? G : 1;
+  FSN_REQUIRE(B == 1 || B > G, FSN_ERR_SHAPE, "sb_lstm_tc2: batch size %d <= num_groups %d", B, G);
+  const int Fsub = g > 1 ? F / g : F;
+  FSN_REQUIRE(Fsub > 0, FSN_ERR_SHAPE, "sb_lstm_tc2: num_freqs < num_groups");
+  FSN_REQUIRE(steps > 0 && steps <= src_T && la >= 0 && la < steps, FSN_ERR_SHAPE,
+              "sb_lstm_tc2: steps %d / look-ahead %d for %d source frames", steps, la, src_T);
+  FSN_REQUIRE(sb_tc_shape_ok(H, (2 * Ns + 1) + (2 * Nf + 1)), FSN_ERR_UNSUPPORTED,
+              "sb_lstm_tc2: unsupported hidden size %d / input width %d", H, (2 * Ns + 1) + (2 * Nf + 1));
+  cudaStream_t st = (cudaStream_t)stream;
+  int rc = sb_tc_pack_raw(sb, H, (2 * Ns + 1) + (2 * Nf + 1), 2, packed, st, x3 != 0);
+  if (rc) return rc;
+  SbTcArgs a;
+  memset(&a, 0, sizeof(a));
+  a.packed = packed; a.magT = magT; a.fbT = fbT; a.inv2 = inv2; a.unit_scale = unit_scale; a.crm = crm;
+  a.B = B; a.F = F; a.Tp = src_T; a.la = la; a.Ns = Ns; a.Nf = Nf; a.H = H; a.act = act;
+  a.steps = steps; a.shrink = 1; a.x3 = x3 != 0;
+  a.map = RowMap{B, F, Fsub, g};
+  a.stages = stages;
+  a.h0ws = h0ws; a.split_chunk = chunk_pairs;
+  return sb_tc_forward(a, st);
+}
+
 extern "C" int fsn_debug_sb_lstm_tc_probe(const fsn_seq_weights* sb, int H, int Ns, int Nf, int fc_out, int act, int x3,
                                           const float* magT, const float* fbT, int B, int F, int src_T, int G,
                                           const float* inv2, const float* unit_scale, int la, int steps, int shrink,
diff --git a/fullsubnet_b200/csrc/fsn_tc_ptx.cuh b/fullsubnet_b200/csrc/fsn_tc_ptx.cuh
--- a/fullsubnet_b200/csrc/fsn_tc_ptx.cuh
+++ b/fullsubnet_b200/csrc/fsn_tc_ptx.cuh
@@ -180,6 +180,13 @@
       : "memory");
 }
 __device__ __forceinline__ void fence_proxy_async() { asm volatile("fence.proxy.async;" ::: "memory"); }
+__device__ __forceinline__ void bulk_s2g(void* dst, const void* src, uint32_t bytes) {
+  asm volatile("cp.async.bulk.global.shared::cta.bulk_group [%0], [%1], %2;" ::"l"(dst), "r"(smem_u32(src)), "r"(bytes)
+               : "memory");
+}
+__device__ __forceinline__ void bulk_commit() { asm volatile("cp.async.bulk.commit_group;" ::: "memory"); }
+__device__ __forceinline__ void bulk_wait_read_all() { asm volatile("cp.async.bulk.wait_group.read 0;" ::: "memory"); }
+__device__ __forceinline__ void bulk_wait_all() { asm volatile("cp.async.bulk.wait_group 0;" ::: "memory"); }
 
 __device__ __forceinline__ void mbar_arrive(uint64_t* bar) {
   asm volatile("mbarrier.arrive.shared::cta.b64 _, [%0];" ::"r"(smem_u32(bar)) : "memory");
diff --git a/fullsubnet_b200/csrc/fsn_wgmma.cuh b/fullsubnet_b200/csrc/fsn_wgmma.cuh
--- a/fullsubnet_b200/csrc/fsn_wgmma.cuh
+++ b/fullsubnet_b200/csrc/fsn_wgmma.cuh
@@ -54,6 +54,20 @@
       : "memory");
 }
 
+__device__ __forceinline__ void mma_f16_n48_w(float (&d)[24], uint32_t a_lo, uint32_t a_off, uint32_t a_hi,
+                                              uint32_t b_lo, uint32_t b_off, uint32_t b_hi) {
+  asm volatile(
+      "{\n\t.reg .b32 al, bl;\n\t.reg .b64 a, b;\n\t"
+      "add.u32 al, %24, %25;\n\tadd.u32 bl, %27, %28;\n\t"
+      "mov.b64 a, {al, %26};\n\tmov.b64 b, {bl, %29};\n\t"
+      "wgmma.mma_async.sync.aligned.m64n48k16.f32.f16.f16 {%0,%1,%2,%3,%4,%5,%6,%7,%8,%9,%10,%11,%12,%13,%14,%15,%16,%17,"
+      "%18,%19,%20,%21,%22,%23}, a, b, 1, 1, 1, 0, 0;\n\t}"
+      : "+f"(d[0]), "+f"(d[1]), "+f"(d[2]), "+f"(d[3]), "+f"(d[4]), "+f"(d[5]), "+f"(d[6]), "+f"(d[7]), "+f"(d[8]), "+f"(d[9]), "+f"(d[10]), "+f"(d[11]), "+f"(d[12]), "+f"(d[13]), "+f"(d[14]), "+f"(d[15]),
+        "+f"(d[16]), "+f"(d[17]), "+f"(d[18]), "+f"(d[19]), "+f"(d[20]), "+f"(d[21]), "+f"(d[22]), "+f"(d[23])
+      : "r"(a_lo), "r"(a_off), "r"(a_hi), "r"(b_lo), "r"(b_off), "r"(b_hi)
+      : "memory");
+}
+
 __device__ __forceinline__ void mma_f16_n64(float (&d)[32], uint64_t a, uint64_t b, uint32_t scale_d) {
   asm volatile(
       "{\n\t.reg .pred p;\n\tsetp.ne.b32 p, %34, 0;\n\t"
diff --git a/include/fsn_b200.h b/include/fsn_b200.h
--- a/include/fsn_b200.h
+++ b/include/fsn_b200.h
@@ -362,6 +362,11 @@
                          const float* magT, const float* fbT, int B, int F, int src_T, int G,
                          const float* inv2, const float* unit_scale, int la, int steps, int shrink,
                          int stages, int cluster, void* packed, float* crm, fsn_stream_t stream);
+size_t fsn_debug_sb_lstm_tc2_ws_bytes(int R, int steps, int H, int x3, int chunk_pairs);
+int fsn_debug_sb_lstm_tc2(const fsn_seq_weights* sb, int H, int Ns, int Nf, int act, int x3, const float* magT,
+                          const float* fbT, int B, int F, int src_T, int G, const float* inv2, const float* unit_scale,
+                          int la, int steps, int stages, int chunk_pairs, void* packed, void* h0ws, float* crm,
+                          fsn_stream_t stream);
 int fsn_debug_sb_lstm_tc_carry(const fsn_seq_weights* sb, int H, int Ns, int Nf, int act, int x3, const float* magT,
                                const float* fbT, int B, int F, int src_T, const float* unit_scale, int steps,
                                const int32_t* restart, int store_step, float* h, float* c, void* packed, float* crm,
```

New measurement: 157,900, median of 6. +24.0%, better.
